# yangfei1223/CRFConv

Measured on AMD Instinct MI355X. Metric: M points/sec fwd+bwd, S3DIS 40960-pt cloud, K=16, 3 CRF iters; mIoU parity, higher is better.
Workload: dtype f32; 1 GPU; BASELINE configs[1]: S3DIS-like synthetic clouds (one point per 4 cm voxel of an 8x8x3 m box), 4 clouds x 40960 pts per GPU, K=16, ratios [4,4,4,4,2], PointConvBig(in=6, classes=13, use_crf, steps=3), train mode: fwd + weighted CE + bwd + flat-bucket grad all-reduce + SGD(momentum) step; tables resident in HBM; point order from the device collate: morton; global_batch=4, points_per_cloud=40960, parallelism=dp1 (batch-sharded)

## Files before the change

crfconv_amd/_lib.py:

```python
import ctypes
import os

_HERE = os.path.dirname(os.path.abspath(__file__))
LIB_PATH = os.environ.get('CRFCONV_LIB') or os.path.join(_HERE, 'libcrfconv_amd.so')

_vp, _i, _i64, _sz, _f = ctypes.c_void_p, ctypes.c_int, ctypes.c_int64, ctypes.c_size_t, ctypes.c_float
_d = ctypes.c_double
_u64 = ctypes.c_uint64

SIGNATURES = {
    'crfconv_abi_version': (_i, []),
    'crfconv_last_error': (ctypes.c_char_p, []),
    'crfconv_knn': (_i, [_vp, _sz, _sz, _vp, _sz, _sz, _vp]),
    'crfconv_knn_omp': (_i, [_vp, _sz, _sz, _vp, _sz, _sz, _vp]),
    'crfconv_knn_batch': (_i, [_vp, _sz, _sz, _sz, _vp, _sz, _sz, _vp]),
    'crfconv_knn_batch_omp': (_i, [_vp, _sz, _sz, _sz, _vp, _sz, _sz, _vp]),
    'crfconv_knn_batch_dev_workspace': (_sz, [_sz, _sz, _sz, _sz]),
    'crfconv_knn_batch_dev': (_i, [_vp, _sz, _sz, _sz, _vp, _sz, _sz, _vp, _vp, _vp, _sz, _vp]),
    'crfconv_fps': (_i, [_vp, _i, _vp, _vp, _vp, _vp, _vp, _vp, _vp, _vp]),
    'crfconv_grid_subsample': (_i64, [_vp, _i64, _vp, _i, _vp, _i, _f, _vp, _vp, _vp, _i64]),
    'crfconv_grid_subsample_dev_workspace': (_sz, [_i64, _i, _i]),
    'crfconv_grid_subsample_dev': (_i64, [_vp, _i64, _vp, _i, _vp, _i, _f, _vp, _vp, _vp, _i64, _vp, _sz, _vp]),
    'crfconv_index_narrow': (_i, [_vp, _i64, _i64, _i, _i64, _vp, _vp, _vp, _vp]),
    'crfconv_index_narrow_sorted': (_i, [_vp, _i64, _i64, _i, _i64, _i, _vp, _vp, _vp, _vp]),
    'crfconv_reverse_csr_workspace': (_sz, [_i64, _i64]),
    'crfconv_reverse_csr': (_i, [_vp, _i64, _i64, _vp, _vp, _vp, _sz, _vp]),
    'crfconv_reverse_csr_batched_workspace': (_sz, [_vp, _i]),
    'crfconv_reverse_csr_batched': (_i, [_vp, _i, _vp, _sz, _vp]),
    'crfconv_meanfield_forward': (_i, [_vp, _vp, _vp, _i, _i, _i64, _i, _vp, _vp, _i, _vp, _vp, _vp]),
    'crfconv_meanfield_forward_u16': (_i, [_vp, _vp, _vp, _vp, _i, _i, _i, _i, _i64, _i, _vp, _vp, _i, _vp, _vp, _vp]),
    'crfconv_meanfield_forward_block_rows': (_i, [_i64, _i, _i, _i, _i]),
    'crfconv_meanfield_forward_block': (_i, [_vp, _vp, _vp, _vp, _i, _i, _i, _i, _i64, _i, _vp, _vp, _i, _vp, _vp, _vp, _vp]),
    'crfconv_meanfield_forward_block_stamps': (_i, [_vp, _vp, _vp, _vp, _i, _i, _i64, _vp, _vp, _i, _vp, _vp, _vp, _i, _vp, _vp]),
    'crfconv_block_locality': (_i, [_vp, _i64, _i, _i, _i, _vp, _vp]),
    'crfconv_meanfield_bwd_edge': (_i, [_vp, _vp, _vp, _vp, _i, _i, _i64, _i, _vp, _vp, _vp, _vp, _i, _vp]),
    'crfconv_meanfield_bwd_scatter': (_i, [_vp, _vp, _vp, _vp, _i, _i, _i64, _i, _vp, _vp, _vp]),
    'crfconv_meanfield_backward_supported': (_i, [_i, _i, _i]),
    'crfconv_meanfield_backward_param_grads_inside': (_i, [_i]),
    'crfconv_meanfield_backward_workspace': (_sz, [_i64, _i, _i]),
    'crfconv_meanfield_backward': (_i, [_vp] * 7 + [_i, _i, _vp, _vp, _i, _i, _i64, _i, _vp, _vp, _i] + [_vp] * 11 + [_sz, _vp, _vp]),
    'crfconv_wide_similarity': (_i, [_vp, _vp, _i, _i, _i64, _i, _vp, _vp]),
    'crfconv_wide_aggregate': (_i, [_vp, _vp, _vp, _i, _i, _i64, _i, _vp, _vp]),
    'crfconv_wide_bwd_edge': (_i, [_vp, _vp, _vp, _i, _i, _i64, _i, _vp, _i, _vp]),
    'crfconv_wide_scatter': (_i, [_vp, _vp, _vp, _vp, _i, _i64, _i, _vp, _i, _vp, _vp]),
    'crfconv_wide_similarity_bwd': (_i, [_vp, _vp, _vp, _vp, _i, _i, _i64, _i, _vp, _vp, _vp]),
    'crfconv_similarity_bwd': (_i, [_vp, _vp, _vp, _vp, _i, _i, _i64, _i, _vp, _vp, _vp]),
    'crfconv_similarity_bwd_scatter': (_i, [_vp, _vp, _vp, _vp, _vp, _i, _i, _i64, _i, _vp, _vp]),
    'crfconv_pointconv_workspace': (_sz, [_i64, _i, _i]),
    'crfconv_pointconv_moments_packed': (_i, [_vp, _vp, _vp, _i, _i64, ctypes.c_double, _vp, _vp, _vp, _vp, _vp, _sz, _vp]),
    'crfconv_pointconv_moments': (_i, [_vp, _vp, _vp, _i, _i64, _vp, _vp, _sz, _vp]),
    'crfconv_pointconv_stats': (_i, [_vp, _vp, _vp, _i, _i64, _i, _vp, _vp, _vp, _f, _vp, _vp, _vp, _vp, _sz, _vp]),
    'crfconv_pointconv_forward_uv': (_i, [_vp, _vp, _vp, _vp, _i, _i64, _i, _vp, _vp, _vp, _f, _vp, _vp, _vp, _vp, _vp, _vp, _sz, _vp, _vp]),
    'crfconv_pointconv_forward_uv_hosts': (_i, [_i, _i]),
    'crfconv_pointconv_forward_uv_hosting': (_i, [_vp, _vp, _vp, _vp, _i, _i64, _i, _vp, _vp, _vp, _f, _vp, _vp, _vp, _vp, _vp, _vp, _sz, _vp,
                                                  _vp, _vp, _i, _vp, _vp, _vp]),
    'crfconv_pointconv_combine': (_i, [_vp, _vp, _vp, _vp, _vp, _vp, _d, _vp, _vp, _f, _f, _i64, _i, _vp, _vp, _vp, _vp, _vp]),
    'crfconv_pointconv_bwd_reduce_uv': (_i, [_vp, _vp, _vp, _i64, _i, _vp, _vp, _vp, _d, _i, _vp, _vp, _vp, _vp, _vp, _vp, _sz, _vp, _vp]),
    'crfconv_pointconv_forward': (_i, [_vp, _vp, _vp, _vp, _i, _i64, _i, _vp, _vp, _vp, _f, _vp, _vp, _vp, _vp]),
    'crfconv_pointconv_bwd_reduce': (_i, [_vp, _vp, _vp, _vp, _vp, _i, _i64, _i, _vp, _vp, _vp, _f, _vp, _vp, _vp, _sz, _vp]),
    'crfconv_pointconv_bwd_params': (_i, [_vp, _vp, _vp, _vp, _vp, _i, _i64, _i, _vp, _vp, _vp, _f, _vp, _vp, _vp,
                                          _vp, _vp, _vp, _sz, _vp]),
    'crfconv_pointconv_bwd_dump': (_i, [_vp, _vp, _vp, _vp, _vp, _i, _i64, _i, _vp, _vp, _vp, _f, _vp, _vp, _vp, _vp, _vp, _vp, _vp]),
    'crfconv_pointconv_bwd_a1_workspace': (_sz, [_i64, _i]),
    'crfconv_pointconv_bwd_a1': (_i, [_vp, _vp, _vp, _i64, _i, _f, _vp, _vp, _sz, _vp]),
    'crfconv_pointconv_bwd_input': (_i, [_vp, _vp, _vp, _vp, _vp, _i, _i64, _i, _vp, _vp, _vp, _f, _vp, _vp, _vp, _vp]),
    'crfconv_pointconv_bwd_input_reduce': (_i, [_vp, _vp, _vp, _vp, _vp, _i, _i64, _i64, _i, _vp, _vp, _vp, _f, _vp, _vp, _vp, _vp, _vp, _vp, _vp, _vp, _d, _i,
                                                _vp, _vp, _vp, _vp, _vp, _vp, _sz, _vp, _vp]),
    'crfconv_pointconv_fold1': (_i, [_vp, _vp, _vp, _vp, ctypes.c_double, _vp, _vp, _f, _f, _i, _i, _vp, _vp, _vp, _vp]),
    'crfconv_pointconv_fold1_batched': (_i, [_vp, _i, _vp]),
    'crfconv_pointconv_fold1_bwd_batched': (_i, [_vp, _i, _vp]),
    'crfconv_pointconv_fold1_bwd': (_i, [_vp, _vp, _vp, _vp, _vp, _f, _i, _i, _vp, _vp, _vp, _vp, _vp, _vp]),
    'crfconv_pointconv_fold2': (_i, [_vp, _vp, _vp, _vp, ctypes.c_double, _vp, _vp, _f, _f, _i, _i, _vp, _vp, _vp, _vp]),
    'crfconv_pointconv_fold2_bwd': (_i, [_vp, _vp, _vp, _vp, ctypes.c_double, _i, _i, _vp, _vp, _vp, _vp, _vp, _vp]),
    'crfconv_linear_wgrad_workspace': (_sz, [_i64, _i, _i]),
    'crfconv_linear_wgrad': (_i, [_vp, _vp, _i64, _i, _i, _vp, _vp, _vp, _sz, _vp]),
    'crfconv_random_subsets': (_i, [_vp, _vp, _vp, _vp, _i, _u64, _vp, _vp]),
    'crfconv_upindex_workspace': (_sz, [_i64, _i64]),
    'crfconv_upindex_from_table': (_i, [_vp, _vp, _vp, _vp, _i64, _i64, _i, _i64, _vp, _vp, _sz, _vp]),
    'crfconv_gather_rows_batched': (_i, [_vp, _vp, _vp, _i, _vp, _i, _i64, _i64, _i64, _vp]),
    'crfconv_argsort_codes_workspace': (_sz, [_i64, _i64]),
    'crfconv_argsort_codes': (_i, [_vp, _i64, _i64, _vp, _vp, _sz, _vp]),
    'crfconv_gridsync_workspace': (_sz, []),
    'crfconv_gridsync_fail_word': (_i, []),
    'crfconv_mlp_small_supported': (_i, [_i64, _i, _i]),
    'crfconv_mlp_small_workspace': (_sz, [_i64, _i]),
    'crfconv_mlp_small_forward': (_i, [_vp, _vp, _i64, _i, _i, _vp, _vp, _vp, _vp, _f, _f, _f, _vp, _vp, _vp, _vp, _sz, _vp, _sz, _vp]),
    'crfconv_mlp_small_forward_join': (_i, [_vp, _vp, _i64, _i, _i, _vp, _vp, _vp, _vp, _f, _f, _f, _vp, _f, _vp, _vp, _vp, _vp, _sz, _vp, _sz, _vp]),
    'crfconv_ticket_bytes': (_sz, []),
    'crfconv_mlp_backward_supported': (_i, [_i64, _i, _i]),
    'crfconv_mlp_backward_workspace': (_sz, [_i64, _i, _i]),
    'crfconv_mlp_backward': (_i, [_vp, _vp, _vp, _vp, _vp, _f, _i64, _i, _i, _vp, _vp, _vp, _vp, _vp, _sz, _vp, _vp]),
    'crfconv_linear_forward_cat': (_i, [_vp, _vp, _i, _vp, _vp, _i64, _i, _i, _vp, _vp, _vp]),
    'crfconv_linear_forward_uv_supported': (_i, [_i, _i]),
    'crfconv_linear_forward_uv': (_i, [_vp, _vp, _i64, _i, _i, _vp, _vp, _vp]),
    'crfconv_mlp_small_forward_uv_supported': (_i, [_i]),
    'crfconv_mlp_small_forward_join_uv': (_i, [_vp, _vp, _i64, _i, _i, _vp, _vp, _vp, _vp, _f, _f, _f, _vp, _f, _vp, _vp, _vp, _vp, _sz, _vp, _sz, _vp]),
    'crfconv_gemm_stats_uv_supported': (_i, [_i64, _i, _i]),
    'crfconv_gemm_stats_uv': (_i, [_vp, _vp, _i64, _i, _i, _vp, _vp, _vp]),
    'crfconv_mlp_dw_jobs': (_i, [_vp, _i, _vp]),
    'crfconv_mlp_dw_jobs_hosting': (_i, [_vp, _i, _vp, _vp, _vp, _vp, _vp, _i, _vp, _vp]),
    'crfconv_mlp_backward_add': (_i, [_vp, _vp, _vp, _vp, _vp, _f, _i64, _i, _i, _vp, _vp, _vp, _vp, _vp, _vp, _sz, _vp, _vp]),
    'crfconv_mlp_backward_add_mask': (_i, [_vp, _vp, _vp, _vp, _vp, _f, _i64, _i, _i, _vp, _f, _vp, _vp, _vp, _vp, _vp, _sz, _vp, _vp]),
    'crfconv_mlp_backward_cat': (_i, [_vp, _vp, _vp, _vp, _i, _vp, _vp, _f, _i64, _i, _i, _vp, _vp, _vp, _vp, _vp, _vp, _sz, _vp, _vp]),
    'crfconv_bn_workspace': (_sz, [_i64, _i]),
    'crfconv_bn_forward': (_i, [_vp, _i64, _i, _vp, _vp, _vp, _vp, _f, _f, _i, _f, _vp, _vp, _vp, _sz, _vp]),
    'crfconv_bn_backward': (_i, [_vp, _vp, _vp, _i64, _i, _i, _f, _vp, _vp, _vp, _vp, _sz, _vp]),
    'crfconv_bn_apply': (_i, [_vp, _i64, _i, _vp, _f, _vp, _vp]),
    'crfconv_pointconv_bwd_params_slabs': (_i, [_vp, _i64, _i, _vp, _vp, _vp]),
    'crfconv_pointconv_bwd_a1_nblk': (_i64, [_i64, _i]),
    'crfconv_reduce_jobs_f64': (_i, [_vp, _i, _vp]),
    'crfconv_pointconv_bwd_dump_jobs': (_i, [_vp, _i, _vp]),
    'crfconv_pointconv_bwd_a1_jobs': (_i, [_vp, _i, _vp]),
    'crfconv_pointconv_wide_params_supported': (_i, [_i64, _i, _i]),
    'crfconv_pointconv_wide_params_nblk': (_i64, [_i64, _i]),
    'crfconv_pointconv_wide_params_jobs': (_i, [_vp, _i, _vp]),
    'crfconv_gemm_jobs': (_i, [_vp, _i, _vp]),
    'crfconv_linear_wgrad_nblk': (_i, [_i64, _i, _i]),
    'crfconv_linear_wgrad_partial_jobs': (_i, [_vp, _i, _vp]),
    'crfconv_linear_wgrad_partial': (_i, [_vp, _vp, _i64, _i, _i, _i, _vp, _sz, _vp, _vp]),
    'crfconv_morton_codes': (_i, [_vp, _i64, _i64, _vp, _vp, _vp]),
    'crfconv_copy_jobs': (_i, [_vp, _i, _vp]),
    'crfconv_index_narrow_batched': (_i, [_vp, _i, _vp]),
    'crfconv_pointconv_moments_batched_workspace': (_sz, [_vp, _i]),
    'crfconv_pointconv_moments_batched': (_i, [_vp, _i, _vp, _sz, _vp]),
    'crfconv_reduce_jobs_both': (_i, [_vp, _i, _vp, _i, _vp]),
    'crfconv_reduce_jobs': (_i, [_vp, _i, _vp]),
    'crfconv_linear_forward_supported': (_i, [_i, _i]),
    'crfconv_linear_forward_stat_records': (_sz, [_i64]),
    'crfconv_linear_forward': (_i, [_vp, _vp, _vp, _i64, _i, _i, _i, _vp, _vp, _vp]),
    'crfconv_cat2': (_i, [_vp, _vp, _i64, _i, _i, _vp, _vp]),
    'crfconv_split2': (_i, [_vp, _i64, _i, _i, _vp, _vp, _vp]),
    'crfconv_add_i64': (_i, [_vp, _i64, _i64, _vp]),
    'crfconv_gate_mark': (_i, [_vp, _vp]),
    'crfconv_gate_wait': (_i, [_vp, _i, _vp]),
    'crfconv_mlp_small_backward_supported': (_i, [_i64, _i, _i]),
    'crfconv_gemm_stats_jobs': (_i, [_vp, _i, _vp]),
    'crfconv_bn_apply_from_records_jobs': (_i, [_vp, _i, _vp]),
    'crfconv_mlp_small_backward_jobs': (_i, [_vp, _i, _vp, _vp]),
    'crfconv_mlp_small_backward_jobs_one_launch': (_i, [_vp, _i, _vp, _vp, _vp]),
    'crfconv_mlp_small_backward_workspace': (_sz, [_i64, _i]),
    'crfconv_mlp_small_backward': (_i, [_vp, _vp, _vp, _vp, _vp, _i64, _i, _i, _i, _f, _vp, _vp, _vp, _vp, _vp, _sz, _vp, _vp]),
    'crfconv_gemm_stat_records': (_sz, [_i64]),
    'crfconv_gemm_stats': (_i, [_vp, _vp, _i64, _i, _i, _vp, _vp, _vp]),
    'crfconv_gemm_supported': (_i, [_i64, _i, _i]),
    'crfconv_gemm': (_i, [_vp, _vp, _vp, _vp, _i64, _i, _i, _i, _vp, _vp]),
    'crfconv_bn_apply_from_records': (_i, [_vp, _i64, _vp, _i64, _i, _vp, _vp, _vp, _vp, _f, _f, _vp, _f, _vp, _vp, _vp]),
    'crfconv_bn_coef_from_nrecords': (_i, [_vp, _i64, _i64, _i, _vp, _vp, _vp, _vp, _f, _f, _vp, _vp]),
    'crfconv_bn_coef_from_records': (_i, [_vp, _i64, _i, _vp, _vp, _vp, _vp, _f, _f, _vp, _vp]),
    'crfconv_softmax_ce_workspace': (_sz, [_i64]),
    'crfconv_softmax_ce_forward': (_i, [_vp, _vp, _vp, _i64, _i, _i64, _i64, _vp, _vp, _vp, _vp, _sz, _vp, _vp]),
    'crfconv_softmax_ce_backward': (_i, [_vp, _vp, _vp, _vp, _vp, _vp, _i64, _i, _i64, _i64, _vp, _vp]),
    'crfconv_crf_matrices': (_i, [_vp, _i, _vp, _vp, _vp]),
    'crfconv_crf_matrices_backward': (_i, [_vp, _vp, _vp, _vp, _i, _vp, _vp]),
    'crfconv_crf_matrices_batched': (_i, [_vp, _vp, _i, _vp, _vp, _vp]),
    'crfconv_crf_matrices_backward_batched': (_i, [_vp, _vp, _vp, _vp, _vp, _i, _vp, _vp]),
    'crfconv_add_lrelu': (_i, [_vp, _vp, _i64, _f, _vp, _vp]),
    'crfconv_bn_apply_add': (_i, [_vp, _i64, _i, _vp, _vp, _f, _vp, _vp]),
    'crfconv_bn_apply_dropout': (_i, [_vp, _i64, _i, _vp, _f, _f, _u64, _vp, _vp, _vp, _vp]),
    'crfconv_head_stats': (_i, [_vp, _vp, _i64, _i, _i, _vp, _vp]),
    'crfconv_head_stat_records': (_sz, [_i64]),
    'crfconv_head_supported': (_i, [_i64, _i, _i, _i]),
    'crfconv_head_mask_words': (_sz, [_i64]),
    'crfconv_head_backward_workspace': (_sz, [_i64, _i, _i, _i]),
    'crfconv_head_forward': (_i, [_vp, _vp, _vp, _f, _f, _u64, _vp, _vp, _vp, _i64, _i, _i, _i, _vp, _vp, _vp, _vp]),
    'crfconv_head_backward': (_i, [_vp, _vp, _vp, _vp, _f, _f, _vp, _vp, _i64, _i, _i, _i] + [_vp] * 7 + [_sz, _vp]),
    'crfconv_linear_forward_dropout': (_i, [_vp, _vp, _i64, _i, _i, _i, _f, _u64, _vp, _vp, _vp]),
    'crfconv_dropout_backward': (_i, [_vp, _i64, _f, _u64, _vp, _vp, _vp]),
    'crfconv_add_lrelu_backward': (_i, [_vp, _vp, _i64, _f, _vp, _vp]),
    'crfconv_add_mask': (_i, [_vp, _vp, _vp, _i64, _f, _vp, _vp]),
    'crfconv_sgd_step': (_i, [_vp, _vp, _vp, _i64, _f, _f, _f, _f, _i, _i, _vp]),
    'crfconv_sgd_step_hyper': (_i, [_vp, _vp, _vp, _i64, _vp, _i, _i, _vp]),
    'crfconv_sgd_step_guarded': (_i, [_vp, _vp, _vp, _i64, _vp, _i, _i, _vp, _vp]),
    'crfconv_sgd_step_guarded_all': (_i, [_vp, _vp, _vp, _i64, _vp, _i, _i, _vp, _i, _vp, _vp]),
    'crfconv_sgd_guard_publish': (_i, [_vp, _i, _vp, _vp]),
    'crfconv_adam_workspace': (_sz, [_i64]),
    'crfconv_adam_coef_floats': (_sz, []),
    'crfconv_adam_step': (_i, [_vp, _vp, _vp, _vp, _vp, _i64, _vp, _vp, _vp, _vp, _i, _i, _vp, _sz, _vp, _i, _vp, _vp]),
    'crfconv_spd_inverse': (_i, [_vp, _i, _vp, _vp]),
    'crfconv_spd_inverse_wide': (_i, [_vp, _i, _vp, _vp]),
    'crfconv_neighbor_maxpool_forward': (_i, [_vp, _vp, _i, _i64, _i, _vp, _vp, _vp]),
    'crfconv_neighbor_maxpool_affine_forward': (_i, [_vp, _vp, _vp, _i, _i64, _i, _vp, _vp, _vp]),
    'crfconv_neighbor_maxpool_backward': (_i, [_vp, _vp, _vp, _vp, _i, _i64, _i, _vp, _vp]),
    'crfconv_gather_rows': (_i, [_vp, _vp, _i64, _i, _vp, _vp]),
    'crfconv_gather_rows_backward': (_i, [_vp, _vp, _vp, _i64, _i, _vp, _vp]),
    'crfconv_meanfield_step': (_i, [_vp, _vp, _vp, _vp, _i, _i, _i64, _i, _vp, _vp, _vp, _vp]),
    'crfconv_kernel_weights_forward': (_i, [_vp, _vp, _i, _vp, _i, _i, _i64, _vp, _vp]),
    'crfconv_kernel_weights_partials': (_sz, [_i64]),
    'crfconv_kernel_weights_backward': (_i, [_vp, _vp, _vp, _vp, _vp, _i, _vp, _i, _i, _i64, _vp, _vp, _vp, _vp]),
    'crfconv_confusion_accumulate': (_i, [_vp, _vp, _vp, _i64, _i, _i64, _i64, _vp, _vp, _vp]),
    'crfconv_vote_accumulate': (_i, [_vp, _vp, _vp, _i64, _i, _d, _vp, _i64, _vp, _vp]),
    'crfconv_vote_accumulate_counted': (_i, [_vp, _vp, _vp, _i64, _i, _d, _vp, _i64, _vp, _vp, _vp]),
    'crfconv_vote_fold': (_i, [_vp, _vp, _vp, _vp, _i64, _i, _d, _vp]),
    'crfconv_vote_project': (_i, [_vp, _vp, _i64, _i, _i64, _i, _vp, _vp, _vp]),
    'crfconv_argmin_workspace': (_sz, []),
    'crfconv_argmin_f64': (_i, [_vp, _i64, _vp, _vp, _vp, _sz, _vp]),
    'crfconv_possibility_crop_workspace': (_sz, [_i64, _i64]),
    'crfconv_possibility_crop': (_i, [_vp, _i64, _i64, _vp, _vp, _vp, _vp, _vp, _vp, _vp, _vp, _vp, _sz, _vp]),
    'crfconv_augment_workspace': (_sz, [_i64, _i64]),
    'crfconv_augment': (_i, [_vp, _vp, _i64, _i64, _i, _vp, _u64, _vp, _vp, _vp, _vp, _vp, _sz, _vp]),
    'crfconv_possibility_crop_batch_workspace': (_sz, [_i64, _i64, _i64]),
    'crfconv_possibility_crop_batch': (_i, [_vp, _i, _i64, _vp, _vp, _i64, _i64, _u64, _vp, _d, _vp, _vp, _i, _vp, _vp, _i, _vp, _vp,
                                            _vp, _vp, _vp, _vp, _vp, _sz, _vp]),
    'crfconv_possibility_crop_batch_s3dis_workspace': (_sz, [_i64, _i64, _i64]),
    'crfconv_possibility_crop_batch_s3dis': (_i, [_vp, _i, _i64, _i64, _vp, _vp, _i64, _i64, _u64, _vp, _d, _vp, _vp, _i, _vp, _vp, _vp, _i,
                                                  _vp, _vp, _vp, _vp, _vp, _vp, _vp, _vp, _sz, _vp]),
    'crfconv_vote_update_repeated': (_i, [_vp, _vp, _vp, _i64, _i, _d, _vp, _i64, _vp, _vp, _vp, _vp]),
    'crfconv_vote_update_batch': (_i, [_vp, _i, _vp, _vp, _vp, _vp, _i64, _i64, _i64, _i, _d, _vp, _i, _vp]),
    'crfconv_vote_confusion': (_i, [_vp, _i64, _i, _vp, _vp, _i64, _i64, _vp, _vp, _vp]),
    'crfconv_linear_bn_act': (_i, [_vp, _vp, _i, _vp, _vp, _vp, _vp, _f, _i64, _i, _i, _vp, _vp]),
    'crfconv_gemm_bn_act': (_i, [_vp, _vp, _vp, _vp, _vp, _f, _i64, _i, _i, _i, _vp, _vp]),
    'crfconv_bn_eval_coef_jobs': (_i, [_vp, _i, _vp]),
}



class AugmentSpec(ctypes.Structure):
    _fields_ = [('rotate_axis', ctypes.c_int32), ('deg_lo', ctypes.c_float), ('deg_hi', ctypes.c_float), ('scale', ctypes.c_int32),
                ('scale_lo', ctypes.c_float), ('scale_span', ctypes.c_float), ('flip_axes', ctypes.c_int32), ('noise', ctypes.c_int32),
                ('sigma', ctypes.c_float), ('clip', ctypes.c_float), ('drop', ctypes.c_int32), ('drop_p', ctypes.c_float)]


class ReduceJob(ctypes.Structure):
    _fields_ = [('partial', ctypes.c_void_p), ('out', ctypes.c_void_p), ('nblk', ctypes.c_int32), ('nslots', ctypes.c_int32)]


class CopyJob(ctypes.Structure):
    _fields_ = [('src', ctypes.c_void_p), ('dst', ctypes.c_void_p), ('nbytes', ctypes.c_int64)]


class MlpDwJob(ctypes.Structure):
    _fields_ = [('workspace', ctypes.c_void_p), ('coef', ctypes.c_void_p), ('dW', ctypes.c_void_p), ('M', ctypes.c_int64),
                ('Ci', ctypes.c_int32), ('Co', ctypes.c_int32)]


class PcDumpJob(ctypes.Structure):
    _fields_ = [('x', ctypes.c_void_p), ('gout', ctypes.c_void_p), ('pos_src', ctypes.c_void_p), ('pos_tgt', ctypes.c_void_p),
                ('idx32', ctypes.c_void_p), ('K', ctypes.c_int32), ('m_tgt', ctypes.c_int64), ('d', ctypes.c_int32), ('A1', ctypes.c_void_p),
                ('b1', ctypes.c_void_p), ('W2', ctypes.c_void_p), ('slope', ctypes.c_float), ('ca', ctypes.c_void_p), ('cb', ctypes.c_void_p),
                ('cc', ctypes.c_void_p), ('h1', ctypes.c_void_p), ('gh2', ctypes.c_void_p), ('rel', ctypes.c_void_p)]


class PcWideJob(ctypes.Structure):
    _fields_ = [('x', ctypes.c_void_p), ('gout', ctypes.c_void_p), ('pos_src', ctypes.c_void_p), ('pos_tgt', ctypes.c_void_p),
                ('idx32', ctypes.c_void_p), ('K', ctypes.c_int32), ('m_tgt', ctypes.c_int64), ('d', ctypes.c_int32), ('A1', ctypes.c_void_p),
                ('b1', ctypes.c_void_p), ('W2', ctypes.c_void_p), ('slope', ctypes.c_float), ('ca', ctypes.c_void_p), ('cb', ctypes.c_void_p),
                ('cc', ctypes.c_void_p), ('dw2_partial', ctypes.c_void_p), ('a1_partial', ctypes.c_void_p)]

# ... 131 lines not shown
```

crfconv_amd/csrc/linear.hip:

```cpp
#include "common.hpp"
#include "gridsync.hpp"
#include "wgrad_body.hpp"
#include "crf_matrices_body.hpp"
#include "reduce64_body.hpp"
#include "uv_fold.hpp"

#include <cstdlib>

namespace crf {

template <int TCO, int TCI>
__global__ __launch_bounds__(WG_BLOCK) void wgrad_kernel(const float* __restrict__ G,
                                                         const float* __restrict__ X, int64_t M, int Co,
                                                         int Ci, int rows_per_block,
                                                         float* __restrict__ partial ,
                                                         float* __restrict__ partial_b ) {
    __shared__ float s_red[WG_RED_BUFS * TCO * TCI * 256];
    __shared__ float s_b[WG_WAVES * TCO * 16];
    wgrad_body<TCO, TCI>(G, X, M, Co, Ci, rows_per_block, partial, partial_b, blockIdx.x, blockIdx.y, blockIdx.z, s_red, s_b);
}

__global__ __launch_bounds__(WG_BLOCK) void wgrad_jobs_any_kernel(const WgJobTable t) {
    __shared__ float s_red[WG_RED_BUFS * 4 * 4 * 256];
    __shared__ float s_b[WG_WAVES * 4 * 16];
    wgrad_any_run(t, (int)blockIdx.x, s_red, s_b);
}


__device__ __forceinline__ void mlp_channel_part(int c, double s1, double s2, const float* __restrict__ coef, int64_t M, int Co,
                                                 float* __restrict__ dgamma, float* __restrict__ dbeta, float* __restrict__ bcoef) {
    dbeta[c] = (float)s1;
    dgamma[c] = (float)s2;
    const double a = coef[c], mu = coef[2 * Co + c], rs = coef[3 * Co + c];
    const double c2 = s1 / (double)M, c3 = s2 / (double)M;
    bcoef[c] = coef[c];
    bcoef[Co + c] = coef[Co + c];
    bcoef[2 * Co + c] = (float)a;
    bcoef[3 * Co + c] = (float)(-a * c3 * rs);
    bcoef[4 * Co + c] = (float)(-a * c2 + a * c3 * rs * mu);
}

template <int TCO, int TCI>
__global__ __launch_bounds__(WG_BLOCK) void mlp_bwd_p1_kernel(const float* __restrict__ GA, const float* __restrict__ Y,
                                                              const float* __restrict__ X,
                                                              const float* __restrict__ X2, int split ,
                                                              const float* __restrict__ coef ,
                                                              float slope, int64_t M, int Co, int Ci, int rows_per_block,
                                                              float* __restrict__ PA ,
                                                              float* __restrict__ PB ,
                                                              float* __restrict__ PG ,
                                                              float* __restrict__ PX ,
                                                              unsigned* __restrict__ ticket ,
                                                              float* __restrict__ dgamma, float* __restrict__ dbeta,
                                                              float* __restrict__ bcoef) {
    const int lane = threadIdx.x & 63, wave = threadIdx.x >> 6;
    const int co_base = blockIdx.y * 16 * TCO, ci_base = blockIdx.z * 16 * TCI;
    const int kk = lane >> 4, cc = lane & 15;
    f32x4 accA[TCO][TCI], accB[TCO][TCI];
#pragma unroll
    for (int a = 0; a < TCO; ++a)
#pragma unroll
        for (int b = 0; b < TCI; ++b) { accA[a][b] = f32x4{0.f, 0.f, 0.f, 0.f}; accB[a][b] = f32x4{0.f, 0.f, 0.f, 0.f}; }
    float ca[TCO], cb[TCO], cm[TCO], cr[TCO], sg[TCO], sgy[TCO], sx[TCI];
#pragma unroll
    for (int a = 0; a < TCO; ++a) {
        const int co = co_base + 16 * a + cc;
        const bool ok = co < Co;
        ca[a] = ok ? coef[co] : 0.f;
        cb[a] = ok ? coef[Co + co] : 0.f;
        cm[a] = ok ? coef[2 * Co + co] : 0.f;
        cr[a] = ok ? coef[3 * Co + co] : 0.f;
        sg[a] = 0.f;
        sgy[a] = 0.f;
    }
#pragma unroll
    for (int b = 0; b < TCI; ++b) sx[b] = 0.f;

    const int64_t row_begin = (int64_t)blockIdx.x * rows_per_block;
    const int64_t row_end = row_begin + rows_per_block < M ? row_begin + rows_per_block : M;
#ifndef P1_PREFETCH_
#define P1_PREFETCH_ 0
#endif
    struct Frag { float gv[4][TCO], yv[4][TCO], bv[4][TCI]; };
    auto load = [&](int64_t r0, Frag& f) {
#pragma unroll
        for (int u = 0; u < 4; ++u) {
            const int64_t r = r0 + 4 * u + kk;
            const bool rv = r < row_end;
#pragma unroll
            for (int a = 0; a < TCO; ++a) {
                const int co = co_base + 16 * a + cc;
                const bool ok = rv && co < Co;
                f.gv[u][a] = ok ? GA[r * Co + co] : 0.f;
                f.yv[u][a] = ok ? Y[r * Co + co] : cm[a];
            }
#pragma unroll
            for (int b = 0; b < TCI; ++b) {
                const int ci = ci_base + 16 * b + cc;
                float xv = 0.f;
                if (rv && ci < Ci) xv = (X2 == nullptr || ci < split) ? X[r * (X2 ? split : Ci) + ci] : X2[r * (Ci - split) + (ci - split)];
                f.bv[u][b] = xv;
            }
        }
    };
    auto compute = [&](const Frag& f) {
#pragma unroll
        for (int u = 0; u < 4; ++u) {
#pragma unroll
            for (int b = 0; b < TCI; ++b) sx[b] += f.bv[u][b];
#pragma unroll
            for (int a = 0; a < TCO; ++a) {
                const float g1 = f.gv[u][a] * (fmaf(ca[a], f.yv[u][a], cb[a]) > 0.f ? 1.f : slope);
                const float yh = (f.yv[u][a] - cm[a]) * cr[a];
                sg[a] += g1;
                sgy[a] = fmaf(g1, yh, sgy[a]);
#pragma unroll
                for (int b = 0; b < TCI; ++b) {
                    accA[a][b] = __builtin_amdgcn_mfma_f32_16x16x4f32(g1, f.bv[u][b], accA[a][b], 0, 0, 0);
                    accB[a][b] = __builtin_amdgcn_mfma_f32_16x16x4f32(yh, f.bv[u][b], accB[a][b], 0, 0, 0);
                }
            }
        }
    };
    if constexpr (P1_PREFETCH_ != 0) {
        Frag cur, nxt;
        load(row_begin + 16 * wave, cur);
        for (int64_t r0 = row_begin + 16 * wave; r0 < row_end; r0 += 16 * WG_WAVES) {
            load(r0 + 16 * WG_WAVES, nxt);
            compute(cur);
            cur = nxt;
        }
    } else {
        for (int64_t r0 = row_begin + 16 * wave; r0 < row_end; r0 += 16 * WG_WAVES) {
            Frag f;
            load(r0, f);
            compute(f);
        }
    }
    __shared__ __attribute__((aligned(16))) float s_red[WG_WAVES][TCO * TCI * 256];
    __shared__ float s_v[WG_WAVES][(2 * TCO + TCI) * 16];
    const int64_t pb = (int64_t)blockIdx.x;
    for (int pass = 0; pass < 2; ++pass) {
        if (pass) __syncthreads();
#pragma unroll
        for (int a = 0; a < TCO; ++a)
#pragma unroll
            for (int b = 0; b < TCI; ++b)
#pragma unroll
                for (int g = 0; g < 4; ++g)
                    s_red[wave][(a * TCI + b) * 256 + (4 * kk + g) * 16 + cc] = pass ? accB[a][b][g] : accA[a][b][g];
        if (pass == 0) {
#pragma unroll
            for (int a = 0; a < TCO; ++a) {
                float t1 = sg[a], t2 = sgy[a];
                t1 += __shfl_xor(t1, 16, WAVE); t1 += __shfl_xor(t1, 32, WAVE);
                t2 += __shfl_xor(t2, 16, WAVE); t2 += __shfl_xor(t2, 32, WAVE);
                if (kk == 0) { s_v[wave][a * 16 + cc] = t1; s_v[wave][(TCO + a) * 16 + cc] = t2; }
            }
// ... 465 lines not shown
    const bool live = (int)threadIdx.x < CMB_BLOCK && row < H && j < H;
    if (live) s_t[0][r][j] = (double)cmat[row * H + j];
    __syncthreads();
    double acc = 0.0;
    if (live)
        for (int k = 0; k < H; ++k) acc += s_t[0][r][k] * (double)s_q[k * 65 + j];
    if (live) s_t[1][r][j] = acc;
    __syncthreads();
    acc = 0.0;
    if (live)
        for (int k = 0; k < H; ++k) acc += s_t[1][r][k] * ((double)s_d[k * 65 + j] + (double)s_d[j * 65 + k]);
    if (live) s_t[0][r][j] = acc;
    __syncthreads();
    acc = 0.0;
    if (live) {
        for (int k = 0; k < H; ++k) acc += s_t[0][r][k] * (double)s_q[k * 65 + j];
        dc[row * H + j] = (float)(-acc);
    }
}
__global__ __launch_bounds__(CMB_BLOCK) void crf_matrices_bwd_kernel(const float* __restrict__ cmat, const float* __restrict__ Q,
                                                               const float* __restrict__ dQ, const float* __restrict__ dP,
                                                               int H, float* __restrict__ dc) {
    crf_matrices_bwd_slab(cmat, Q, dQ, dP, H, (int)blockIdx.x * CMB_ROWS, dc);
}
__global__ __launch_bounds__(CMB_BLOCK) void crf_matrices_bwd_batched_kernel(const CrfMatJobs j) {
    int b = 0;
    while (b + 1 < CM_MAX && (int)blockIdx.x >= j.slab_base[b + 1]) ++b;
    crf_matrices_bwd_slab(j.c[b], j.Q_in[b], j.gQ[b], j.gP[b], j.H[b], ((int)blockIdx.x - j.slab_base[b]) * CMB_ROWS, j.dc[b]);
}
static_assert(MF_BLOCK >= CMB_BLOCK, "a rider fits the host's workgroup");
__global__ __launch_bounds__(MF_BLOCK) void mlp_dw_jobs_hosting_kernel(const MlpDwTable t, const CrfMatJobs j, const int n_side) {
    if ((int)blockIdx.x < n_side) {
        int b = 0;
        while (b + 1 < CM_MAX && (int)blockIdx.x >= j.slab_base[b + 1]) ++b;
        crf_matrices_bwd_slab(j.c[b], j.Q_in[b], j.gQ[b], j.gP[b], j.H[b], ((int)blockIdx.x - j.slab_base[b]) * CMB_ROWS, j.dc[b]);
        return;
    }
    const int g = (int)blockIdx.x - n_side;
    int lo = 0, hi = t.njobs;
    while (hi - lo > 1) {
        const int mid = (lo + hi) >> 1;
        if (t.group_begin[mid] <= g) lo = mid; else hi = mid;
    }
    mlp_dw_slots(t.PA[lo], t.PB[lo], t.PG[lo], t.PX[lo], t.nblk[lo], t.coef[lo], (int64_t)t.M[lo], t.Co[lo], t.Ci[lo],
                 g - t.group_begin[lo], t.dW[lo]);
}
}

extern "C" int crfconv_crf_matrices_batched(const float* const* c, const int* H, int n, float* const* Q, float* const* P,
                                            crf_stream_t stream) {
    CRF_REQUIRE(c && H && Q && P && n >= 1 && n <= crf::CM_MAX, CRF_ERR_ARG, "null pointer or n=%d outside [1, %d]", n, crf::CM_MAX);
    crf::CrfMatJobs j = {};
    for (int i = 0; i < n; ++i) {
        CRF_REQUIRE(c[i] && Q[i] && P[i] && H[i] >= 1 && H[i] <= 64, CRF_ERR_ARG, "job %d: null pointer or H=%d outside [1, 64]", i, H[i]);
        j.c[i] = c[i]; j.Q[i] = Q[i]; j.P[i] = P[i]; j.H[i] = H[i];
    }
    hipLaunchKernelGGL(crf::crf_matrices_batched_kernel, dim3((unsigned)n), dim3(crf::CMF_BLOCK), 0, crf::as_stream(stream), j);
    CRF_LAUNCH_CHECK();
    return CRF_OK;
}

static int crf_matrices_bwd_jobs(const float* const* c, const float* const* Q, const float* const* gQ, const float* const* gP, const int* H, int n,
                                 float* const* dc, crf::CrfMatJobs& j, int& nslab) {
    CRF_REQUIRE(c && Q && gQ && gP && H && dc && n >= 1 && n <= crf::CM_MAX, CRF_ERR_ARG, "null pointer or n=%d outside [1, %d]", n, crf::CM_MAX);
    j = crf::CrfMatJobs();
    for (int i = 0; i < n; ++i) {
        CRF_REQUIRE(c[i] && Q[i] && dc[i] && H[i] >= 1 && H[i] <= 64, CRF_ERR_ARG, "job %d: null pointer or H=%d outside [1, 64]", i, H[i]);
        j.c[i] = c[i]; j.Q_in[i] = Q[i]; j.gQ[i] = gQ[i]; j.gP[i] = gP[i]; j.dc[i] = dc[i]; j.H[i] = H[i];
        j.slab_base[i + 1] = j.slab_base[i] + (H[i] + crf::CMB_ROWS - 1) / crf::CMB_ROWS;
    }
    nslab = j.slab_base[n];
    for (int i = n; i < crf::CM_MAX; ++i) j.slab_base[i + 1] = 0x7fffffff;
    return CRF_OK;
}
extern "C" int crfconv_crf_matrices_backward_batched(const float* const* c, const float* const* Q, const float* const* gQ,
                                                     const float* const* gP, const int* H, int n, float* const* dc,
                                                     crf_stream_t stream) {
    crf::CrfMatJobs j;
    int nslab = 0;
    if (int rc = crf_matrices_bwd_jobs(c, Q, gQ, gP, H, n, dc, j, nslab)) return rc;
    hipLaunchKernelGGL(crf::crf_matrices_bwd_batched_kernel, dim3((unsigned)nslab), dim3(crf::CMB_BLOCK), 0, crf::as_stream(stream), j);
    CRF_LAUNCH_CHECK();
    return CRF_OK;
}

namespace crf {
constexpr int SW_BLOCK = 1024, SW_MAXH = 512;
__global__ __launch_bounds__(SW_BLOCK) void spd_inverse_wide_kernel(const float* __restrict__ M, int H, float* __restrict__ Q) {
    __shared__ float s_row[SW_MAXH], s_col[SW_MAXH];
    const int n = H * H;
    for (int e = threadIdx.x; e < n; e += SW_BLOCK) Q[e] = M[e];
    __syncthreads();
    for (int k = 0; k < H; ++k) {
        for (int t = threadIdx.x; t < H; t += SW_BLOCK) {
            s_row[t] = Q[k * H + t];
            s_col[t] = Q[t * H + k];
        }
        __syncthreads();
        const float inv = 1.0f / s_row[k];
        for (int e = threadIdx.x; e < n; e += SW_BLOCK) {
            const int i = e / H, j = e - i * H;
            float v;
            if (i == k) v = j == k ? inv : s_row[j] * inv;
            else if (j == k) v = -s_col[i] * inv;
            else v = fmaf(-s_col[i] * inv, s_row[j], Q[e]);
            Q[e] = v;
        }
        __syncthreads();
    }
}
}

extern "C" int crfconv_spd_inverse_wide(const float* M, int H, float* Q, crf_stream_t stream) {
    CRF_REQUIRE(M && Q && M != Q, CRF_ERR_ARG, "null pointer / aliased operands");
    CRF_REQUIRE(H >= 1 && H <= crf::SW_MAXH, CRF_ERR_UNSUPPORTED, "H=%d outside [1, %d]", H, crf::SW_MAXH);
    hipLaunchKernelGGL(crf::spd_inverse_wide_kernel, dim3(1), dim3(crf::SW_BLOCK), 0, crf::as_stream(stream), M, H, Q);
    CRF_LAUNCH_CHECK();
    return CRF_OK;
}

extern "C" int crfconv_spd_inverse(const float* M, int H, float* Q, crf_stream_t stream) {
    CRF_REQUIRE(M && Q, CRF_ERR_ARG, "null pointer");
    CRF_REQUIRE(H >= 1 && H <= 64, CRF_ERR_UNSUPPORTED, "H=%d outside [1, 64]", H);
    hipLaunchKernelGGL(crf::spd_inverse_kernel, dim3(1), dim3(256), 0, crf::as_stream(stream), M, H, Q);
    CRF_LAUNCH_CHECK();
    return CRF_OK;
}

extern "C" int crfconv_crf_matrices(const float* c, int H, float* Q, float* P, crf_stream_t stream) {
    CRF_REQUIRE(c && Q && P, CRF_ERR_ARG, "null pointer");
    CRF_REQUIRE(H >= 1 && H <= 64, CRF_ERR_UNSUPPORTED, "H=%d outside [1, 64]", H);
    hipLaunchKernelGGL(crf::crf_matrices_kernel, dim3(1), dim3(crf::CMF_BLOCK), 0, crf::as_stream(stream), c, H, Q, P);
    CRF_LAUNCH_CHECK();
    return CRF_OK;
}

extern "C" int crfconv_crf_matrices_backward(const float* c, const float* Q, const float* dQ, const float* dP, int H,
                                             float* dc, crf_stream_t stream) {
    CRF_REQUIRE(c && Q && dc, CRF_ERR_ARG, "null pointer");
    CRF_REQUIRE(H >= 1 && H <= 64, CRF_ERR_UNSUPPORTED, "H=%d outside [1, 64]", H);
    hipLaunchKernelGGL(crf::crf_matrices_bwd_kernel, dim3((unsigned)((H + crf::CMB_ROWS - 1) / crf::CMB_ROWS)), dim3(crf::CMB_BLOCK), 0,
                       crf::as_stream(stream), c, Q, dQ, dP, H, dc);
    CRF_LAUNCH_CHECK();
    return CRF_OK;
}

namespace crf {

#ifndef LF_BLOCK_
#define LF_BLOCK_ 256
#endif
constexpr int LF_BLOCK = LF_BLOCK_, LF_WAVES = LF_BLOCK / WAVE;

constexpr int EPI_NONE = 0, EPI_ADD = 1, EPI_DROPOUT = 2, EPI_ADD_MASK = 3, EPI_UV = 4, EPI_BN_ACT = 5;
#ifndef LF_PF_MAX_
#define LF_PF_MAX_ 4
#endif
template <int TCO, bool PRO = false, bool VEC4 = true, int EPI = EPI_NONE, int NCH = 0>
__global__ __launch_bounds__(LF_BLOCK) void linear_fwd_kernel(const float* __restrict__ X, const float* __restrict__ W,
                                                              const float* __restrict__ bias, int64_t M, int Ci, int Co,
                                                              int transpose_w, float* __restrict__ Y,
                                                              float* __restrict__ stat_partial ,
                                                              const float* __restrict__ Y2 = nullptr,
                                                              const float* __restrict__ pro = nullptr, float slope = 1.f,
                                                              const float* __restrict__ Xb = nullptr, int xsplit = 0,
                                                              float* __restrict__ Yb = nullptr, int ysplit = 0,
                                                              const float* __restrict__ addend = nullptr,
                                                              const long long* __restrict__ drop_counter = nullptr,
                                                              unsigned long long drop_seed = 0ull, unsigned drop_threshold = 0u,
                                                              float drop_scale = 1.f,
                                                              const float* __restrict__ mask_ref = nullptr, float mask_slope = 1.f,
                                                              const UvFold uv = UvFold()) {
    static_assert(EPI != EPI_ADD_MASK || (PRO && VEC4), "the masked epilogue is the aligned dX product's");
    static_assert(EPI != EPI_UV || (!PRO && VEC4 && NCH == 1), "the combine prologue is the narrow aligned forward's");
    static_assert(EPI != EPI_BN_ACT || !PRO, "the BatchNorm epilogue is the forward product's");
    constexpr bool UV = EPI == EPI_UV, TWO = PRO || UV;
    constexpr bool BNA = EPI == EPI_BN_ACT;
    extern __shared__ float sW[];
    const int Cip = ((Ci + 15) / 16) * 16 + 4;
    const int Cik = ((Ci + 15) / 16) * 16;
    float* sPro = sW + 16 * TCO * Cip;
    [[maybe_unused]] float* sTile = sPro + (PRO ? 5 * Cik : 0);
    if constexpr (PRO) {
        for (int t = threadIdx.x; t < 5 * Cik; t += LF_BLOCK) {
            const int which = t / Cik, k = t - which * Cik;
            sPro[t] = k < Ci ? pro[which * Ci + k] : 0.f;
        }
    }
    const int co_base = blockIdx.y * 16 * TCO;
    if (!transpose_w && (Ci % 4) == 0) {
        const int Cip4 = Cip / 4, Ci4 = Ci / 4;
        for (int t = threadIdx.x; t < 16 * TCO * Cip4; t += LF_BLOCK) {
            const int r = t / Cip4, k4 = t - r * Cip4;
            const int co = co_base + r;
            float4 v = make_float4(0.f, 0.f, 0.f, 0.f);
            if (co < Co && k4 < Ci4) v = *reinterpret_cast<const float4*>(W + (int64_t)co * Ci + 4 * k4);
            *reinterpret_cast<float4*>(sW + r * Cip + 4 * k4) = v;
        }
    } else {
        for (int t = threadIdx.x; t < 16 * TCO * Cip; t += LF_BLOCK) {
            const int r = t / Cip, k = t - r * Cip;
            const int co = co_base + r;
            float v = 0.f;
            if (co < Co && k < Ci) v = transpose_w ? W[(int64_t)k * Co + co] : W[(int64_t)co * Ci + k];
            sW[t] = v;
        }
    }
    __syncthreads();
    const int lane = threadIdx.x & 63, wave = threadIdx.x >> 6;
    const int rr = lane & 15, g = lane >> 4;
    const bool vec = (Ci % 4) == 0;
    float bsel[TCO][4];
#pragma unroll
    for (int t = 0; t < TCO; ++t)
#pragma unroll
        for (int e = 0; e < 4; ++e) {
            const int co = co_base + 16 * t + 4 * g + e;
            bsel[t][e] = (bias != nullptr && co < Co) ? bias[co] : 0.f;
        }
    [[maybe_unused]] float4 bna[BNA ? TCO : 1], bnb[BNA ? TCO : 1];
    if constexpr (BNA) {
#pragma unroll
        for (int t = 0; t < TCO; ++t) {
            const int co = TCO >= 2 ? co_base + 4 * ((lane + WAVE * t) % (4 * TCO)) : co_base + 16 * t + 4 * g;
            bna[t] = bnb[t] = make_float4(0.f, 0.f, 0.f, 0.f);
            if (co < Co) {
                bna[t] = *reinterpret_cast<const float4*>(pro + co);
                bnb[t] = *reinterpret_cast<const float4*>(pro + Co + co);
            }
        }
    }
    [[maybe_unused]] auto bn_act4 = [&](float4 y, const float4 a, const float4 b, const float* skp) -> float4 {
        float4 o = make_float4(fmaf(a.x, y.x, b.x), fmaf(a.y, y.y, b.y), fmaf(a.z, y.z, b.z), fmaf(a.w, y.w, b.w));
        if (skp != nullptr) {
            const float4 k = *reinterpret_cast<const float4*>(skp);
            o = make_float4(add_rn(o.x, k.x), add_rn(o.y, k.y), add_rn(o.z, k.z), add_rn(o.w, k.w));
        }
        if (slope != 1.f) {
            o.x = o.x > 0.f ? o.x : slope * o.x;
            o.y = o.y > 0.f ? o.y : slope * o.y;
            o.z = o.z > 0.f ? o.z : slope * o.z;
            o.w = o.w > 0.f ? o.w : slope * o.w;
        }
        return o;
    };
    float s1[TCO][4], s2[TCO][4], sh[TCO][4];
#pragma unroll
    for (int t = 0; t < TCO; ++t)
#pragma unroll
        for (int e = 0; e < 4; ++e) { s1[t][e] = 0.f; s2[t][e] = 0.f; sh[t][e] = 0.f; }
    bool have_shift = false;
    const int nchunk = (Ci + 15) / 16;

    const float4 zero4 = make_float4(0.f, 0.f, 0.f, 0.f);
    auto load_raw = [&](int64_t r, bool rv, int c, float4& xa, float4& xb2) {
        const int k0 = 16 * c + 4 * g;
        xa = zero4;
        xb2 = zero4;
        if (!rv || k0 >= Ci) return;
        if constexpr (PRO) {
            xa = *reinterpret_cast<const float4*>(X + r * Ci + k0);
            xb2 = *reinterpret_cast<const float4*>(Y2 + r * Ci + k0);
        } else if constexpr (UV) {
            xa = *reinterpret_cast<const float4*>(X + r * Ci + k0);
            xb2 = *reinterpret_cast<const float4*>(uv.V + r * Ci + k0);
        } else if (Xb != nullptr) {
            if (k0 < xsplit) xa = *reinterpret_cast<const float4*>(X + r * xsplit + k0);
            else xa = *reinterpret_cast<const float4*>(Xb + r * (Ci - xsplit) + (k0 - xsplit));
        } else if (VEC4 || vec) {
            xa = *reinterpret_cast<const float4*>(X + r * Ci + k0);
        } else if constexpr (!VEC4) {
            const float* xp = X + r * Ci;
            xa.x = xp[k0];
            xa.y = k0 + 1 < Ci ? xp[k0 + 1] : 0.f;
            xa.z = k0 + 2 < Ci ? xp[k0 + 2] : 0.f;
            xa.w = k0 + 3 < Ci ? xp[k0 + 3] : 0.f;
        }
    };
    auto operand = [&](bool rv, int c, float4 gv, float4 yv) -> float4 {
        if constexpr (PRO) {
            const int k0 = 16 * c + 4 * g;
            float4 xv = zero4;
            if (rv && k0 < Ci) {
                const float4 pa = *reinterpret_cast<const float4*>(sPro + k0), pb = *reinterpret_cast<const float4*>(sPro + Cik + k0);
                const float4 al = *reinterpret_cast<const float4*>(sPro + 2 * Cik + k0), be = *reinterpret_cast<const float4*>(sPro + 3 * Cik + k0);
                const float4 de = *reinterpret_cast<const float4*>(sPro + 4 * Cik + k0);
                xv.x = fmaf(al.x * (fmaf(pa.x, yv.x, pb.x) > 0.f ? 1.f : slope), gv.x, fmaf(be.x, yv.x, de.x));
                xv.y = fmaf(al.y * (fmaf(pa.y, yv.y, pb.y) > 0.f ? 1.f : slope), gv.y, fmaf(be.y, yv.y, de.y));
                xv.z = fmaf(al.z * (fmaf(pa.z, yv.z, pb.z) > 0.f ? 1.f : slope), gv.z, fmaf(be.z, yv.z, de.z));
                xv.w = fmaf(al.w * (fmaf(pa.w, yv.w, pb.w) > 0.f ? 1.f : slope), gv.w, fmaf(be.w, yv.w, de.w));
            }
            return xv;
        } else {
            return gv;
        }
    };
    [[maybe_unused]] float4 uva = zero4, uvt = zero4;
    if constexpr (UV) {
        if (blockIdx.x == 0 && blockIdx.y == 0 && (int)threadIdx.x < Ci) {
            const UvCoef k = uv_coef(threadIdx.x, Ci, uv.stats, uv.shift, uv.gamma, uv.beta, uv.n_edges, uv.eps);
            uv_publish(threadIdx.x, Ci, k, uv.n_edges, uv.run_mean, uv.run_var, uv.momentum, uv.a2, uv.b2, uv.aux2);
        }
        if (4 * g < Ci) {
            float a[4], tv[4];
#pragma unroll
            for (int e = 0; e < 4; ++e) {
                const UvCoef k = uv_coef(4 * g + e, Ci, uv.stats, uv.shift, uv.gamma, uv.beta, uv.n_edges, uv.eps);
                a[e] = k.a;
                tv[e] = uv_vcoef(k);
            }
            uva = make_float4(a[0], a[1], a[2], a[3]);
            uvt = make_float4(tv[0], tv[1], tv[2], tv[3]);
        }
    }
    [[maybe_unused]] auto uv_operand = [&](int64_t r, bool rv, float4 u, float4 v) -> float4 {
        if (!rv || 4 * g >= Ci) return zero4;
        const float4 o = uv_out4(uva, uvt, u, v);
        if (blockIdx.y == 0) *reinterpret_cast<float4*>(uv.out + r * Ci + 4 * g) = o;
        return o;
    };
    constexpr int NCA = NCH > 0 ? NCH : 1;
    constexpr bool PF = NCH > 0 && NCH <= LF_PF_MAX_;
    const int64_t row_stride = (int64_t)gridDim.x * (LF_BLOCK / WAVE) * 16;
    [[maybe_unused]] float4 fa[NCA], fb[TWO ? NCA : 1], na[PF ? NCA : 1], nb[(PF && TWO) ? NCA : 1];
    [[maybe_unused]] auto load_group = [&](int64_t rw0, float4 (&xa)[NCA], float4 (&xb)[TWO ? NCA : 1]) {
        const int64_t rq = rw0 + rr;
        const bool ok = rw0 < M && rq < M;
#pragma unroll
        for (int c = 0; c < NCA; ++c) {
            float4 t0, t1;
            load_raw(rq, ok, c, t0, t1);
            xa[c] = t0;
            if constexpr (TWO) xb[c] = t1;
        }
    };
    if constexpr (PF) load_group(((int64_t)blockIdx.x * (LF_BLOCK / WAVE) + wave) * 16, fa, fb);
    for (int64_t row0 = ((int64_t)blockIdx.x * (LF_BLOCK / WAVE) + wave) * 16; row0 < M; row0 += row_stride) {
        const int64_t r = row0 + rr;
        const bool rv = r < M;
        f32x4 acc[TCO];
#pragma unroll
        for (int t = 0; t < TCO; ++t) acc[t] = f32x4{bsel[t][0], bsel[t][1], bsel[t][2], bsel[t][3]};
        if constexpr (NCH > 0) {
            if constexpr (PF) {
                if constexpr (TWO) load_group(row0 + row_stride, na, nb);
                else load_group(row0 + row_stride, na, fb);
            } else {
                load_group(row0, fa, fb);
            }
#pragma unroll
            for (int c = 0; c < NCH; ++c) {
                const int k0 = 16 * c + 4 * g;
                float4 xv;
                if constexpr (UV) xv = uv_operand(r, rv, fa[c], fb[c]);
                else xv = operand(rv, c, fa[c], fb[PRO ? c : 0]);
#pragma unroll
                for (int t = 0; t < TCO; ++t) {
                    const float4 wv = *reinterpret_cast<const float4*>(sW + (16 * t + rr) * Cip + k0);
                    acc[t] = __builtin_amdgcn_mfma_f32_16x16x4f32(wv.x, xv.x, acc[t], 0, 0, 0);
                    acc[t] = __builtin_amdgcn_mfma_f32_16x16x4f32(wv.y, xv.y, acc[t], 0, 0, 0);
                    acc[t] = __builtin_amdgcn_mfma_f32_16x16x4f32(wv.z, xv.z, acc[t], 0, 0, 0);
                    acc[t] = __builtin_amdgcn_mfma_f32_16x16x4f32(wv.w, xv.w, acc[t], 0, 0, 0);
                }
            }
            if constexpr (PF) {
#pragma unroll
                for (int c = 0; c < NCH; ++c) {
                    fa[c] = na[c];
                    if constexpr (TWO) fb[c] = nb[c];
                }
            }
        } else {
        for (int c = 0; c < nchunk; ++c) {
            const int k0 = 16 * c + 4 * g;
            float4 ra, rb;
            load_raw(r, rv, c, ra, rb);
            const float4 xv = operand(rv, c, ra, rb);
#pragma unroll
            for (int t = 0; t < TCO; ++t) {
                const float4 wv = *reinterpret_cast<const float4*>(sW + (16 * t + rr) * Cip + k0);
                acc[t] = __builtin_amdgcn_mfma_f32_16x16x4f32(wv.x, xv.x, acc[t], 0, 0, 0);
                acc[t] = __builtin_amdgcn_mfma_f32_16x16x4f32(wv.y, xv.y, acc[t], 0, 0, 0);
                acc[t] = __builtin_amdgcn_mfma_f32_16x16x4f32(wv.z, xv.z, acc[t], 0, 0, 0);
                acc[t] = __builtin_amdgcn_mfma_f32_16x16x4f32(wv.w, xv.w, acc[t], 0, 0, 0);
            }
        }
        }
        if constexpr (TCO >= 2) {
            constexpr int TW = 16 * TCO, TLD = TW + 4, F4R = TW / 4;
            float* tile = sTile + wave * 16 * TLD;
#pragma unroll
            for (int t = 0; t < TCO; ++t)
                *reinterpret_cast<float4*>(tile + rr * TLD + 16 * t + 4 * g) = make_float4(acc[t][0], acc[t][1], acc[t][2], acc[t][3]);
            __builtin_amdgcn_wave_barrier();
#pragma unroll
            for (int i = 0; i < (16 * F4R) / WAVE; ++i) {
                const int qd = lane + WAVE * i, trow = qd / F4R, tc4 = qd - trow * F4R;
                const int64_t orow = row0 + trow;
                const int co = co_base + 4 * tc4;
                if (orow < M && co < Co) {
                    float4 o4 = *reinterpret_cast<const float4*>(tile + trow * TLD + 4 * tc4);
                    if constexpr (EPI == EPI_ADD) {
                        {
                            if (VEC4 || (Co % 4) == 0) {
                                const float4 a4 = *reinterpret_cast<const float4*>(addend + orow * Co + co);
                                o4.x += a4.x; o4.y += a4.y; o4.z += a4.z; o4.w += a4.w;
                            } else {
                                o4.x += addend[orow * Co + co];
                                if (co + 1 < Co) o4.y += addend[orow * Co + co + 1];
                                if (co + 2 < Co) o4.z += addend[orow * Co + co + 2];
                                if (co + 3 < Co) o4.w += addend[orow * Co + co + 3];
                            }
                        }
                    }
                    if constexpr (EPI == EPI_ADD_MASK) {
                        const float4 a4 = *reinterpret_cast<const float4*>(addend + orow * Co + co);
                        const float4 r4 = *reinterpret_cast<const float4*>(mask_ref + orow * Co + co);
                        o4.x += a4.x; o4.y += a4.y; o4.z += a4.z; o4.w += a4.w;
                        o4.x = r4.x > 0.f ? o4.x : mask_slope * o4.x;
                        o4.y = r4.y > 0.f ? o4.y : mask_slope * o4.y;
                        o4.z = r4.z > 0.f ? o4.z : mask_slope * o4.z;
                        o4.w = r4.w > 0.f ? o4.w : mask_slope * o4.w;
                    }
                    if constexpr (BNA) o4 = bn_act4(o4, bna[i], bnb[i], addend != nullptr ? addend + orow * Co + co : nullptr);
                    if constexpr (EPI == EPI_DROPOUT) {
                        {
                            const unsigned long long ctr = (unsigned long long)drop_counter[0];
                            const unsigned long long e = (unsigned long long)(orow * Co + co);
                            o4.x = dropout_keep(drop_seed, ctr, e, drop_threshold) ? o4.x * drop_scale : 0.f;
                            o4.y = dropout_keep(drop_seed, ctr, e + 1, drop_threshold) ? o4.y * drop_scale : 0.f;
                            o4.z = dropout_keep(drop_seed, ctr, e + 2, drop_threshold) ? o4.z * drop_scale : 0.f;
                            o4.w = dropout_keep(drop_seed, ctr, e + 3, drop_threshold) ? o4.w * drop_scale : 0.f;
                        }
                    }
                    if (Yb != nullptr) {
                        if (co < ysplit) *reinterpret_cast<float4*>(Y + orow * ysplit + co) = o4;
                        else *reinterpret_cast<float4*>(Yb + orow * (Co - ysplit) + (co - ysplit)) = o4;
                    } else if (VEC4 || (Co % 4) == 0) {
                        *reinterpret_cast<float4*>(Y + orow * Co + co) = o4;
                    } else if constexpr (!VEC4) {
                        const float ov[4] = {o4.x, o4.y, o4.z, o4.w};
#pragma unroll
                        for (int e = 0; e < 4; ++e)
                            if (co + e < Co) Y[orow * Co + co + e] = ov[e];
                    }
                }
            }
            __builtin_amdgcn_wave_barrier();
        } else {
#pragma unroll
        for (int t = 0; t < TCO; ++t) {
            const int co = co_base + 16 * t + 4 * g;
            if constexpr (EPI == EPI_ADD) {
                if (rv) {
#pragma unroll
                    for (int e = 0; e < 4; ++e)
                        if (co + e < Co) acc[t][e] += addend[r * Co + co + e];
                }
            }
            if constexpr (EPI == EPI_ADD_MASK) {
                if (rv && co < Co) {
                    const float4 a4 = *reinterpret_cast<const float4*>(addend + r * Co + co);
                    const float4 r4 = *reinterpret_cast<const float4*>(mask_ref + r * Co + co);
                    const float av[4] = {a4.x, a4.y, a4.z, a4.w}, rf[4] = {r4.x, r4.y, r4.z, r4.w};
#pragma unroll
                    for (int e = 0; e < 4; ++e) {
                        const float v = acc[t][e] + av[e];
                        acc[t][e] = rf[e] > 0.f ? v : mask_slope * v;
                    }
                }
            }
            if constexpr (BNA) {
                if (rv && co < Co) {
                    const float4 o4 = bn_act4(make_float4(acc[t][0], acc[t][1], acc[t][2], acc[t][3]), bna[t], bnb[t],
                                              addend != nullptr ? addend + r * Co + co : nullptr);
                    acc[t] = f32x4{o4.x, o4.y, o4.z, o4.w};
                }
            }
            if constexpr (EPI == EPI_DROPOUT) {
                if (rv) {
                    const unsigned long long ctr = (unsigned long long)drop_counter[0];
#pragma unroll
                    for (int e = 0; e < 4; ++e)
                        if (co + e < Co)
                            acc[t][e] = dropout_keep(drop_seed, ctr, (unsigned long long)(r * Co + co + e), drop_threshold)
                                            ? acc[t][e] * drop_scale : 0.f;
                }
            }
            if (rv) {
                if (Yb != nullptr) {
                    const float4 o4 = make_float4(acc[t][0], acc[t][1], acc[t][2], acc[t][3]);
                    if (co < ysplit) *reinterpret_cast<float4*>(Y + r * ysplit + co) = o4;
                    else if (co < Co) *reinterpret_cast<float4*>(Yb + r * (Co - ysplit) + (co - ysplit)) = o4;
                } else if (VEC4) {
                    if (co < Co) *reinterpret_cast<float4*>(Y + r * Co + co) = make_float4(acc[t][0], acc[t][1], acc[t][2], acc[t][3]);
                } else if (co + 3 < Co && (Co % 4) == 0) {
                    *reinterpret_cast<float4*>(Y + r * Co + co) = make_float4(acc[t][0], acc[t][1], acc[t][2], acc[t][3]);
                } else if constexpr (!VEC4) {
#pragma unroll
                    for (int e = 0; e < 4; ++e)
                        if (co + e < Co) Y[r * Co + co + e] = acc[t][e];
                }
            }
        }
        }
        if (!BNA && stat_partial != nullptr) {
            if (!have_shift) {
// ... 22 lines not shown
        for (int64_t row0 = ((int64_t)blockIdx.x * (LF_BLOCK / WAVE) + wave) * 16; row0 < M;
             row0 += (int64_t)gridDim.x * (LF_BLOCK / WAVE) * 16)
            nrows += (M - row0) < 16 ? (M - row0) : 16;
#pragma unroll
        for (int t = 0; t < TCO; ++t)
#pragma unroll
            for (int e = 0; e < 4; ++e) {
                float a = s1[t][e], b = s2[t][e];
#pragma unroll
                for (int o = 8; o > 0; o >>= 1) {
                    a += __shfl_xor(a, o, WAVE);
                    b += __shfl_xor(b, o, WAVE);
                }
                if (rr == 0) {
                    const int cl = 16 * t + 4 * g + e;
                    sw[cl] = sh[t][e];
                    sw[16 * TCO + cl] = (float)nrows;
                    sw[2 * 16 * TCO + cl] = a;
                    sw[3 * 16 * TCO + cl] = b;
                }
            }
        __syncthreads();
        for (int cl = threadIdx.x; cl < 16 * TCO; cl += LF_BLOCK) {
            const int co = co_base + cl;
            if (co >= Co) continue;
            const float s0 = sW[cl];
            double n = 0.0, S1 = 0.0, S2 = 0.0;
            for (int w = 0; w < LF_BLOCK / WAVE; ++w) {
                const float* q = sW + w * 4 * 16 * TCO;
                const double nb = q[16 * TCO + cl];
                if (nb <= 0.0) continue;
                const double d = (double)q[cl] - (double)s0, a = q[2 * 16 * TCO + cl], b = q[3 * 16 * TCO + cl];
                n += nb;
                S1 += a + nb * d;
                S2 += b + 2.0 * d * a + nb * d * d;
            }
            *reinterpret_cast<float4*>(stat_partial + ((int64_t)blockIdx.x * Co + co) * 4) =
                make_float4(s0, (float)n, (float)S1, (float)S2);
        }
    }
}

constexpr int FR_BLOCK = 1024, FR_CH = 16, FR_RL = FR_BLOCK / FR_CH;
template <int FR_UN = 8>
__device__ __forceinline__ bool bn_finalize_records_body(const float* __restrict__ rec, int nrec, int64_t M, int C,
                                                         const float* __restrict__ gamma, const float* __restrict__ beta, float eps,
                                                         float* __restrict__ run_mean, float* __restrict__ run_var, float momentum,
                                                         float* __restrict__ coef, int slab, bool write, float (&ab)[2]) {
    __shared__ double s_red[FR_BLOCK / WAVE][2][FR_CH];
    const int cl = threadIdx.x & (FR_CH - 1), rl = threadIdx.x >> 4;
    const int c = slab * FR_CH + cl;
    const bool cv = c < C;
    const int cc = cv ? c : C - 1;
    const double s0 = rec[(int64_t)cc * 4];
    double S1 = 0.0, S2 = 0.0;
    for (int r0 = rl; r0 < nrec; r0 += FR_UN * FR_RL) {
        float4 v[FR_UN];
#pragma unroll
        for (int u = 0; u < FR_UN; ++u) {
            const int r = r0 + u * FR_RL;
            v[u] = r < nrec ? *reinterpret_cast<const float4*>(rec + ((int64_t)r * C + cc) * 4)
                            : make_float4(0.f, 0.f, 0.f, 0.f);
        }
#pragma unroll
        for (int u = 0; u < FR_UN; ++u) {
            const double nb = v[u].y;
            if (nb > 0.0) {
                const double d = (double)v[u].x - s0, a = v[u].z, b = v[u].w;
                S1 += a + nb * d;
                S2 += b + 2.0 * d * a + nb * d * d;
            }
        }
    }
    S1 += __shfl_xor(S1, 16, WAVE); S2 += __shfl_xor(S2, 16, WAVE);
    S1 += __shfl_xor(S1, 32, WAVE); S2 += __shfl_xor(S2, 32, WAVE);
    const int wave = threadIdx.x >> 6;
    if ((threadIdx.x & 63) < FR_CH) { s_red[wave][0][cl] = S1; s_red[wave][1][cl] = S2; }
    __syncthreads();
    if (threadIdx.x >= FR_CH || !cv) return false;
    S1 = 0.0; S2 = 0.0;
    for (int w = 0; w < FR_BLOCK / WAVE; ++w) { S1 += s_red[w][0][cl]; S2 += s_red[w][1][cl]; }
    const double m1 = S1 / (double)M;
    const double mean = s0 + m1;
    const double m2 = S2 - S1 * m1;
    double var = m2 / (double)M;
    if (var < 0.0) var = 0.0;
    const double rstd = 1.0 / sqrt(var + (double)eps);
    const double a = (double)gamma[c] * rstd;
    ab[0] = (float)a;
    ab[1] = (float)((double)beta[c] - a * mean);
    if (!write) return true;
    coef[c] = ab[0];
    coef[C + c] = ab[1];
    coef[2 * C + c] = (float)mean;
    coef[3 * C + c] = (float)rstd;
    if (run_mean != nullptr) {
        const double unb = M > 1 ? var * ((double)M / (double)(M - 1)) : var;
        run_mean[c] = (float)((1.0 - (double)momentum) * (double)run_mean[c] + (double)momentum * mean);
        run_var[c] = (float)((1.0 - (double)momentum) * (double)run_var[c] + (double)momentum * unb);
    }
    return true;
}
__global__ __launch_bounds__(FR_BLOCK) void bn_finalize_records_kernel(const float* __restrict__ rec, int nrec, int64_t M,
                                                                       int C, const float* __restrict__ gamma,
                                                                       const float* __restrict__ beta, float eps,
                                                                       float* __restrict__ run_mean, float* __restrict__ run_var,
                                                                       float momentum, float* __restrict__ coef) {
    float ab[2];
    bn_finalize_records_body(rec, nrec, M, C, gamma, beta, eps, run_mean, run_var, momentum, coef, blockIdx.x, true, ab);
}

template <bool ADD, int UN = 8>
__device__ __forceinline__ void bn_apply_records_body(const float* __restrict__ rec, int nrec, int64_t M, int C,
                                                      const float* __restrict__ gamma, const float* __restrict__ beta,
                                                      float eps, float* __restrict__ run_mean, float* __restrict__ run_var,
                                                      float momentum, float* __restrict__ coef, const float* __restrict__ x,
                                                      const float* __restrict__ skip, float slope, int rows_per_tile,
                                                      float* __restrict__ y, const int slab, const int tile) {
    __shared__ float s_ab[2][FR_CH];
    float ab[2];
    const int q = threadIdx.x & 3, rl = threadIdx.x >> 2;
    const int c = slab * FR_CH + 4 * q;
    const bool cok = c < C;
    const int64_t r0 = (int64_t)tile * rows_per_tile;
    const int64_t r1 = r0 + rows_per_tile < M ? r0 + rows_per_tile : M;
    float4 v[4];
    [[maybe_unused]] float4 k[ADD ? 4 : 1];
    auto request = [&](int64_t rb) {
#pragma unroll
        for (int u = 0; u < 4; ++u) {
            const int64_t r = rb + (int64_t)u * (FR_BLOCK / 4);
            const bool in = cok && r < r1;
            v[u] = in ? *reinterpret_cast<const float4*>(x + r * C + c) : make_float4(0.f, 0.f, 0.f, 0.f);
            if constexpr (ADD) k[u] = in ? *reinterpret_cast<const float4*>(skip + r * C + c) : make_float4(0.f, 0.f, 0.f, 0.f);
        }
    };
#ifndef BN_APPLY_PREFETCH_
#define BN_APPLY_PREFETCH_ 1
#endif
    if (BN_APPLY_PREFETCH_) request(r0 + rl);
    if (bn_finalize_records_body<UN>(rec, nrec, M, C, gamma, beta, eps, run_mean, run_var, momentum, coef, slab, tile == 0, ab)) {
        s_ab[0][threadIdx.x] = ab[0];
        s_ab[1][threadIdx.x] = ab[1];
    }
    __syncthreads();
    if (!cok) return;
    const float4 a = *reinterpret_cast<const float4*>(&s_ab[0][4 * q]), b = *reinterpret_cast<const float4*>(&s_ab[1][4 * q]);
    for (int64_t rb = r0 + rl; rb < r1; rb += 4 * (FR_BLOCK / 4)) {
        if (!BN_APPLY_PREFETCH_ || rb != r0 + rl) request(rb);
#pragma unroll
        for (int u = 0; u < 4; ++u) {
            const int64_t r = rb + (int64_t)u * (FR_BLOCK / 4);
            if (r >= r1) continue;
            float4 o = make_float4(fmaf(a.x, v[u].x, b.x), fmaf(a.y, v[u].y, b.y), fmaf(a.z, v[u].z, b.z), fmaf(a.w, v[u].w, b.w));
            if constexpr (ADD) {
                o.x = add_rn(o.x, k[u].x); o.y = add_rn(o.y, k[u].y); o.z = add_rn(o.z, k[u].z); o.w = add_rn(o.w, k[u].w);
            }
            o.x = o.x > 0.f ? o.x : slope * o.x;
            o.y = o.y > 0.f ? o.y : slope * o.y;
            o.z = o.z > 0.f ? o.z : slope * o.z;
            o.w = o.w > 0.f ? o.w : slope * o.w;
            *reinterpret_cast<float4*>(y + r * C + c) = o;
        }
    }
}

template <bool ADD>
__global__ __launch_bounds__(FR_BLOCK) void bn_apply_records_kernel(const float* __restrict__ rec, int nrec, int64_t M, int C,
                                                                    const float* __restrict__ gamma, const float* __restrict__ beta,
                                                                    float eps, float* __restrict__ run_mean, float* __restrict__ run_var,
                                                                    float momentum, float* __restrict__ coef, const float* __restrict__ x,
                                                                    const float* __restrict__ skip, float slope, int rows_per_tile,
                                                                    float* __restrict__ y) {
    bn_apply_records_body<ADD>(rec, nrec, M, C, gamma, beta, eps, run_mean, run_var, momentum, coef, x, skip, slope, rows_per_tile, y,
                               blockIdx.y, blockIdx.x);
}
constexpr int BA_MAX = 4;
struct BnApplyJobs {
    const float* rec[BA_MAX]; const float* gamma[BA_MAX]; const float* beta[BA_MAX]; float* run_mean[BA_MAX]; float* run_var[BA_MAX];
    float* coef[BA_MAX]; const float* x[BA_MAX]; const float* skip[BA_MAX]; float* y[BA_MAX];
    long long M[BA_MAX];
    int nrec[BA_MAX], C[BA_MAX], rows_per_tile[BA_MAX], tiles[BA_MAX];
    float eps[BA_MAX], momentum[BA_MAX], slope[BA_MAX];
    int blk_base[BA_MAX + 1];
    int njobs;
};
__global__ __launch_bounds__(FR_BLOCK) void bn_apply_records_jobs_kernel(const BnApplyJobs t) {
    int j = 0;
    while (j + 1 < t.njobs && t.blk_base[j + 1] <= (int)blockIdx.x) ++j;
    const int local = (int)blockIdx.x - t.blk_base[j];
    const int tiles = uni(t.tiles[j]);
    const int tile = uni(local % tiles), slab = uni(local / tiles);
    const float* rec = uni(t.rec[j]); const float* gamma = uni(t.gamma[j]); const float* beta = uni(t.beta[j]);
    float* run_mean = uni(t.run_mean[j]); float* run_var = uni(t.run_var[j]); float* coef = uni(t.coef[j]);
    const float* x = uni(t.x[j]); const float* skip = uni(t.skip[j]); float* y = uni(t.y[j]);
    const long long M = uni(t.M[j]);
    const int nrec = uni(t.nrec[j]), C = uni(t.C[j]), rows = uni(t.rows_per_tile[j]);
    const float eps = uni(t.eps[j]), momentum = uni(t.momentum[j]), slope = uni(t.slope[j]);
    if (skip != nullptr) bn_apply_records_body<true, 4>(rec, nrec, M, C, gamma, beta, eps, run_mean, run_var, momentum, coef, x, skip, slope, rows, y, slab, tile);
    else bn_apply_records_body<false, 4>(rec, nrec, M, C, gamma, beta, eps, run_mean, run_var, momentum, coef, x, nullptr, slope, rows, y, slab, tile);
}

static int lf_blocks(int64_t M) {
    constexpr int cap = 512;
    int64_t nb = (M + 16 * LF_WAVES - 1) / (16 * LF_WAVES);
    if (nb > cap) nb = cap;
    return (int)(nb < 1 ? 1 : nb);
}

}

static size_t lf_lds_bytes_at(int Ci, int tco, bool pro) {
    const size_t cip = (size_t)((Ci + 15) / 16) * 16 + 4, cik = cip - 4;
    size_t floats = 16 * (size_t)tco * cip;
    const size_t stats = (size_t)crf::LF_WAVES * 4 * 16 * (size_t)tco;
    if (floats < stats) floats = stats;
    if (pro) floats += 5 * cik;
    if (tco >= 2) floats += (size_t)crf::LF_WAVES * 16 * (16 * (size_t)tco + 4);
    return sizeof(float) * floats;
}
static int lf_tco(int Ci, int Co, bool pro) {
    constexpr int max_tco = 4;
    const int tiles = (Co + 15) / 16;
    int tco = tiles >= 8 ? 8 : (tiles >= 4 ? 4 : (tiles >= 2 ? 2 : 1));
    if (tco > max_tco) tco = max_tco;
    while (tco > 1 && lf_lds_bytes_at(Ci, tco, pro) > 64 * 1024) tco >>= 1;
    return tco;
}
static size_t lf_lds_bytes(int Ci, int Co, bool pro) { return lf_lds_bytes_at(Ci, lf_tco(Ci, Co, pro), pro); }
static int lf_hoist_chunks(int Ci, bool vec4) {
    if (!vec4 || Ci > 128) return 0;
    const int n = (Ci + 15) / 16;
    return n <= 1 ? 1 : (n <= 2 ? 2 : (n <= 4 ? 4 : 8));
}

extern "C" int crfconv_linear_forward_supported(int Ci, int Co) {
    if (Ci < 1 || Co < 1) return 0;
    return lf_lds_bytes(Ci, Co, false) <= 64 * 1024 ? 1 : 0;
}

extern "C" size_t crfconv_linear_forward_stat_records(int64_t M) { return (size_t)crf::lf_blocks(M); }

struct LinearDropout {
    const long long* counter = nullptr;
    unsigned long long seed = 0ull;
    unsigned threshold = 0u;
    float scale = 1.f;
};

struct LinearBnAct {
    const float* coef = nullptr;
    const float* skip = nullptr;
    float slope = 1.f;
};

static int linear_forward_impl(const float* X, const float* Xb, int xsplit, const float* W, const float* bias, int64_t M,
                               int Ci, int Co, int transpose_w, float* Y, float* stat_rec, crf_stream_t stream,
                               LinearDropout drop = LinearDropout(), LinearBnAct bn = LinearBnAct()) {
    CRF_REQUIRE(X && W && Y, CRF_ERR_ARG, "null pointer");
    CRF_REQUIRE(M > 0, CRF_ERR_ARG, "M must be positive");
    CRF_REQUIRE(crfconv_linear_forward_supported(Ci, Co), CRF_ERR_UNSUPPORTED, "weight slab %dx%d does not fit LDS", Co, Ci);
    CRF_REQUIRE(Xb == nullptr || (xsplit > 0 && xsplit < Ci && xsplit % 4 == 0 && Ci % 4 == 0), CRF_ERR_ARG,
                "two-operand form needs 0 < split < Ci, both multiples of 4 (split=%d Ci=%d)", xsplit, Ci);
    const int tiles = (Co + 15) / 16;
    const int tco = lf_tco(Ci, Co, false);
    const int gy = (tiles + tco - 1) / tco;
    const dim3 grid((unsigned)crf::lf_blocks(M), (unsigned)gy), blk(crf::LF_BLOCK);
    const size_t lds = lf_lds_bytes(Ci, Co, false);
    hipStream_t st = crf::as_stream(stream);
    const bool vec4 = (Ci % 4) == 0 && (Co % 4) == 0;
    const int nch = lf_hoist_chunks(Ci, vec4);
#define LF4(T, V, E, N) hipLaunchKernelGGL((crf::linear_fwd_kernel<T, false, V, E, N>), grid, blk, lds, st, X, W, bias, M, Ci, Co, transpose_w, Y, stat_rec, (const float*)nullptr, bn.coef, bn.slope, Xb, xsplit, (float*)nullptr, 0, bn.skip, drop.counter, drop.seed, drop.threshold, drop.scale)
#define LF3(T, V, E) do { if (V && nch == 1) LF4(T, V, E, 1); else if (V && nch == 2) LF4(T, V, E, 2); else if (V && nch == 4) LF4(T, V, E, 4); else if (V && nch == 8) LF4(T, V, E, 8); else LF4(T, V, E, 0); } while (0)
#define LF2(T, V) do { if (bn.coef != nullptr) LF3(T, V, crf::EPI_BN_ACT); else if (drop.counter != nullptr) LF4(T, V, crf::EPI_DROPOUT, 0); else LF3(T, V, crf::EPI_NONE); } while (0)
#define LF(T) do { if (vec4) LF2(T, true); else if (bn.coef != nullptr) LF4(T, false, crf::EPI_BN_ACT, 0); else if (drop.counter != nullptr) LF4(T, false, crf::EPI_DROPOUT, 0); else LF4(T, false, crf::EPI_NONE, 0); } while (0)
    switch (tco) {
        case 1: LF(1); break;
        case 2: LF(2); break;
        case 4: LF(4); break;
        default: LF(8); break;
    }
#undef LF
#undef LF2
#undef LF3
#undef LF4
    CRF_LAUNCH_CHECK();
    return CRF_OK;
}

extern "C" int crfconv_linear_forward(const float* X, const float* W, const float* bias, int64_t M, int Ci, int Co,
                                      int transpose_w, float* Y, float* stat_rec, crf_stream_t stream) {
    return linear_forward_impl(X, nullptr, 0, W, bias, M, Ci, Co, transpose_w, Y, stat_rec, stream);
}

extern "C" int crfconv_linear_forward_dropout(const float* X, const float* W, int64_t M, int Ci, int Co, int transpose_w,
                                              float p, uint64_t seed, const int64_t* counter, float* Y, crf_stream_t stream) {
    CRF_REQUIRE(counter, CRF_ERR_ARG, "null pointer");
    CRF_REQUIRE(p >= 0.f && p < 1.f, CRF_ERR_ARG, "dropout probability %g outside [0, 1)", (double)p);
    LinearDropout d;
    d.counter = reinterpret_cast<const long long*>(counter);
    d.seed = (unsigned long long)seed;
    d.threshold = crf::dropout_threshold(p);
    d.scale = 1.f / (1.f - p);
    return linear_forward_impl(X, nullptr, 0, W, nullptr, M, Ci, Co, transpose_w, Y, nullptr, stream, d);
}

extern "C" int crfconv_linear_forward_cat(const float* Xa, const float* Xb, int split, const float* W, const float* bias,
                                          int64_t M, int Ci, int Co, float* Y, float* stat_rec, crf_stream_t stream) {
    CRF_REQUIRE(Xb, CRF_ERR_ARG, "null pointer");
    return linear_forward_impl(Xa, Xb, split, W, bias, M, Ci, Co, 0, Y, stat_rec, stream);
}

extern "C" int crfconv_linear_bn_act(const float* X, const float* Xb, int split, const float* W, const float* bias, const float* coef,
                                     const float* skip, float slope, int64_t M, int Ci, int Co, float* Y, crf_stream_t stream) {
    CRF_REQUIRE(coef, CRF_ERR_ARG, "null pointer");
    CRF_REQUIRE(Co % 4 == 0, CRF_ERR_UNSUPPORTED, "Co=%d must be a multiple of 4", Co);
    LinearBnAct bn;
    bn.coef = coef;
    bn.skip = skip;
    bn.slope = slope;
    return linear_forward_impl(X, Xb, Xb ? split : 0, W, bias, M, Ci, Co, 0, Y, nullptr, stream, LinearDropout(), bn);
}

extern "C" int crfconv_linear_forward_uv_supported(int Ci, int Co) { return ((Ci == 8 && Co == 32) || (Ci == 16 && Co == 64)) ? 1 : 0; }

extern "C" int crfconv_linear_forward_uv(const crf_uv_fold* f, const float* W, int64_t M, int Ci, int Co, float* Y, float* stat_rec,
                                         crf_stream_t stream) {
    CRF_REQUIRE(W && Y, CRF_ERR_ARG, "null pointer");
    CRF_REQUIRE(crf::uv_fold_complete(f), CRF_ERR_ARG, "combine record: null pointer, or running statistics not as a pair");
    CRF_REQUIRE(M > 0, CRF_ERR_ARG, "M must be positive");
    CRF_REQUIRE(crfconv_linear_forward_uv_supported(Ci, Co), CRF_ERR_UNSUPPORTED, "combine prologue: %d -> %d is not a fine-level lin_out", Ci, Co);
    const int tco = lf_tco(Ci, Co, false);
    CRF_REQUIRE(16 * tco == Co && lf_hoist_chunks(Ci, true) == 1, CRF_ERR_UNSUPPORTED, "combine prologue: one column group, one chunk");
    const dim3 grid((unsigned)crf::lf_blocks(M), 1u), blk(crf::LF_BLOCK);
    const size_t lds = lf_lds_bytes(Ci, Co, false);
    hipStream_t st = crf::as_stream(stream);
    const crf::UvFold uv = crf::uv_fold_args(f);
#define LFU(T) hipLaunchKernelGGL((crf::linear_fwd_kernel<T, false, true, crf::EPI_UV, 1>), grid, blk, lds, st, f->U, W, (const float*)nullptr, M, Ci, Co, 0, Y, stat_rec, (const float*)nullptr, (const float*)nullptr, 1.f, (const float*)nullptr, 0, (float*)nullptr, 0, (const float*)nullptr, (const long long*)nullptr, 0ull, 0u, 1.f, (const float*)nullptr, 1.f, uv)
    if (tco == 2) LFU(2);
    else LFU(4);
#undef LFU
    CRF_LAUNCH_CHECK();
    return CRF_OK;
}

extern "C" int crfconv_bn_coef_from_records(const float* stat_rec, int64_t M, int C, const float* gamma,
                                            const float* beta, float* run_mean, float* run_var, float momentum,
                                            float eps, float* coef, crf_stream_t stream) {
    CRF_REQUIRE(stat_rec && gamma && beta && coef, CRF_ERR_ARG, "null pointer");
    CRF_REQUIRE(M > 0 && C > 0, CRF_ERR_ARG, "bad shape");
    return crfconv_bn_coef_from_nrecords(stat_rec, (int64_t)crfconv_linear_forward_stat_records(M), M, C, gamma, beta, run_mean, run_var,
                                         momentum, eps, coef, stream);
}

extern "C" int crfconv_bn_coef_from_nrecords(const float* stat_rec, int64_t nrec, int64_t M, int C, const float* gamma,
                                             const float* beta, float* run_mean, float* run_var, float momentum,
                                             float eps, float* coef, crf_stream_t stream) {
    CRF_REQUIRE(stat_rec && gamma && beta && coef, CRF_ERR_ARG, "null pointer");
    CRF_REQUIRE(M > 0 && C > 0 && nrec > 0 && nrec < ((int64_t)1 << 31), CRF_ERR_ARG, "bad shape");
    hipLaunchKernelGGL(crf::bn_finalize_records_kernel, dim3((C + crf::FR_CH - 1) / crf::FR_CH), dim3(crf::FR_BLOCK), 0, crf::as_stream(stream), stat_rec,
                       (int)nrec, M, C, gamma, beta, eps, run_mean, run_var, momentum, coef);
    CRF_LAUNCH_CHECK();
    return CRF_OK;
}

#ifndef BN_APPLY_WGS_
#define BN_APPLY_WGS_ 256
#endif
static void bn_apply_plan(int64_t M, int C, int wgs, int64_t& tiles, int64_t& rows) {
    const int slabs = (C + crf::FR_CH - 1) / crf::FR_CH;
    tiles = wgs / slabs;
    if (tiles < 1) tiles = 1;
    rows = (M + tiles - 1) / tiles;
    rows = (rows + 1023) / 1024 * 1024;
    tiles = (M + rows - 1) / rows;
    if (tiles > 8) tiles = (tiles + 7) / 8 * 8;
}

extern "C" int crfconv_bn_apply_from_records(const float* stat_rec, int64_t nrec, const float* x, int64_t M, int C, const float* gamma,
                                             const float* beta, float* run_mean, float* run_var, float momentum, float eps,
                                             const float* skip, float slope, float* coef, float* y, crf_stream_t stream) {
    CRF_REQUIRE(stat_rec && x && gamma && beta && coef && y, CRF_ERR_ARG, "null pointer");
    CRF_REQUIRE(M > 0 && C >= 4 && C % 4 == 0 && nrec > 0 && nrec < ((int64_t)1 << 31), CRF_ERR_ARG, "bad shape");
    const int slabs = (C + crf::FR_CH - 1) / crf::FR_CH;
    int64_t tiles, rows;
    bn_apply_plan(M, C, BN_APPLY_WGS_, tiles, rows);
    const dim3 grid((unsigned)tiles, (unsigned)slabs), blk(crf::FR_BLOCK);
    if (skip != nullptr)
        hipLaunchKernelGGL(crf::bn_apply_records_kernel<true>, grid, blk, 0, crf::as_stream(stream), stat_rec, (int)nrec, M, C, gamma, beta, eps,
                           run_mean, run_var, momentum, coef, x, skip, slope, (int)rows, y);
    else
        hipLaunchKernelGGL(crf::bn_apply_records_kernel<false>, grid, blk, 0, crf::as_stream(stream), stat_rec, (int)nrec, M, C, gamma, beta, eps,
                           run_mean, run_var, momentum, coef, x, skip, slope, (int)rows, y);
    CRF_LAUNCH_CHECK();
    return CRF_OK;
}

extern "C" int crfconv_bn_apply_from_records_jobs(const crf_bn_apply_job* jobs, int njobs, crf_stream_t stream) {
    CRF_REQUIRE(jobs && njobs >= 1 && njobs <= crf::BA_MAX, CRF_ERR_ARG, "1 .. %d jobs (got %d)", crf::BA_MAX, njobs);
    crf::BnApplyJobs t;
    int64_t blocks = 0;
    for (int j = 0; j <= crf::BA_MAX; ++j) {
        t.blk_base[j] = (int)blocks;
        if (j >= crf::BA_MAX) break;
        if (j >= njobs) {
            t.rec[j] = nullptr; t.gamma[j] = nullptr; t.beta[j] = nullptr; t.run_mean[j] = nullptr; t.run_var[j] = nullptr; t.coef[j] = nullptr;
            t.x[j] = nullptr; t.skip[j] = nullptr; t.y[j] = nullptr; t.M[j] = 0; t.nrec[j] = 0; t.C[j] = 4; t.rows_per_tile[j] = 1024; t.tiles[j] = 1;
            t.eps[j] = 0.f; t.momentum[j] = 0.f; t.slope[j] = 1.f;
            continue;
        }
        const crf_bn_apply_job& b = jobs[j];
        CRF_REQUIRE(b.stat_rec && b.x && b.gamma && b.beta && b.coef && b.y, CRF_ERR_ARG, "job %d: null pointer", j);
        CRF_REQUIRE(b.M > 0 && b.C >= 4 && b.C % 4 == 0 && b.nrec > 0 && b.nrec < ((int64_t)1 << 31), CRF_ERR_ARG, "job %d: bad shape", j);
        int64_t tiles, rows;
        bn_apply_plan(b.M, b.C, BN_APPLY_WGS_ / njobs, tiles, rows);
        t.rec[j] = b.stat_rec; t.gamma[j] = b.gamma; t.beta[j] = b.beta; t.run_mean[j] = b.run_mean; t.run_var[j] = b.run_var; t.coef[j] = b.coef;
        t.x[j] = b.x; t.skip[j] = b.skip; t.y[j] = b.y; t.M[j] = (long long)b.M; t.nrec[j] = (int)b.nrec; t.C[j] = b.C; t.rows_per_tile[j] = (int)rows;
        t.tiles[j] = (int)tiles; t.eps[j] = b.eps; t.momentum[j] = b.momentum; t.slope[j] = b.slope;
        blocks += tiles * ((b.C + crf::FR_CH - 1) / crf::FR_CH);
        CRF_REQUIRE(blocks < ((int64_t)1 << 31), CRF_ERR_UNSUPPORTED, "too many workgroups in one batch");
    }
    t.njobs = njobs;
    hipLaunchKernelGGL(crf::bn_apply_records_jobs_kernel, dim3((unsigned)blocks), dim3(crf::FR_BLOCK), 0, crf::as_stream(stream), t);
    CRF_LAUNCH_CHECK();
    return CRF_OK;
}

namespace crf {
struct MlpPlan {
    int tco, tci, gy, gz, nblk, rows_per_block;
};
static MlpPlan mlp_plan(int64_t M, int Co, int Ci) {
    MlpPlan p;
    const int t_co = (Co + 15) / 16, t_ci = (Ci + 15) / 16;
    p.tco = t_co >= 4 ? 4 : (t_co >= 2 ? 2 : 1);
    p.tci = t_ci >= 4 ? 4 : (t_ci >= 2 ? 2 : 1);
    if (p.tco * p.tci == 16) p.tci = 2;
    p.gy = (t_co + p.tco - 1) / p.tco;
    p.gz = (t_ci + p.tci - 1) / p.tci;
#ifndef MLP_P1_TARGET_
#define MLP_P1_TARGET_ 512
#endif
    constexpr int target = MLP_P1_TARGET_;
    int64_t slices = target / ((int64_t)p.gy * p.gz);
    if (slices < 32) slices = 32;
    int64_t rows = (M + slices - 1) / slices;
    if (rows < 64) rows = 64;
    rows = (rows + 63) / 64 * 64;
    p.rows_per_block = (int)rows;
    p.nblk = (int)((M + rows - 1) / rows);
    return p;
}
static size_t mlp_ws_layout(int64_t M, int Co, int Ci, size_t off[5]) {
    const MlpPlan p = mlp_plan(M, Co, Ci);
    auto up = [](size_t v) { return (v + 255) & ~(size_t)255; };
    size_t o = 0;
    off[0] = o; o = up(o + sizeof(float) * (size_t)p.nblk * Co * Ci);
    off[1] = o; o = up(o + sizeof(float) * (size_t)p.nblk * Co * Ci);
    off[2] = o; o = up(o + sizeof(float) * (size_t)p.nblk * 2 * Co);
    off[3] = o; o = up(o + sizeof(float) * (size_t)p.nblk * Ci);
    off[4] = o; o = up(o + sizeof(float) * 5 * (size_t)Co);
    return o;
}
}

extern "C" size_t crfconv_ticket_bytes(void) { return sizeof(unsigned) * crf::LW_TICKET_WORDS; }

extern "C" int crfconv_mlp_backward_supported(int64_t M, int Ci, int Co) {
    if (!(M > 0 && Co % 4 == 0 && Ci >= 1 && Co >= 4 && Co <= 1024 && Ci <= 1024)) return 0;
    return lf_lds_bytes(Co, Ci, true) <= 64 * 1024 ? 1 : 0;
}

extern "C" size_t crfconv_mlp_backward_workspace(int64_t M, int Ci, int Co) {
    if (M <= 0 || Co <= 0 || Ci <= 0) return 0;
    size_t off[5];
    return crf::mlp_ws_layout(M, Co, Ci, off) + 256;
}

static int mlp_backward_impl(const float* gA, const float* Y, const float* X, const float* Xb, int xsplit, const float* W,
                             const float* coef, float slope, int64_t M, int Ci, int Co, float* dX, float* dXb, float* dW,
                             float* dgamma, float* dbeta, void* workspace, size_t workspace_bytes, unsigned* ticket,
                             crf_stream_t stream, const float* dX_add = nullptr, const float* mask_ref = nullptr,
                             float mask_slope = 1.f);

extern "C" int crfconv_mlp_backward(const float* gA, const float* Y, const float* X, const float* W, const float* coef,
                                    float slope, int64_t M, int Ci, int Co, float* dX, float* dW, float* dgamma,
                                    float* dbeta, void* workspace, size_t workspace_bytes, unsigned* ticket,
                                    crf_stream_t stream) {
    return mlp_backward_impl(gA, Y, X, nullptr, 0, W, coef, slope, M, Ci, Co, dX, nullptr, dW, dgamma, dbeta, workspace,
                             workspace_bytes, ticket, stream);
}

extern "C" int crfconv_mlp_backward_add(const float* gA, const float* Y, const float* X, const float* W, const float* coef,
                                        float slope, int64_t M, int Ci, int Co, const float* dX_add, float* dX, float* dW,
// ... 161 lines not shown
```

crfconv_amd/models/common.py:

```python
import torch
import torch.nn as nn

from .. import ops
from ..graph import require_gpu


class FastBatchNorm1d(nn.Module):
    def __init__(self, num_features, momentum=0.1, **kwargs):
        super().__init__()
        self.batch_norm = nn.BatchNorm1d(num_features, momentum=momentum, **kwargs)

    def forward(self, x):
        if x.dim() not in (2, 3):
            raise ValueError('Non supported number of dimensions {}'.format(x.dim()))
        bn = self.batch_norm
        if not bn.affine or x.dtype != torch.float32:
            raise ops._lib.CrfConvError('FastBatchNorm1d: affine float32 BatchNorm only (the kernels of csrc/bn.hip); got affine=%s, %s'
                                        % (bn.affine, x.dtype))
        return ops.bn_act(x, bn, self.training)


class MLP(nn.Module):

    def __init__(self, in_channels, out_channels, bn=True, activation=None):
        super(MLP, self).__init__()
        self.lin = nn.Linear(in_channels, out_channels, bias=not bn)
        self.bn = FastBatchNorm1d(out_channels) if bn else None
        self.activation = activation

    def forward(self, x, *args, **kwargs):
        require_gpu(x)
        co = self.lin.out_features
        fusable = (self.bn is not None and x.dtype == torch.float32 and co % 4 == 0 and co <= 1024
                   and self.bn.batch_norm.affine
                   and (self.activation is None or isinstance(self.activation, nn.LeakyReLU)))
        if fusable:
            slope = 1.0 if self.activation is None else self.activation.negative_slope
            if ops.mlp_block_ok(x, self.lin.weight, self.lin.bias, self.bn.batch_norm, self.training):
                return ops.mlp_block(x, self.lin.weight, self.bn.batch_norm, slope)
            records = None
            if self.training:
                x, records = ops.linear(x, self.lin.weight, self.lin.bias, want_stats=True)
            else:
                x = ops.linear(x, self.lin.weight, self.lin.bias)
            slope = 1.0 if self.activation is None else self.activation.negative_slope
            return ops.bn_act(x, self.bn.batch_norm, self.training, slope, records=records)
        x = ops.linear(x, self.lin.weight, self.lin.bias)
        if self.bn is not None:
            x = self.bn(x)
        if self.activation is not None:
            x = self.activation(x)
        return x


def mlp_fork(mlp, x, input_mask=None):
    if (mlp.training and mlp.bn is not None and x.dtype == torch.float32 and mlp.bn.batch_norm.affine and x.requires_grad
            and mlp.lin.out_features % 4 == 0 and mlp.lin.out_features <= 1024
            and (mlp.activation is None or isinstance(mlp.activation, nn.LeakyReLU))
            and ops.mlp_block_ok(x, mlp.lin.weight, mlp.lin.bias, mlp.bn.batch_norm, True)):
        require_gpu(x)
        slope = 1.0 if mlp.activation is None else mlp.activation.negative_slope
        return ops.mlp_block(x, mlp.lin.weight, mlp.bn.batch_norm, slope, fork=True, input_mask=input_mask)
    return mlp(x), x


def _group_spec(mlp, x):
    if not (isinstance(mlp, MLP) and mlp.training and mlp.bn is not None and mlp.lin.bias is None and x.dtype == torch.float32
            and mlp.bn.batch_norm.affine and (mlp.activation is None or isinstance(mlp.activation, nn.LeakyReLU))):
        return None
    return mlp.lin.weight, mlp.bn.batch_norm, (1.0 if mlp.activation is None else mlp.activation.negative_slope)


def mlp_group(pairs, shared=False, input_mask=None):
    blocks = []
    for mlp, x, fork in pairs:
        spec = _group_spec(mlp, x)
        if spec is None:
            return None
        require_gpu(x)
        blocks.append((x, spec[0], spec[1], spec[2], fork))
    return ops.mlp_group(blocks, shared=shared, input_mask=input_mask)


def mlp_join(mlp, x, skip, slope=0.01, mask=None, combine=None):
    if (mlp.training and mlp.bn is not None and mlp.activation is None and mlp.lin.bias is None and x.dtype == torch.float32
            and mlp.bn.batch_norm.affine and mlp.lin.out_features % 4 == 0):
        out = ops.mlp_block_join(x, mlp.lin.weight, mlp.bn.batch_norm, skip, slope, mask=mask, combine=combine)
        if out is not None:
            return out
    if combine is not None:
        combine.flush()
    return ops.add_lrelu(mlp(x), skip, slope)


class Base(nn.Module):

    def save(self, filename):
        torch.save(self.state_dict(), filename)

    def __getstate__(self):
        state = dict(super().__getstate__())
        state.pop('_autograph', None)
        return state

    def _apply(self, fn, *args, **kwargs):
        self.__dict__.pop('_autograph', None)
        return super()._apply(fn, *args, **kwargs)

    def load(self, filename):
        self.load_state_dict(torch.load(filename))
```

crfconv_amd/models/point_conv_big.py:

```python
import torch
import torch.nn as nn
import torch.nn.functional as F

from .. import ops
from ..graph import table_of
from .common import MLP, Base, mlp_fork, mlp_group, mlp_join
from .continuous_crf_conv_big import ContinuousGaussianCRFConv as CRFConv

WIDTHS = (32, 64, 128, 256, 512)


def _lrelu():
    return nn.LeakyReLU(negative_slope=0.1)


def _flat(t):
    return t.reshape(-1, t.shape[-1])


class PointConv(nn.Module):

    def __init__(self, d_model):
        super().__init__()
        self.weight_nn = nn.Sequential(MLP(3, d_model, activation=_lrelu()), MLP(d_model, d_model, activation=None))

    def _moments(self, table, p_src, p_tgt):
        key = ('moments', p_src.data_ptr(), p_tgt.data_ptr(), tuple(p_src.shape), tuple(p_tgt.shape))
        entry = table.cache.get(key)
        if entry is None:
            ps, pt = p_src.float().contiguous(), p_tgt.float().contiguous()
            keep_s = p_src if ps.data_ptr() == p_src.data_ptr() else ps
            keep_t = p_tgt if pt.data_ptr() == p_tgt.data_ptr() else pt
            entry = table.cache[key] = ops.MomentsEntry(ops.relpos_moments(ps, pt, table), keep_s, keep_t)
        elif entry.stale():
            entry.refresh_(table)
        return entry

    def _geometry(self, pos, neighbor_idx):
        strided = not torch.is_tensor(pos)
        src = pos[0] if strided else pos
        p_src = _flat(src)
        p_tgt = _flat(pos[1]) if strided else p_src
        return table_of(neighbor_idx, src.shape[1]), p_src, p_tgt

    def prefold_entry(self, pos, neighbor_idx):
        table, p_src, p_tgt = self._geometry(pos, neighbor_idx)
        first = self.weight_nn[0]
        return first.lin.weight, first.bn.batch_norm, self._moments(table, p_src, p_tgt), table

    def forward(self, x, pos, neighbor_idx, prefold=None, defer_combine=False):
        table, p_src, p_tgt = self._geometry(pos, neighbor_idx)
        first, second = self.weight_nn[0], self.weight_nn[1]
        y = ops.point_conv(_flat(x), p_src, p_tgt, table, first.lin.weight, first.bn.batch_norm, second.lin.weight,
                           second.bn.batch_norm, self.training, moments=self._moments(table, p_src, p_tgt), prefold=prefold,
                           defer_combine=defer_combine)
        if defer_combine:
            return y[0].reshape(x.shape[0], -1, x.shape[-1]), y[1]
        return y.reshape(x.shape[0], -1, x.shape[-1])


class ResNetBBlock(nn.Module):

    def __init__(self, in_channels, out_channels):
        super().__init__()
        mid = out_channels // 4
        self.lin_in = MLP(in_channels, mid, activation=_lrelu())
        self.lin_out = MLP(mid, out_channels, activation=None)
        self.shortcut = MLP(in_channels, out_channels, activation=None) if in_channels != out_channels else nn.Identity()
        self.point_conv = PointConv(mid)

    @staticmethod
    def max_pooling(x, idx):
        pooled = ops.neighbor_maxpool(_flat(x), table_of(idx, x.shape[1]))
        return pooled.reshape(x.shape[0], -1, x.shape[-1])

    def forward(self, x, pos, neighbor_idx, return_input_alias=False, prefold=None, join_mask=None, input_mask=None):
        strided = not torch.is_tensor(pos)
        skip = None
        sc = self.shortcut
        grouped = None
        if isinstance(sc, MLP):
            grouped = mlp_group([(self.lin_in, x, True), (sc, x, False)], shared=True, input_mask=input_mask)
        if grouped is not None:
            (h_in, x), skip = grouped
            if strided:
                skip = self.max_pooling(skip, neighbor_idx)
            y, comb = self.point_conv(h_in, pos, neighbor_idx, prefold=prefold, defer_combine=True)
            out = mlp_join(self.lin_out, y, skip, 0.01, mask=join_mask, combine=comb)
            return (out, x) if return_input_alias else out
        h_in, x = mlp_fork(self.lin_in, x, input_mask)
        if (strided and self.training and isinstance(sc, MLP) and sc.bn is not None and sc.activation is None
                and sc.lin.bias is None and x.dtype == torch.float32 and sc.bn.batch_norm.affine):
            pooled = ops.mlp_block_pool(_flat(x), sc.lin.weight, sc.bn.batch_norm, table_of(neighbor_idx, x.shape[1]),
                                        fork=return_input_alias)
            if pooled is not None:
                if return_input_alias:
                    pooled, alias = pooled
                    x = alias.reshape(x.shape)
                skip = pooled.reshape(x.shape[0], -1, pooled.shape[-1])
        if skip is None:
            if return_input_alias and isinstance(sc, MLP):
                skip, x = mlp_fork(sc, x)
            else:
                skip = sc(x)
            if strided:
                skip = self.max_pooling(skip, neighbor_idx)
        y, comb = self.point_conv(h_in, pos, neighbor_idx, prefold=prefold, defer_combine=True)
        out = mlp_join(self.lin_out, y, skip, 0.01, mask=join_mask, combine=comb)
        return (out, x) if return_input_alias else out


class Upsampling(nn.Module):

    def __init__(self, down_channels, up_channels, out_channels):
        super().__init__()
        self.lin = MLP(down_channels, up_channels, activation=_lrelu())
        self.fusion = MLP(up_channels * 2, out_channels, activation=_lrelu())

    @staticmethod
    def upsampling(x, idx):
        up = ops.gather_rows(_flat(x), table_of(idx, x.shape[1]))
        return up.reshape(x.shape[0], -1, x.shape[-1])

    def forward(self, x_down, x_up, up_idx, neighbor_idx=None):
        return self.fusion(ops.cat2(x_up, self.lin(self.upsampling(x_down, up_idx))))


class PointConvResNet(Base):

    def __init__(self, in_channels, n_classes, use_crf=True, steps=1):
        super().__init__()
        self.C = n_classes
        cin = in_channels
        for lvl, width in enumerate(WIDTHS, start=1):
            setattr(self, 'conv%d_1' % lvl, ResNetBBlock(cin, width))
            setattr(self, 'conv%d_2' % lvl, ResNetBBlock(width, width))
            cin = width
        for lvl in range(len(WIDTHS) - 1, 0, -1):
            coarse, fine = WIDTHS[lvl], WIDTHS[lvl - 1]
            stage = CRFConv(coarse, fine, fine, steps=steps) if use_crf else Upsampling(coarse, fine, fine)
            setattr(self, 'deconv%d' % lvl, stage)
        self.classifier = nn.Sequential(MLP(WIDTHS[0], WIDTHS[0] * 4, activation=_lrelu()), nn.Dropout(p=0.5),
                                        nn.Linear(WIDTHS[0] * 4, n_classes))

    phase_hook = None

    def forward(self, data):
        if self.training:
            from .. import train
            if train.autograph_wanted(data):
                out = train.autograph_forward(self, data)
                if out is not None:
                    return out
            with ops.advance_counters(self):
                return self._forward(data)
        return self._forward(data)

    def _forward(self, data):
        ms = data.multiscale
        plan = [(self.conv1_1, ms[0].pos, ms[0].neighbor_idx), (self.conv1_2, ms[0].pos, ms[0].neighbor_idx)]
        for lvl in range(1, len(WIDTHS)):
            fine, coarse = ms[lvl - 1], ms[lvl]
            plan.append((getattr(self, 'conv%d_1' % (lvl + 1)), (fine.pos, coarse.pos), fine.sub_idx))
            plan.append((getattr(self, 'conv%d_2' % (lvl + 1)), coarse.pos, coarse.neighbor_idx))
        decoders = [getattr(self, 'deconv%d' % (lvl + 1)) for lvl in range(len(WIDTHS) - 2, -1, -1)]
        mats = [None] * len(decoders)
        if all(isinstance(d, CRFConv) for d in decoders):
            mats = ops.crf_matrices_batched([d.c for d in decoders], ride=self.training and data.x.is_cuda)
        pre = [None] * len(plan)
        if self.training and data.x.is_cuda and not ops.state.no_prefold:
            pre = ops.point_conv_prefold([blk.point_conv.prefold_entry(p, i) for blk, p, i in plan], True)
        masks = [ops.JoinMask() for _ in plan]
        h = plan[0][0](data.x, plan[0][1], plan[0][2], prefold=pre[0], join_mask=masks[0])
        h = plan[1][0](h, plan[1][1], plan[1][2], prefold=pre[1], join_mask=masks[1], input_mask=masks[0])
        skips = [h]
        for lvl in range(1, len(WIDTHS)):
            if lvl == 2 and self.phase_hook is not None:
                self.phase_hook('coarse')
            (b1, p1, i1), (b2, p2, i2) = plan[2 * lvl], plan[2 * lvl + 1]
            h, skips[-1] = b1(h, p1, i1, return_input_alias=True, prefold=pre[2 * lvl], join_mask=masks[2 * lvl], input_mask=masks[2 * lvl - 1])
            h = b2(h, p2, i2, prefold=pre[2 * lvl + 1], join_mask=masks[2 * lvl + 1] if lvl + 1 < len(WIDTHS) else None,
                   input_mask=masks[2 * lvl])
            skips.append(h)
        ops.flush_riders()
        for d, mat, lvl in zip(decoders, mats, range(len(WIDTHS) - 2, -1, -1)):
            if mat is not None:
                h = d(h, skips[lvl], ms[lvl].up_idx, ms[lvl].neighbor_idx, matrices=mat)
            else:
                h = d(h, skips[lvl], ms[lvl].up_idx, ms[lvl].neighbor_idx)
            if lvl == 2 and self.phase_hook is not None and h.requires_grad:
                h.register_hook(lambda g, f=self.phase_hook: (f('coarse_backward'), None)[1])
        head, drop, last = self.classifier[0], self.classifier[1], self.classifier[2]
        fused = logits = None
        if (self.training and type(drop) is nn.Dropout and not drop.inplace and isinstance(head, MLP) and head.bn is not None
                and head.lin.bias is None and isinstance(head.activation, nn.LeakyReLU) and head.bn.batch_norm.affine
                and h.dtype == torch.float32):
            slope = head.activation.negative_slope
            if type(last) is nn.Linear:
                logits = ops.mlp_dropout_linear(h, head.lin.weight, head.bn.batch_norm, slope, drop.p, last.weight, last.bias)
            if logits is None:
                fused = ops.mlp_block_dropout(h, head.lin.weight, head.bn.batch_norm, slope, drop.p)
        if logits is None:
            h = fused if fused is not None else drop(head(h))
            logits = ops.linear(h, last.weight, last.bias)
        h = logits
        return h.reshape(-1, self.C)
```

crfconv_amd/ops/_base.py:

```python
import ctypes

import torch

from .. import _lib
from ..graph import NeighborTable, ptr, require_gpu, stream_ptr

BN_EPS = 1e-5


def _f32c(t):
    if t.dtype is torch.float32 and t.is_contiguous():
        return t.detach()
    return t.detach().to(torch.float32).contiguous()


def _pad_channels(t, C):
    if t.shape[-1] == C:
        return t
    return torch.nn.functional.pad(t, (0, C - t.shape[-1]))


def _next_supported(c, choices):
    for v in choices:
        if c <= v:
            return v
    raise _lib.CrfConvError('channel count %d exceeds the largest supported (%d)' % (c, choices[-1]))


def _ptr_array(tensors):
    return (ctypes.c_void_p * len(tensors))(*[None if t is None else t.data_ptr() for t in tensors])



_TICKETS = {}
_raw_stream = getattr(torch._C, '_cuda_getCurrentRawStream', None)


def _stream_key(device):
    idx = device.index if isinstance(device, torch.device) else None
    if idx is None:
        dev = torch.device(device)
        idx = dev.index if dev.index is not None else torch.cuda.current_device()
    if torch.cuda.is_current_stream_capturing():
        return idx, 'capture'
    if _raw_stream is not None:
        return idx, int(_raw_stream(idx))
    return idx, int(torch.cuda.current_stream(idx).cuda_stream)


def _stream_buf(table, device, make):
    key = _stream_key(device)
    buf = table.get(key)
    if buf is None:
        buf = table[key] = make()
        if key[1] != 'capture' and (key[0], 'capture') not in table:
            table[(key[0], 'capture')] = make()
    return buf


def _ticket(device):
    return _stream_buf(_TICKETS, device, lambda: torch.zeros(_lib.load().crfconv_ticket_bytes() // 4, dtype=torch.int32, device=device))




def _pc_ticket(device):
    return ptr(_ticket(device))




def _mlp_ticket(device):
    return ptr(_ticket(device))


_sync_ws = {}


def gridsync_ws(dev):
    return _stream_buf(_sync_ws, dev, lambda: torch.zeros(_lib.load().crfconv_gridsync_workspace() // 4, dtype=torch.int32, device=dev))




def fail_word_ptrs(dev):
    want = torch.device(dev).index
    if want is None:
        want = torch.cuda.current_device()
    word = _lib.load().crfconv_gridsync_fail_word()
    keys = [k for k in _sync_ws if k[0] == want]
    first = [k for k in ((want, 'capture'), (want, int(torch.cuda.current_stream(want).cuda_stream))) if k in _sync_ws]
    rest = [k for k in reversed(keys) if k not in first]
    if len(first) + len(rest) > 8:
        import warnings
        warnings.warn('fail_word_ptrs: %d barrier workspaces on device %d, the update guard watches 8 (capture buffer, current stream, '
                      'newest streams); ops.check_gridsync() reads all of them' % (len(first) + len(rest), want))
    return [_sync_ws[k].data_ptr() + 4 * word for k in (first + rest)[:8]]


def check_gridsync(dev=None, reduced_flag=None):
    word = _lib.load().crfconv_gridsync_fail_word()
    bad = []
    want = None if dev is None else torch.device(dev).index
    for table in (_sync_ws,):
        for key, ws in list(table.items()):
            if want is not None and key[0] is not None and key[0] != want:
                continue
            code = int(ws[word].item())
            if code != 0:
                ws.zero_()
                bad.append((key, code))
    remote = False
    if reduced_flag is not None and reduced_flag.numel():
        v = float(reduced_flag.reshape(-1)[0].item())
        remote = not (v == 0.0)
        if remote:
            reduced_flag.zero_()
    if bad or remote:
        state.small_mlp_disabled = True
        where = ('device(s) %s (code 0x%x)' % (sorted({k[0] for k, _ in bad}), bad[0][1])) if bad else 'another rank of the process group'
        raise _lib.CrfConvError('grid barrier timed out on %s: a one-launch kernel could not get all its '
                                'workgroups resident; its outputs were poisoned with NaN.  The one-launch MLP path is now '
                                'disabled for this process (CRFCONV_NO_ONE_LAUNCH_MLP=1 does the same up front).' % where)




def _env_families(name):
    v = __import__('os').environ.get(name)
    if v is None:
        return False
    v = v.strip().lower()
    return True if v in ('', '1', 'all') else frozenset(q.strip() for q in v.split(',') if q.strip())


class _State:
    no_join = False
    no_fork = False
    no_prefold = False
    no_mask_fold = __import__('os').environ.get('CRFCONV_NO_MASK_FOLD') is not None
    no_combine_fold = _env_families('CRFCONV_NO_COMBINE_FOLD')
    small_mlp_disabled = __import__('os').environ.get('CRFCONV_NO_ONE_LAUNCH_MLP') is not None
    small_bwd_one_launch = __import__('os').environ.get('CRFCONV_SMALL_BWD_TWO_LAUNCHES') is None
    dw_hosts_mats = __import__('os').environ.get('CRFCONV_NO_TAIL_RIDERS') is None
    mfma_min_rows = 12288
    mf_block = __import__('os').environ.get('CRFCONV_MF_BLOCK', 'auto')
    mf_block_min_rows = 65536
    mf_block_min_locality = 0.6


state = _State()
```

crfconv_amd/ops/mlp.py:

```python
import ctypes

import torch

from .. import _lib
from ..graph import ptr, require_gpu, stream_ptr
from ._base import _f32c, _mlp_ticket, _ticket, gridsync_ws, state



class JoinMask:
    __slots__ = ('slope', 'folded')

    def __init__(self):
        self.slope = None
        self.folded = False


def _take_mask(mask, ok):
    if mask is None or mask.slope is None or mask.folded or state.no_mask_fold or not ok:
        return None
    mask.folded = True
    return float(mask.slope)


def _bn_args(bn):
    return bn.weight, bn.bias, bn.running_mean, bn.running_var, 0.1 if bn.momentum is None else bn.momentum, bn.eps


def _use_fork(fork, x):
    return bool(fork and x.requires_grad and torch.is_grad_enabled() and not state.no_fork)


def _stream_fwd(x, Wc, gamma, beta, run_mean, run_var, momentum, eps, slope=None, skip=None, fold=None):
    st = stream_ptr()
    if fold is not None:
        m, ci = x.shape
        co = Wc.shape[0]
        y = torch.empty((m, co), dtype=torch.float32, device=x.device)
        nrec = _lib.load().crfconv_linear_forward_stat_records(m)
        rec = torch.empty((nrec, 4, co), dtype=torch.float32, device=x.device)
        _lib.call('crfconv_linear_forward_uv', ctypes.byref(fold[0]), ptr(Wc), m, ci, co, ptr(y), ptr(rec), st)
    elif isinstance(x, tuple):
        xa, xb = x
        m, split = xa.shape
        ci, co = split + xb.shape[1], Wc.shape[0]
        y = torch.empty((m, co), dtype=torch.float32, device=xa.device)
        nrec = _lib.load().crfconv_linear_forward_stat_records(m)
        rec = torch.empty((nrec, 4, co), dtype=torch.float32, device=xa.device)
        _lib.call('crfconv_linear_forward_cat', ptr(xa), ptr(xb), split, ptr(Wc), None, m, ci, co, ptr(y), ptr(rec), st)
    else:
        y, rec = _mfma_matmul(x, Wc, None, False, True)
    m, co = y.shape
    coef = torch.empty(4 * co, dtype=torch.float32, device=y.device)
    g, b = _f32c(gamma), _f32c(beta)
    if slope is None:
        _lib.call('crfconv_bn_coef_from_records', ptr(rec), m, co, ptr(g), ptr(b), ptr(run_mean), ptr(run_var), float(momentum),
                  float(eps), ptr(coef), st)
        return y, coef, None
    out = torch.empty_like(y)
    _lib.call('crfconv_bn_apply_from_records', ptr(rec), rec.shape[0], ptr(y), m, co, ptr(g), ptr(b), ptr(run_mean), ptr(run_var),
              float(momentum), float(eps), ptr(skip), float(slope), ptr(coef), ptr(out), st)
    return y, coef, out


def _dropout_fwd(x, Wc, gamma, beta, run_mean, run_var, momentum, eps, slope, p, seed, counter):
    y, coef, _ = _stream_fwd(x, Wc, gamma, beta, run_mean, run_var, momentum, eps)
    m, co = y.shape
    out = torch.empty_like(y)
    used = torch.empty(1, dtype=torch.int64, device=y.device)
    _lib.call('crfconv_bn_apply_dropout', ptr(y), m, co, ptr(coef), float(slope), float(p), int(seed), ptr(counter), ptr(out),
              ptr(used), stream_ptr())
    return y, coef, out, used


def _stream_bwd(prm, x, W, y, coef, gA, slope, want_dx, adds=False, g_alias=None, mask_slope=None):
    m = y.shape[0]
    co, ci = W.shape
    dev = y.device
    outs, dfr = _mlp_param_outs(prm, W, dev)
    dW, dgamma, dbeta = outs[0][0], outs[1][0], outs[2][0]
    nbytes = _lib.load().crfconv_mlp_backward_workspace(m, ci, co)
    ws = torch.empty(nbytes, dtype=torch.uint8, device=dev)
    tail = (ptr(None if dfr else dW), ptr(dgamma), ptr(dbeta), ptr(ws), nbytes, _mlp_ticket(dev), stream_ptr())
    if isinstance(x, tuple):
        xa, xb = x
        dxs = (torch.empty_like(xa), torch.empty_like(xb)) if want_dx else (None, None)
        _lib.call('crfconv_mlp_backward_cat', ptr(gA), ptr(y), ptr(xa), ptr(xb), xa.shape[1], ptr(W), ptr(coef), slope, m, ci, co,
                  ptr(dxs[0]), ptr(dxs[1]), *tail)
        return (*dxs, *_mlp_param_rets(prm, outs, dfr, ws, m, ci, co, coef))
    dX = torch.empty_like(x) if want_dx else None
    head = (ptr(gA), ptr(y), ptr(x), ptr(W), ptr(coef), slope, m, ci, co)
    if adds or mask_slope is not None:
        add = _f32c(g_alias) if (g_alias is not None and want_dx) else None
        if mask_slope is None:
            _lib.call('crfconv_mlp_backward_add', *head, ptr(add), ptr(dX), *tail)
        elif not want_dx:
            raise _lib.CrfConvError('_MLPBlock: a folded join mask without an input gradient')
        else:
            _lib.call('crfconv_mlp_backward_add_mask', *head, ptr(add), mask_slope, ptr(dX), *tail)
    else:
        _lib.call('crfconv_mlp_backward', *head, ptr(dX), *tail)
    return (dX, *_mlp_param_rets(prm, outs, dfr, ws, m, ci, co, coef))


def _join_g1(ctx, g, out):
    if ctx.mask is not None and ctx.mask.folded:
        return g
    g1 = torch.empty_like(g)
    _lib.call('crfconv_add_lrelu_backward', ptr(g), ptr(out), out.numel(), ctx.slope, ptr(g1), stream_ptr())
    return g1


class _MLPBlock(torch.autograd.Function):

    @staticmethod
    def forward(ctx, x_in, W, gamma, beta, run_mean, run_var, momentum, eps, slope, fork=False, mask=None):
        x = x_in.contiguous()
        Wc = W.contiguous()
        ci, co = x.shape[1], Wc.shape[0]
        ctx.mask_slope = _take_mask(mask, fork and ci % 4 == 0 and co % 4 == 0)
        y, coef, out = _stream_fwd(x, Wc, gamma, beta, run_mean, run_var, momentum, eps, slope)
        ctx.prm = (W, gamma, beta)
        ctx.save_for_backward(x, Wc, y, coef)
        ctx.slope = float(slope)
        if fork:
            ctx.set_materialize_grads(False)
            return out, x_in
        return out

    @staticmethod
    def backward(ctx, gA, g_alias=None):
        x, W, y, coef = ctx.saved_tensors
        gA = torch.zeros_like(y) if gA is None else gA.contiguous()
        return (*_stream_bwd(ctx.prm, x, W, y, coef, gA, ctx.slope, ctx.needs_input_grad[0], True, g_alias, ctx.mask_slope),
                None, None, None, None, None, None, None)


class _MLPBlockJoin(torch.autograd.Function):

    @staticmethod
    def forward(ctx, x, W, gamma, beta, run_mean, run_var, momentum, eps, skip, slope, mask=None, fold=None):
        x, Wc, skip = x.contiguous(), W.contiguous(), skip.contiguous()
        ctx.mask = mask
        y, coef, out = _stream_fwd(x, Wc, gamma, beta, run_mean, run_var, momentum, eps, slope, skip, fold)
        ctx.prm = (W, gamma, beta)
        ctx.save_for_backward(x, Wc, y, coef, out)
        ctx.slope = float(slope)
        return out

    @staticmethod
    def backward(ctx, g):
        x, W, y, coef, out = ctx.saved_tensors
        g1 = _join_g1(ctx, g.contiguous(), out)
        gskip = g1 if ctx.needs_input_grad[8] else None
        return (*_stream_bwd(ctx.prm, x, W, y, coef, g1, 1.0, ctx.needs_input_grad[0]), None, None, None, None, gskip, None, None, None)


class _MLPBlockDropout(torch.autograd.Function):

    @staticmethod
    def forward(ctx, x, W, gamma, beta, run_mean, run_var, momentum, eps, slope, p, seed, counter):
        x, Wc = x.contiguous(), W.contiguous()
        y, coef, out, used = _dropout_fwd(x, Wc, gamma, beta, run_mean, run_var, momentum, eps, slope, p, seed, counter)
        ctx.prm = (W, gamma, beta)
        ctx.save_for_backward(x, Wc, y, coef, used)
        ctx.slope, ctx.p, ctx.seed = float(slope), float(p), int(seed)
        return out

    @staticmethod
    def backward(ctx, g):
        x, W, y, coef, counter = ctx.saved_tensors
        g = g.contiguous()
        gA = torch.empty_like(g)
        _lib.call('crfconv_dropout_backward', ptr(g), g.numel(), ctx.p, ctx.seed, ptr(counter), ptr(gA), stream_ptr())
        return (*_stream_bwd(ctx.prm, x, W, y, coef, gA, ctx.slope, ctx.needs_input_grad[0]), None, None, None, None, None, None, None, None)


class _MLPDropoutLinear(torch.autograd.Function):

    @staticmethod
    def forward(ctx, x, W, gamma, beta, run_mean, run_var, momentum, eps, slope, p, seed, counter, W2, b2):
        x, Wc, W2c = x.contiguous(), W.contiguous(), W2.contiguous()
        y, coef, h, used = _dropout_fwd(x, Wc, gamma, beta, run_mean, run_var, momentum, eps, slope, p, seed, counter)
        logits = _mfma_matmul(h, W2c, None if b2 is None else b2.contiguous(), False)[0]
        ctx.prm = (W, gamma, beta)
        ctx.save_for_backward(x, Wc, y, coef, used, h, W2c)
        ctx.slope, ctx.p, ctx.seed = float(slope), float(p), int(seed)
        ctx.params2 = (W2, b2)
        return logits

    @staticmethod
    def backward(ctx, g):
        x, W, y, coef, counter, h, W2 = ctx.saved_tensors
        m = x.shape[0]
        co, c2 = W.shape[0], W2.shape[0]
        g = g.contiguous()
        gA = torch.empty((m, co), dtype=torch.float32, device=x.device)
        _lib.call('crfconv_linear_forward_dropout', ptr(g), ptr(W2), m, c2, co, 1, ctx.p, ctx.seed, ptr(counter), ptr(gA), stream_ptr())
        dW2, db2 = _weight_grad(g, h, ctx.params2, ctx.params2[1] is not None)
        return (*_stream_bwd(ctx.prm, x, W, y, coef, gA, ctx.slope, ctx.needs_input_grad[0]), None, None, None, None, None, None, None, None,
                dW2, db2)


class _HeadRecompute(torch.autograd.Function):

    @staticmethod
    def forward(ctx, x, W, gamma, beta, run_mean, run_var, momentum, eps, slope, p, seed, counter, W2, b2):
        x, Wc, W2c = x.contiguous(), W.contiguous(), W2.contiguous()
        m, ci = x.shape
        co, c2 = Wc.shape[0], W2c.shape[0]
        dev = x.device
        lib = _lib.load()
        st = stream_ptr()
        nrec = lib.crfconv_head_stat_records(m)
        rec = torch.empty((nrec, co, 4), dtype=torch.float32, device=dev)
        _lib.call('crfconv_head_stats', ptr(x), ptr(Wc), m, ci, co, ptr(rec), st)
        coef = torch.empty(4 * co, dtype=torch.float32, device=dev)
        _lib.call('crfconv_bn_coef_from_nrecords', ptr(rec), nrec, m, co, ptr(_f32c(gamma)), ptr(_f32c(beta)), ptr(run_mean),
                  ptr(run_var), float(momentum), float(eps), ptr(coef), st)
        logits = torch.empty((m, c2), dtype=torch.float32, device=dev)
        mask = torch.empty(lib.crfconv_head_mask_words(m), dtype=torch.int32, device=dev)
        b2c = None if b2 is None else b2.contiguous()
        _lib.call('crfconv_head_forward', ptr(x), ptr(Wc), ptr(coef), float(slope), float(p), int(seed), ptr(counter), ptr(W2c),
                  ptr(b2c), m, ci, co, c2, ptr(logits), ptr(mask), None, st)
        ctx.prm = (W, gamma, beta, W2, b2)
        ctx.save_for_backward(x, Wc, coef, mask, W2c)
        ctx.slope, ctx.p = float(slope), float(p)
        return logits

    @staticmethod
    def backward(ctx, g):
        x, W, coef, mask, W2 = ctx.saved_tensors
        m, ci = x.shape
        co, c2 = W.shape[0], W2.shape[0]
        dev = x.device
        g = g.contiguous()
        Wp, gp, bp, W2p, b2p = ctx.prm
        outs = [_param_out(Wp, (co, ci), dev), _param_out(gp, (co,), dev), _param_out(bp, (co,), dev), _param_out(W2p, (c2, co), dev)]
        ob2 = _param_out(b2p, (c2,), dev) if b2p is not None else (None, False)
        dX = torch.empty_like(x) if ctx.needs_input_grad[0] else None
        nbytes = _lib.load().crfconv_head_backward_workspace(m, ci, co, c2)
        ws = torch.empty(nbytes, dtype=torch.uint8, device=dev)
        _lib.call('crfconv_head_backward', ptr(g), ptr(x), ptr(W), ptr(coef), ctx.slope, ctx.p, ptr(W2), ptr(mask), m, ci, co, c2,
                  ptr(dX), ptr(outs[0][0]), ptr(outs[1][0]), ptr(outs[2][0]), ptr(outs[3][0]), ptr(ob2[0]), ptr(ws), nbytes, stream_ptr())
        rets = [_param_ret(prm, o[0], o[1]) for prm, o in zip((Wp, gp, bp, W2p), outs)]
        rb2 = _param_ret(b2p, ob2[0], ob2[1]) if b2p is not None else None
        return dX, rets[0], rets[1], rets[2], None, None, None, None, None, None, None, None, rets[3], rb2


def dropout_seed(ci, co):
    return (torch.initial_seed() * 0x9E3779B97F4A7C15 + co * 7919 + ci) & 0xFFFFFFFFFFFFFFFF


def dropout_keep_mask(seed, counter, n, p):
    import numpy as np
    t = float(p) * 4294967296.0
    thr = np.uint32(0xffffffff if t >= 4294967295.0 else (0 if t <= 0.0 else int(t)))
    mask64 = 0xFFFFFFFFFFFFFFFF
    z = (int(seed) + 0x9E3779B97F4A7C15 * (int(counter) + 1)) & mask64
    z = ((z ^ (z >> 30)) * 0xBF58476D1CE4E5B9) & mask64
    z = ((z ^ (z >> 27)) * 0x94D049BB133111EB) & mask64
    z ^= z >> 31
    k0, k1 = np.uint32(z & 0xFFFFFFFF), np.uint32(z >> 32)
    with np.errstate(over='ignore'):
        e = np.arange(int(n), dtype=np.uint64)
        hi = (e >> np.uint64(32)).astype(np.uint32)
        x = e.astype(np.uint32) + k0 + ((hi << np.uint32(13)) | (hi >> np.uint32(19)))
        x ^= x >> np.uint32(16)
        x *= np.uint32(0x7feb352d)
        x ^= x >> np.uint32(15)
        x += k1
        x *= np.uint32(0x846ca68b)
        x ^= x >> np.uint32(16)
    return x >= thr


def mlp_dropout_linear(x, W, bn, slope, p, W2, b2, recompute=None):
    if not (0.0 <= p < 1.0) or bn.num_batches_tracked is None:
        return None
    m = x.numel() // x.shape[-1]
    ci, co, c2 = x.shape[-1], W.shape[0], W2.shape[0]
    if not (mlp_block_ok(x, W, None, bn, True) and not _mlp_small_ok(m, ci, co) and _mfma_ok(m, co, c2) and _mfma_ok(m, c2, co)
            and W2.dtype == torch.float32):
        return None
    require_gpu(x, W, W2)
    tick(bn)
    seed = dropout_seed(ci, co)
    node = _MLPDropoutLinear
    head_ok = bool(_lib.load().crfconv_head_supported(m, ci, co, c2))
    if recompute and not head_ok:
        return None
    if head_ok and (recompute or recompute is None):
        node = _HeadRecompute
    out = node.apply(x.reshape(-1, ci), W, *_bn_args(bn), slope, p, seed, bn.num_batches_tracked, W2, b2)
    return out.reshape(x.shape[:-1] + (c2,))


def mlp_block_dropout(x, W, bn, slope, p):
    if not (0.0 <= p < 1.0) or bn.num_batches_tracked is None:
        return None
    m = x.numel() // x.shape[-1]
    ci, co = x.shape[-1], W.shape[0]
    if not mlp_block_ok(x, W, None, bn, True):
        return None
    if _mlp_small_ok(m, ci, co):
        lib = _lib.load()
        if not (co % 4 == 0 and lib.crfconv_linear_forward_supported(ci, co) and lib.crfconv_mlp_backward_supported(m, ci, co) == 1):
            return None
# ... 15 lines not shown
        arg = torch.empty((table.m_tgt, co), dtype=torch.int32, device=x.device)
        _lib.call('crfconv_neighbor_maxpool_affine_forward', ptr(y), ptr(coef), ptr(table.idx32), table.K, table.m_tgt, co,
                  ptr(out), ptr(arg), stream_ptr())
        ctx.table = table
        ctx.prm = (W, gamma, beta)
        ctx.save_for_backward(x, Wc, y, coef, arg)
        if fork:
            ctx.set_materialize_grads(False)
            return out, x_in
        return out

    @staticmethod
    def backward(ctx, g, g_alias=None):
        x, W, y, coef, arg = ctx.saved_tensors
        table = ctx.table
        m, co = y.shape
        dev = x.device
        g = torch.zeros((table.m_tgt, co), dtype=torch.float32, device=dev) if g is None else _f32c(g)
        rev_ptr, rev_eid = table.reverse
        gA = torch.empty((m, co), dtype=torch.float32, device=dev)
        _lib.call('crfconv_neighbor_maxpool_backward', ptr(g), ptr(arg), ptr(rev_ptr), ptr(rev_eid), table.K, m, co, ptr(gA), stream_ptr())
        return (*_stream_bwd(ctx.prm, x, W, y, coef, gA, 1.0, ctx.needs_input_grad[0], True, g_alias), None, None, None, None, None, None)


def mlp_block_pool(x, W, bn, table, fork=False):
    if state.no_join or table.padded:
        return None
    m, ci = x.shape
    co = W.shape[0]
    if m != table.m_src or not (mlp_block_ok(x, W, None, bn, True) and not _mlp_small_ok(m, ci, co)):
        return None
    require_gpu(x, W)
    tick(bn)
    if _use_fork(fork, x):
        return _MLPBlockPool.apply(x, W, *_bn_args(bn), table, True)
    out = _MLPBlockPool.apply(x, W, *_bn_args(bn), table, False)
    return (out, x) if fork else out

def _small_bwd_jobs(jobs, n, dev, st):
    if state.small_bwd_one_launch and not state.small_mlp_disabled:
        _lib.call('crfconv_mlp_small_backward_jobs_one_launch', ctypes.cast(jobs, ctypes.c_void_p), n, ptr(_ticket(dev)), ptr(gridsync_ws(dev)), st)
    else:
        _lib.call('crfconv_mlp_small_backward_jobs', ctypes.cast(jobs, ctypes.c_void_p), n, ptr(_ticket(dev)), st)


def _mlp_bwd_jobs(blocks):
    jobs = (_lib.MlpBwdJob * len(blocks))()
    for i, (gA, y, coef, W, add, slope, gY, dX, dgamma, dbeta, ws, mask) in enumerate(blocks):
        m, co = y.shape
        mref, mslope = (None, 1.0) if mask is None else (mask[0].data_ptr(), float(mask[1]))
        jobs[i] = _lib.MlpBwdJob(gA.data_ptr(), y.data_ptr(), coef.data_ptr(), W.data_ptr(), None if add is None else add.data_ptr(), m,
                                 W.shape[1], co, 1, float(slope), gY.data_ptr(), dX.data_ptr(), dgamma.data_ptr(), dbeta.data_ptr(),
                                 ws.data_ptr(), ws.numel(), mref, mslope)
    return jobs


def _small_bwd(gA, y, coef, W, addend, slope, dgamma, dbeta, need_dx, mask=None):
    m, co = y.shape
    ci = W.shape[1]
    dev = y.device
    gY = torch.empty_like(y)
    lib = _lib.load()
    if need_dx and lib.crfconv_mlp_small_backward_supported(m, ci, co) == 1:
        dX = torch.empty((m, ci), dtype=torch.float32, device=dev)
        nbytes = lib.crfconv_mlp_small_backward_workspace(m, co)
        ws = torch.empty(nbytes, dtype=torch.uint8, device=dev)
        add = None if addend is None else addend.contiguous()
        jobs = _mlp_bwd_jobs([(gA, y, coef, W, add, slope, gY, dX, dgamma, dbeta, ws, mask)])
        _small_bwd_jobs(jobs, 1, dev, stream_ptr())
        return gY, dX
    if mask is not None:
        raise _lib.CrfConvError('_small_bwd: a folded join mask needs the fused dX product (%d x %d -> %d)' % (m, ci, co))
    nbytes = lib.crfconv_bn_workspace(m, co)
    ws = torch.empty(nbytes, dtype=torch.uint8, device=dev)
    _lib.call('crfconv_bn_backward', ptr(gA), ptr(y), ptr(coef), m, co, 1, float(slope), ptr(gY), ptr(dgamma), ptr(dbeta), ptr(ws),
              nbytes, stream_ptr())
    return gY, (_gemm(gY, W, addend=addend) if need_dx else None)


def _small_fwd(x, Wc, gamma, beta, run_mean, run_var, momentum, eps, slope, skip=None, join_slope=1.0, fold=None):
    m, ci = x.shape
    co = Wc.shape[0]
    dev = x.device
    lib = _lib.load()
    y = torch.empty((m, co), dtype=torch.float32, device=dev)
    out = torch.empty_like(y)
    coef = torch.empty(4 * co, dtype=torch.float32, device=dev)
    g, b = _f32c(gamma), _f32c(beta)
    if not state.small_mlp_disabled and lib.crfconv_mlp_small_supported(m, ci, co) == 1:
        nbytes = lib.crfconv_mlp_small_workspace(m, co)
        ws = torch.empty(nbytes, dtype=torch.uint8, device=dev)
        sync = gridsync_ws(dev)
        if fold is not None:
            _lib.call('crfconv_mlp_small_forward_join_uv', ctypes.byref(fold[0]), ptr(Wc), m, ci, co, ptr(g), ptr(b), ptr(run_mean),
                      ptr(run_var), float(momentum), float(eps), float(slope), ptr(skip), float(join_slope), ptr(y), ptr(out), ptr(coef),
                      ptr(ws), nbytes, ptr(sync), sync.numel() * 4, stream_ptr())
        elif skip is None:
            _lib.call('crfconv_mlp_small_forward', ptr(x), ptr(Wc), m, ci, co, ptr(g), ptr(b), ptr(run_mean), ptr(run_var),
                      float(momentum), float(eps), float(slope), ptr(y), ptr(out), ptr(coef), ptr(ws), nbytes, ptr(sync),
                      sync.numel() * 4, stream_ptr())
        else:
            _lib.call('crfconv_mlp_small_forward_join', ptr(x), ptr(Wc), m, ci, co, ptr(g), ptr(b), ptr(run_mean), ptr(run_var),
                      float(momentum), float(eps), float(slope), ptr(skip), float(join_slope), ptr(y), ptr(out), ptr(coef), ptr(ws),
                      nbytes, ptr(sync), sync.numel() * 4, stream_ptr())
        return y, out, coef
    nrec = lib.crfconv_gemm_stat_records(m)
    rec = torch.empty((nrec, co, 4), dtype=torch.float32, device=dev)
    if fold is not None:
        _lib.call('crfconv_gemm_stats_uv', ctypes.byref(fold[0]), ptr(Wc), m, co, ci, ptr(y), ptr(rec), stream_ptr())
    else:
        _lib.call('crfconv_gemm_stats', ptr(x), ptr(Wc), m, co, ci, ptr(y), ptr(rec), stream_ptr())
    _lib.call('crfconv_bn_apply_from_records', ptr(rec), nrec, ptr(y), m, co, ptr(g), ptr(b), ptr(run_mean), ptr(run_var),
              float(momentum), float(eps), ptr(skip), float(slope if skip is None else join_slope), ptr(coef), ptr(out), stream_ptr())
    return y, out, coef


def _small_tail(ctx, x, W, y, coef, gA, addend, slope, mask=None):
    outs = [_param_out(q, (W.shape[0],), x.device) for q in ctx.prm[1:]]
    gY, dX = _small_bwd(gA, y, coef, W, addend, slope, outs[0][0], outs[1][0], ctx.needs_input_grad[0], mask)
    dW = _weight_grad(gY, x, ctx.params, False)[0]
    return (dX, dW, *(_param_ret(q, o, k) for q, (o, k) in zip(ctx.prm[1:], outs)))


class _MLPSmallJoin(torch.autograd.Function):

    @staticmethod
    def forward(ctx, x, W, gamma, beta, run_mean, run_var, momentum, eps, skip, slope, mask=None, fold=None):
        x, Wc, skip = x.contiguous(), W.contiguous(), skip.contiguous()
        ctx.mask = mask
        y, out, coef = _small_fwd(x, Wc, gamma, beta, run_mean, run_var, momentum, eps, 1.0, skip, slope, fold)
        ctx.prm = (W, gamma, beta)
        ctx.save_for_backward(x, Wc, y, coef, out)
        ctx.slope = float(slope)
        ctx.params = (W, None)
        return out

    @staticmethod
    def backward(ctx, g):
        x, W, y, coef, out = ctx.saved_tensors
        g1 = _join_g1(ctx, g.contiguous(), out)
        gskip = g1 if ctx.needs_input_grad[8] else None
        return (*_small_tail(ctx, x, W, y, coef, g1, None, 1.0), None, None, None, None, gskip, None, None, None)


def _join_fold_family(small, m, ci, co):
    lib = _lib.load()
    if not small:
        return 'fine' if lib.crfconv_linear_forward_uv_supported(ci, co) == 1 else None
    if not state.small_mlp_disabled and lib.crfconv_mlp_small_supported(m, ci, co) == 1:
        return 'small' if lib.crfconv_mlp_small_forward_uv_supported(ci) == 1 else None
    return 'tiled' if lib.crfconv_gemm_stats_uv_supported(m, co, ci) == 1 else None


def mlp_block_join(x, W, bn, skip, slope, mask=None, combine=None):
    if state.no_join or skip.shape[:-1] != x.shape[:-1] or skip.shape[-1] != W.shape[0] or skip.dtype != torch.float32:
        return None
    m = x.numel() // x.shape[-1]
    ci, co = x.shape[-1], W.shape[0]
    if not mlp_block_ok(x, W, None, bn, True):
        return None
    require_gpu(x, W, skip)
    tick(bn)
    small = _mlp_small_ok(m, ci, co)
    fn = _MLPSmallJoin if small else _MLPBlockJoin
    fold = None
    if combine is not None and combine.pending:
        family = _join_fold_family(small, m, ci, co) if combine.feeds(x.reshape(-1, ci)) else None
        if family is not None and not combine.fold_off(family):
            fold = combine.take()
        else:
            combine.flush()
    if mask is not None and not state.no_mask_fold and torch.is_grad_enabled():
        mask.slope = float(slope)
    else:
        mask = None
    out = fn.apply(x.reshape(-1, ci), W, *_bn_args(bn), skip.reshape(-1, co), slope, mask, fold)
    return out.reshape(x.shape[:-1] + (co,))


def _mlp_small_ok(m, ci, co):
    if m >= state.mfma_min_rows:
        return False
    lib = _lib.load()
    if not state.small_mlp_disabled and lib.crfconv_mlp_small_supported(m, ci, co) == 1:
        return True
    return ci % 4 == 0 and co % 4 == 0 and lib.crfconv_mlp_small_backward_supported(m, ci, co) == 1


class _MLPSmall(torch.autograd.Function):

    @staticmethod
    def forward(ctx, x_in, W, gamma, beta, run_mean, run_var, momentum, eps, slope, fork=False, mask=None):
        x = x_in.contiguous()
        Wc = W.contiguous()
        ctx.mask_slope = _take_mask(mask, fork and _lib.load().crfconv_mlp_small_backward_supported(x.shape[0], x.shape[1], Wc.shape[0]) == 1)
        y, out, coef = _small_fwd(x, Wc, gamma, beta, run_mean, run_var, momentum, eps, slope)
        ctx.prm = (W, gamma, beta)
        ctx.save_for_backward(x, Wc, y, coef)
        ctx.slope = float(slope)
        ctx.params = (W, None)
        if fork:
            ctx.set_materialize_grads(False)
            return out, x_in
        return out

    @staticmethod
    def backward(ctx, gA, g_alias=None):
        x, W, y, coef = ctx.saved_tensors
        gA = torch.zeros_like(y) if gA is None else gA.contiguous()
        return (*_small_tail(ctx, x, W, y, coef, gA, None if g_alias is None else g_alias.reshape(x.shape), ctx.slope,
                             None if ctx.mask_slope is None else (x, ctx.mask_slope)), None, None, None, None, None, None, None)


class _MLPSmallGroup(torch.autograd.Function):

    NARG = 10

    @staticmethod
    def forward(ctx, shared, mask, *args):
        n = len(args) // _MLPSmallGroup.NARG
        jobs = [args[i * _MLPSmallGroup.NARG:(i + 1) * _MLPSmallGroup.NARG] for i in range(n)]
        lib = _lib.load()
        st = stream_ptr()
        keep, outs, prm, slopes, forks, tmp = [], [], [], [], [], []
        gs = (_lib.GemmStatsJob * n)()
        ba = (_lib.BnApplyJob * n)()
        for i, (x_in, W, gamma, beta, rm, rv, mom, eps, slope, fork) in enumerate(jobs):
            if x_in is None:
                x_in = jobs[0][0]
            x, Wc = x_in.contiguous(), W.contiguous()
            m, ci = x.shape
            co = Wc.shape[0]
            dev = x.device
            y = torch.empty((m, co), dtype=torch.float32, device=dev)
            out = torch.empty_like(y)
            coef = torch.empty(4 * co, dtype=torch.float32, device=dev)
            nrec = lib.crfconv_gemm_stat_records(m)
            rec = torch.empty((nrec, co, 4), dtype=torch.float32, device=dev)
            g, b = _f32c(gamma), _f32c(beta)
            gs[i] = _lib.GemmStatsJob(x.data_ptr(), Wc.data_ptr(), m, co, ci, y.data_ptr(), rec.data_ptr())
            ba[i] = _lib.BnApplyJob(rec.data_ptr(), nrec, y.data_ptr(), m, co, g.data_ptr(), b.data_ptr(),
                                    None if rm is None else rm.data_ptr(), None if rv is None else rv.data_ptr(), float(mom), float(eps),
                                    None, float(slope), coef.data_ptr(), out.data_ptr())
            keep += [x, Wc, y, coef]
            prm.append((W, gamma, beta))
            slopes.append(float(slope))
            forks.append(bool(fork))
            outs.append(out)
            if fork:
                outs.append(x_in)
            tmp.append((rec, g, b))
        _lib.call('crfconv_gemm_stats_jobs', ctypes.cast(gs, ctypes.c_void_p), n, st)
        _lib.call('crfconv_bn_apply_from_records_jobs', ctypes.cast(ba, ctypes.c_void_p), n, st)
        del tmp
        ctx.n, ctx.prm, ctx.slopes, ctx.forks, ctx.shared = n, prm, slopes, forks, bool(shared)
        ctx.mask_slope = _take_mask(mask, bool(shared) and n >= 2 and forks[0] and ctx.needs_input_grad[2])
        ctx.save_for_backward(*keep)
        ctx.set_materialize_grads(False)
        return tuple(outs)

    @staticmethod
    def backward(ctx, *grads):
        n = ctx.n
        saved = ctx.saved_tensors
        lib = _lib.load()
        st = stream_ptr()
        per, gi = [], 0
        for i in range(n):
            x, W, y, coef = saved[4 * i:4 * i + 4]
            m, ci = x.shape
            co = W.shape[0]
            dev = x.device
            gA = grads[gi]
            gi += 1
            g_alias = None
            if ctx.forks[i]:
                g_alias = grads[gi]
                gi += 1
            gA = torch.zeros_like(y) if gA is None else gA.contiguous()
            need_dx = ctx.needs_input_grad[2 + (0 if (ctx.shared and i == 1) else i) * _MLPSmallGroup.NARG]
            outs = [_param_out(q, (co,), dev) for q in ctx.prm[i][1:]]
            gY = torch.empty_like(y)
            dX = torch.empty((m, ci), dtype=torch.float32, device=dev)
            nbytes = lib.crfconv_mlp_small_backward_workspace(m, co)
            ws = torch.empty(nbytes, dtype=torch.uint8, device=dev)
            add = None if g_alias is None else _f32c(g_alias).reshape(m, ci)
            per.append((x, W, gY, dX, outs, need_dx, (gA, y, coef, W, add, ctx.slopes[i], gY, dX, outs[0][0], outs[1][0], ws, None)))
        _small_bwd_jobs(_mlp_bwd_jobs([p[6] for p in per]), n, per[0][0].device, st)
        rets = [None, None]
        dxs = [p[3] if p[5] else None for p in per]
        if ctx.shared and dxs[0] is not None and dxs[1] is not None:
            tot = torch.empty_like(dxs[0])
            if ctx.mask_slope is not None:
                _lib.call('crfconv_add_mask', ptr(dxs[0]), ptr(dxs[1]), ptr(saved[0]), tot.numel(), ctx.mask_slope, ptr(tot), st)
            else:
                _lib.call('crfconv_add_lrelu', ptr(dxs[0]), ptr(dxs[1]), tot.numel(), 1.0, ptr(tot), st)
            dxs[0], dxs[1] = tot, None
        elif ctx.mask_slope is not None:
            raise _lib.CrfConvError('_MLPSmallGroup: a folded join mask without both input gradients')
        for i, (x, W, gY, dX, outs, need_dx, _) in enumerate(per):
            Wp, gp, bp = ctx.prm[i]
            dW = _weight_grad(gY, x, (Wp, None), False)[0]
            rets += [dxs[i], dW, _param_ret(gp, outs[0][0], outs[0][1]), _param_ret(bp, outs[1][0], outs[1][1]), None, None, None, None, None, None]
        return tuple(rets)


def mlp_group(blocks, shared=False, input_mask=None):
    if not (2 <= len(blocks) <= 4):
        return None
    lib = _lib.load()
    args, shapes = [], []
    for x, W, bn, slope, fork in blocks:
        ci, co = x.shape[-1], W.shape[0]
        m = x.numel() // max(ci, 1)
        if not (x.is_cuda and x.dtype == torch.float32 and W.dtype == torch.float32 and bn.affine and bn.running_mean is not None
                and m >= 1 and _mlp_small_ok(m, ci, co) and ci % 4 == 0 and co % 4 == 0
                and lib.crfconv_mlp_small_backward_supported(m, ci, co) == 1):
            return None
    if shared and (state.no_fork or blocks[0][0] is not blocks[1][0]):
        return None
    for i, (x, W, bn, slope, fork) in enumerate(blocks):
        tick(bn)
        use_fork = _use_fork(fork, x)
        xa = None if (shared and i == 1) else x.reshape(-1, x.shape[-1])
        args += [xa, W, *_bn_args(bn), float(slope), use_fork]
        shapes.append((x.shape, W.shape[0], fork, use_fork))
    fold = input_mask if (shared and len(blocks) == 2 and args[9]) else None
    res = list(_MLPSmallGroup.apply(bool(shared), fold, *args))
    out = []
    for (xs, co, fork, use_fork), (x, _, _, _, _) in zip(shapes, blocks):
        o = res.pop(0).reshape(xs[:-1] + (co,))
        if fork:
            alias = res.pop(0).reshape(xs) if use_fork else x
            out.append((o, alias))
        else:
            out.append(o)
    return out


class _MLPBlockCat(torch.autograd.Function):

    @staticmethod
    def forward(ctx, xa, xb, W, gamma, beta, run_mean, run_var, momentum, eps, slope):
        xa, xb, Wc = xa.contiguous(), xb.contiguous(), W.contiguous()
        y, coef, out = _stream_fwd((xa, xb), Wc, gamma, beta, run_mean, run_var, momentum, eps, slope)
        ctx.prm = (W, gamma, beta)
        ctx.save_for_backward(xa, xb, Wc, y, coef)
        ctx.slope = float(slope)
        return out

    @staticmethod
    def backward(ctx, gA):
        xa, xb, W, y, coef = ctx.saved_tensors
        want_a, want_b = ctx.needs_input_grad[:2]
        dxa, dxb, *rets = _stream_bwd(ctx.prm, (xa, xb), W, y, coef, gA.contiguous(), ctx.slope, want_a or want_b)
        return (dxa if want_a else None, dxb if want_b else None, *rets, None, None, None, None, None)


class _Cat2(torch.autograd.Function):

    @staticmethod
    def forward(ctx, xa, xb):
        xa, xb = xa.contiguous(), xb.contiguous()
        m, ca = xa.shape
        cb = xb.shape[1]
        out = torch.empty((m, ca + cb), dtype=torch.float32, device=xa.device)
        _lib.call('crfconv_cat2', ptr(xa), ptr(xb), m, ca, cb, ptr(out), stream_ptr())
        ctx.widths = (ca, cb)
        return out

    @staticmethod
    def backward(ctx, g):
        ca, cb = ctx.widths
        g = g.contiguous()
        m = g.shape[0]
        ga = torch.empty((m, ca), dtype=torch.float32, device=g.device)
        gb = torch.empty((m, cb), dtype=torch.float32, device=g.device)
        _lib.call('crfconv_split2', ptr(g), m, ca, cb, ptr(ga), ptr(gb), stream_ptr())
        return ga, gb


def cat2(xa, xb):
    ca, cb = xa.shape[-1], xb.shape[-1]
    if not (xa.is_cuda and xb.is_cuda and xa.dtype == torch.float32 and xb.dtype == torch.float32
            and xa.shape[:-1] == xb.shape[:-1] and ca % 4 == 0 and cb % 4 == 0 and ca >= 4 and cb >= 4 and xa.numel() > 0):
        return torch.cat([xa, xb], dim=-1)
    out = _Cat2.apply(xa.reshape(-1, ca), xb.reshape(-1, cb))
    return out.reshape(xa.shape[:-1] + (ca + cb,))


def mlp_block_cat(xa, xb, W, bn, training, slope=1.0):
    if xa.dim() != xb.dim() or xa.shape[:-1] != xb.shape[:-1]:
        return None
    ca, cb = xa.shape[-1], xb.shape[-1]
    m = xa.numel() // ca
    probe = xa.new_empty((1, ca + cb))
    if not (ca % 4 == 0 and cb % 4 == 0 and xb.dtype == torch.float32 and m >= state.mfma_min_rows
            and mlp_block_ok(probe.expand(m, ca + cb), W, None, bn, training)):
        return None
    require_gpu(xa, xb, W)
    tick(bn)
    out = _MLPBlockCat.apply(xa.reshape(-1, ca), xb.reshape(-1, cb), W, *_bn_args(bn), slope)
    return out.reshape(xa.shape[:-1] + (W.shape[0],))


def mlp_block_ok(x, W, bias, bn, training):
    if not training or bias is not None or x.dtype != torch.float32 or not bn.affine:
        return False
    m = x.numel() // x.shape[-1]
    ci, co = x.shape[-1], W.shape[0]
    if bn.running_mean is None:
        return False
    if _mlp_small_ok(m, ci, co):
        return True
    return (_mfma_ok(m, ci, co) and co % 4 == 0
            and _lib.load().crfconv_mlp_backward_supported(m, ci, co) == 1)


def mlp_block(x, W, bn, slope=1.0, fork=False, input_mask=None):
    require_gpu(x, W)
    shape = x.shape
    tick(bn)
    x2 = x.reshape(-1, shape[-1])
    fn = _MLPSmall if _mlp_small_ok(x2.shape[0], shape[-1], W.shape[0]) else _MLPBlock
    if _use_fork(fork, x2):
        out, alias = fn.apply(x2, W, *_bn_args(bn), slope, True, input_mask)
        return out.reshape(shape[:-1] + (W.shape[0],)), alias.reshape(shape)
    out = fn.apply(x2, W, *_bn_args(bn), slope, False, None)
    out = out.reshape(shape[:-1] + (W.shape[0],))
    return (out, x) if fork else out


def run_lin_bn(seq, x):
    mods = list(seq)
    i = 0
    while i < len(mods):
        lin = mods[i]
        if not isinstance(lin, torch.nn.Linear):
            raise _lib.CrfConvError('run_lin_bn: expected a Linear at position %d, got %s' % (i, type(lin).__name__))
        bn = mods[i + 1] if i + 1 < len(mods) and isinstance(mods[i + 1], torch.nn.BatchNorm1d) else None
        j = i + 1 + (bn is not None)
        act = mods[j] if j < len(mods) and isinstance(mods[j], torch.nn.LeakyReLU) else None
        slope = act.negative_slope if act is not None else 1.0
        co = lin.out_features
        if bn is not None and co % 4 == 0 and co <= 1024 and bn.affine and x.dtype == torch.float32:
            if mlp_block_ok(x, lin.weight, lin.bias, bn, seq.training):
                x = mlp_block(x, lin.weight, bn, slope)
            else:
                records = None
                if seq.training:
                    x, records = linear(x, lin.weight, lin.bias, want_stats=True)
                else:
                    x = linear(x, lin.weight, lin.bias)
                x = bn_act(x, bn, seq.training, slope, records=records)
        else:
            x = linear(x, lin.weight, lin.bias)
            if bn is not None:
                if not bn.affine:
                    raise _lib.CrfConvError('run_lin_bn: affine BatchNorm only (csrc/bn.hip)')
                x = bn_act(x, bn, seq.training, slope)
            elif act is not None:
                x = _LRelu.apply(x, slope)
        i = j + (act is not None)
    return x


from .rows import _LRelu
from .defer import _mlp_param_outs, _mlp_param_rets, _param_out, _param_ret
from .dense import _gemm, _mfma_matmul, _mfma_ok, _weight_grad, bn_act, linear, tick
```

include/crfconv_amd.h:

```cpp
#ifndef CRFCONV_AMD_H
#define CRFCONV_AMD_H

#include <stddef.h>
#include <stdint.h>

#ifdef __cplusplus
extern "C" {
#endif

typedef void* crf_stream_t;

enum {
    CRF_OK = 0,
    CRF_ERR_ARG = -1,
    CRF_ERR_HIP = -2,
    CRF_ERR_UNSUPPORTED = -3,
    CRF_ERR_WORKSPACE = -4
};

#define CRFCONV_ABI_VERSION 1
int crfconv_abi_version(void);
const char* crfconv_last_error(void);


// ... 174 lines not shown
typedef struct { const float* gw; const float* h1; const float* rel; int64_t n_edges; int d; float slope; void* workspace;
                 size_t workspace_bytes; } crf_pc_a1_job;
int crfconv_pointconv_bwd_dump_jobs(const crf_pc_dump_job* jobs, int njobs, crf_stream_t stream);
typedef struct { const float* x; const float* gout; const float* pos_src; const float* pos_tgt; const int32_t* idx32; int K; int64_t m_tgt;
                 int d; const float* A1; const float* b1; const float* W2; float slope; const float* ca; const float* cb; const float* cc;
                 float* dw2_partial; double* a1_partial; } crf_pc_wide_job;
int crfconv_pointconv_wide_params_supported(int64_t m_tgt, int K, int d);
int64_t crfconv_pointconv_wide_params_nblk(int64_t m_tgt, int d);
int crfconv_pointconv_wide_params_jobs(const crf_pc_wide_job* jobs, int njobs, crf_stream_t stream);
int crfconv_pointconv_bwd_a1_jobs(const crf_pc_a1_job* jobs, int njobs, crf_stream_t stream);
typedef struct { const void* partial; int is_float; int64_t nblk; int nslots; double* out; } crf_reduce64_job;
int crfconv_pointconv_bwd_params_slabs(void* workspace, int64_t m_tgt, int d, const float** slab_w2, const double** slab_a1,
                                       int64_t* nblk_out);
int64_t crfconv_pointconv_bwd_a1_nblk(int64_t n_edges, int d);
int crfconv_reduce_jobs_f64(const crf_reduce64_job* jobs, int njobs, crf_stream_t stream);
int crfconv_pointconv_bwd_input(const float* gout, const float* pos_src, const float* pos_tgt,
                                const int32_t* rev_ptr, const int32_t* rev_eid, int K,
                                int64_t m_src, int d, const float* A1, const float* b1,
                                const float* W2, float slope, const float* a2, const float* b2, float* dx,
                                crf_stream_t stream);
int crfconv_pointconv_bwd_input_reduce(const float* gout, const float* pos_src, const float* pos_tgt, const int32_t* rev_ptr,
                                       const int32_t* rev_eid, int K, int64_t m_src, int64_t m_tgt, int d, const float* A1, const float* b1,
                                       const float* W2, float slope, const float* a2, const float* b2, float* dx, const float* U,
                                       const float* V, const float* shift, const double* aux2, const float* gamma2, double n_edges,
                                       int use_batch, float* ca, float* cb, float* cc, float* dgamma2, float* dbeta2, void* workspace,
                                       size_t workspace_bytes, unsigned* ticket, crf_stream_t stream);

int crfconv_pointconv_fold1(const float* W1, const float* gamma1, const float* beta1, const double* mom,
                            double n_edges, float* run_mean, float* run_var, float momentum, float eps,
                            int use_batch, int d, float* A1, float* b1, double* aux1, crf_stream_t stream);
int crfconv_pointconv_fold1_bwd(const float* W1, const float* gamma1, const double* mom, const double* aux1,
                                const double* dA1b1, float eps, int use_batch, int d, float* dW1,
                                float* dgamma1, float* dbeta1, const double* dW2_f64, float* dW2_f32, crf_stream_t stream);
typedef struct {
    const float* W1; const float* gamma1; const float* beta1; const double* mom; double n_edges;
    float* run_mean; float* run_var; float momentum; float eps; int32_t use_batch; int32_t d;
    float* A1; float* b1; double* aux1;
} crf_fold1_job;
int crfconv_pointconv_fold1_batched(const crf_fold1_job* jobs, int njobs, crf_stream_t stream);
typedef struct {
    const float* W1; const float* gamma1; const double* mom; const double* aux1; const double* dA1b1;
    float eps; int32_t use_batch; int32_t d; int32_t pad_;
    float* dW1; float* dgamma1; float* dbeta1; const double* dW2_f64; float* dW2_f32;
} crf_fold1_bwd_job;
int crfconv_pointconv_fold1_bwd_batched(const crf_fold1_bwd_job* jobs, int njobs, crf_stream_t stream);
int crfconv_pointconv_fold2(const double* stats, const float* shift, const float* gamma2, const float* beta2,
                            double n_edges, float* run_mean, float* run_var, float momentum, float eps,
                            int use_batch, int d, float* a2, float* b2, double* aux2, crf_stream_t stream);
int crfconv_pointconv_fold2_bwd(const double* red, const float* shift, const double* aux2, const float* gamma2,
                                double n_edges, int use_batch, int d, float* ca, float* cb, float* cc,
                                float* dgamma2, float* dbeta2, crf_stream_t stream);

size_t crfconv_linear_wgrad_workspace(int64_t M, int Co, int Ci);
int crfconv_linear_wgrad(const float* G, const float* X, int64_t M, int Co, int Ci, float* dW, float* db,
                         void* workspace, size_t workspace_bytes, crf_stream_t stream);
typedef struct { const float* partial; float* out; int32_t nblk; int32_t nslots; } crf_reduce_job;
int crfconv_linear_wgrad_partial(const float* G, const float* X, int64_t M, int Co, int Ci, int want_bias,
                                 void* workspace, size_t workspace_bytes, int* nblk_out, crf_stream_t stream);
typedef struct { const float* G; const float* X; int64_t M; int Co; int Ci; int want_bias; void* workspace; size_t workspace_bytes; } crf_wgrad_job;
int crfconv_linear_wgrad_nblk(int64_t M, int Co, int Ci);
int crfconv_linear_wgrad_partial_jobs(const crf_wgrad_job* jobs, int njobs, crf_stream_t stream);
int crfconv_reduce_jobs(const crf_reduce_job* jobs, int njobs, crf_stream_t stream);
int crfconv_reduce_jobs_both(const crf_reduce_job* jobs, int njobs, const crf_reduce64_job* jobs64, int njobs64, crf_stream_t stream);

size_t crfconv_gridsync_workspace(void);
int crfconv_gridsync_fail_word(void);
int crfconv_mlp_small_supported(int64_t M, int Ci, int Co);
size_t crfconv_mlp_small_workspace(int64_t M, int Co);
int crfconv_mlp_small_forward(const float* X, const float* W, int64_t M, int Ci, int Co, const float* gamma,
                              const float* beta, float* run_mean, float* run_var, float momentum, float eps, float slope,
                              float* Y, float* A, float* coef, void* workspace, size_t workspace_bytes, void* sync_ws,
                              size_t sync_bytes, crf_stream_t stream);

int crfconv_mlp_small_forward_join(const float* X, const float* W, int64_t M, int Ci, int Co, const float* gamma,
                                   const float* beta, float* run_mean, float* run_var, float momentum, float eps, float slope,
                                   const float* skip, float join_slope, float* Y, float* A, float* coef, void* workspace,
                                   size_t workspace_bytes, void* sync_ws, size_t sync_bytes, crf_stream_t stream);
int crfconv_mlp_small_forward_uv_supported(int Ci);
int crfconv_mlp_small_forward_join_uv(const crf_uv_fold* f, const float* W, int64_t M, int Ci, int Co, const float* gamma,
                                      const float* beta, float* run_mean, float* run_var, float momentum, float eps, float slope,
                                      const float* skip, float join_slope, float* Y, float* A, float* coef, void* ws, size_t ws_bytes,
                                      void* sync_ws, size_t sync_bytes, crf_stream_t stream);

size_t crfconv_ticket_bytes(void);
int crfconv_mlp_backward_supported(int64_t M, int Ci, int Co);
size_t crfconv_mlp_backward_workspace(int64_t M, int Ci, int Co);
int crfconv_mlp_backward(const float* gA, const float* Y, const float* X, const float* W, const float* coef, float slope,
                         int64_t M, int Ci, int Co, float* dX, float* dW, float* dgamma, float* dbeta, void* workspace,
                         size_t workspace_bytes, unsigned* ticket, crf_stream_t stream);
typedef struct { const void* workspace; const float* coef; float* dW; int64_t M; int32_t Ci; int32_t Co; } crf_mlp_dw_job;
int crfconv_mlp_dw_jobs(const crf_mlp_dw_job* jobs, int njobs, crf_stream_t stream);
int crfconv_mlp_dw_jobs_hosting(const crf_mlp_dw_job* jobs, int njobs, const float* const* c, const float* const* Q,
                                const float* const* gQ, const float* const* gP, const int* H, int n, float* const* dc,
                                crf_stream_t stream);
int crfconv_mlp_backward_add(const float* gA, const float* Y, const float* X, const float* W, const float* coef, float slope,
                             int64_t M, int Ci, int Co, const float* dX_add, float* dX, float* dW, float* dgamma, float* dbeta,
                             void* workspace, size_t workspace_bytes, unsigned* ticket, crf_stream_t stream);
int crfconv_mlp_backward_add_mask(const float* gA, const float* Y, const float* X, const float* W, const float* coef, float slope,
                                  int64_t M, int Ci, int Co, const float* dX_add, float mask_slope, float* dX, float* dW,
                                  float* dgamma, float* dbeta, void* workspace, size_t workspace_bytes, unsigned* ticket,
                                  crf_stream_t stream);
int crfconv_linear_forward_cat(const float* Xa, const float* Xb, int split, const float* W, const float* bias, int64_t M,
                               int Ci, int Co, float* Y, float* stat_rec, crf_stream_t stream);
int crfconv_linear_bn_act(const float* X, const float* Xb, int split, const float* W, const float* bias, const float* coef,
                          const float* skip, float slope, int64_t M, int Ci, int Co, float* Y, crf_stream_t stream);
int crfconv_gemm_bn_act(const float* A, const float* B, const float* bias, const float* coef, const float* skip, float slope,
                        int64_t M, int N, int K, int b_is_nk, float* C, crf_stream_t stream);
typedef struct { const float* gamma; const float* beta; const float* run_mean; const float* run_var; float eps; int C; float* coef;
} crf_bn_coef_job;
int crfconv_bn_eval_coef_jobs(const crf_bn_coef_job* jobs, int njobs, crf_stream_t stream);
int crfconv_linear_forward_uv_supported(int Ci, int Co);
int crfconv_linear_forward_uv(const crf_uv_fold* f, const float* W, int64_t M, int Ci, int Co, float* Y, float* stat_rec,
                              crf_stream_t stream);
int crfconv_mlp_backward_cat(const float* gA, const float* Y, const float* Xa, const float* Xb, int split, const float* W,
                             const float* coef, float slope, int64_t M, int Ci, int Co, float* dXa, float* dXb, float* dW,
                             float* dgamma, float* dbeta, void* workspace, size_t workspace_bytes, unsigned* ticket,
                             crf_stream_t stream);

size_t crfconv_bn_workspace(int64_t M, int C);
int crfconv_bn_forward(const float* x, int64_t M, int C, const float* gamma, const float* beta, float* run_mean,
                       float* run_var, float momentum, float eps, int use_batch_stats, float slope, float* coef,
                       float* y, void* workspace, size_t workspace_bytes, crf_stream_t stream);
int crfconv_bn_backward(const float* gy, const float* x, const float* coef, int64_t M, int C, int training,
                        float slope, float* gx, float* dgamma, float* dbeta, void* workspace,
                        size_t workspace_bytes, crf_stream_t stream);

int crfconv_bn_apply(const float* x, int64_t M, int C, const float* coef, float slope, float* y, crf_stream_t stream);

int crfconv_linear_forward_supported(int Ci, int Co);
size_t crfconv_linear_forward_stat_records(int64_t M);
int crfconv_linear_forward(const float* X, const float* W, const float* bias, int64_t M, int Ci, int Co,
                           int transpose_w, float* Y, float* stat_rec, crf_stream_t stream);
int crfconv_cat2(const float* xa, const float* xb, int64_t m, int ca, int cb, float* out, crf_stream_t stream);
int crfconv_split2(const float* g, int64_t m, int ca, int cb, float* ga, float* gb, crf_stream_t stream);
int crfconv_add_i64(int64_t* x, int64_t n, int64_t delta, crf_stream_t stream);
int crfconv_gate_mark(uint64_t* gate, crf_stream_t stream);
int crfconv_gate_wait(uint64_t* gate, int max_wait_us, crf_stream_t stream);

int crfconv_mlp_small_backward_supported(int64_t M, int Ci, int Co);
size_t crfconv_mlp_small_backward_workspace(int64_t M, int Co);
int crfconv_mlp_small_backward(const float* gA, const float* Y, const float* coef, const float* W, const float* addend, int64_t M,
                               int Ci, int Co, int training, float slope, float* gY, float* dX, float* dgamma, float* dbeta,
                               void* workspace, size_t workspace_bytes, unsigned* ticket, crf_stream_t stream);
size_t crfconv_gemm_stat_records(int64_t M);
int crfconv_gemm_stats(const float* A, const float* B, int64_t M, int N, int K, float* C, float* stat_rec, crf_stream_t stream);
int crfconv_gemm_stats_uv_supported(int64_t M, int N, int K);
int crfconv_gemm_stats_uv(const crf_uv_fold* f, const float* B, int64_t M, int N, int K, float* C, float* stat_rec, crf_stream_t stream);
typedef struct { const float* A; const float* B; int64_t M; int N; int K; float* C; float* stat_rec; } crf_gemm_stats_job;
int crfconv_gemm_stats_jobs(const crf_gemm_stats_job* jobs, int njobs, crf_stream_t stream);
typedef struct { const float* stat_rec; int64_t nrec; const float* x; int64_t M; int C; const float* gamma; const float* beta;
                 float* run_mean; float* run_var; float momentum; float eps; const float* skip; float slope; float* coef; float* y;
} crf_bn_apply_job;
int crfconv_bn_apply_from_records_jobs(const crf_bn_apply_job* jobs, int njobs, crf_stream_t stream);
typedef struct { const float* gA; const float* Y; const float* coef; const float* W; const float* addend; int64_t M; int Ci; int Co;
                 int training; float slope; float* gY; float* dX; float* dgamma; float* dbeta; void* workspace; size_t workspace_bytes;
                 const float* mask_ref; float mask_slope;
} crf_mlp_bwd_job;
int crfconv_mlp_small_backward_jobs(const crf_mlp_bwd_job* jobs, int njobs, unsigned* ticket, crf_stream_t stream);
int crfconv_mlp_small_backward_jobs_one_launch(const crf_mlp_bwd_job* jobs, int njobs, unsigned* ticket, unsigned* sync_ws,
                                               crf_stream_t stream);
typedef struct { const float* A; const float* B; float* C; int64_t M; int N; int K; } crf_gemm_job;
int crfconv_gemm_jobs(const crf_gemm_job* jobs, int njobs, crf_stream_t stream);
int crfconv_gemm_supported(int64_t M, int N, int K);
int crfconv_gemm(const float* A, const float* B, const float* bias, const float* addend, int64_t M, int N, int K,
                 int b_is_nk, float* C, crf_stream_t stream);
int crfconv_bn_coef_from_records(const float* stat_rec, int64_t M, int C, const float* gamma, const float* beta,
                                 float* run_mean, float* run_var, float momentum, float eps, float* coef,
                                 crf_stream_t stream);
int crfconv_bn_apply_from_records(const float* stat_rec, int64_t nrec, const float* x, int64_t M, int C, const float* gamma,
                                  const float* beta, float* run_mean, float* run_var, float momentum, float eps, const float* skip,
                                  float slope, float* coef, float* y, crf_stream_t stream);
int crfconv_bn_coef_from_nrecords(const float* stat_rec, int64_t nrec, int64_t M, int C, const float* gamma, const float* beta,
                                  float* run_mean, float* run_var, float momentum, float eps, float* coef, crf_stream_t stream);

int crfconv_spd_inverse(const float* M, int H, float* Q, crf_stream_t stream);
int crfconv_spd_inverse_wide(const float* M, int H, float* Q, crf_stream_t stream);
int crfconv_crf_matrices(const float* c, int H, float* Q, float* P, crf_stream_t stream);
int crfconv_crf_matrices_backward(const float* c, const float* Q, const float* dQ, const float* dP, int H,
                                  float* dc, crf_stream_t stream);
int crfconv_crf_matrices_batched(const float* const* c, const int* H, int n, float* const* Q, float* const* P,
                                 crf_stream_t stream);
int crfconv_crf_matrices_backward_batched(const float* const* c, const float* const* Q, const float* const* gQ,
                                          const float* const* gP, const int* H, int n, float* const* dc,
                                          crf_stream_t stream);

int crfconv_neighbor_maxpool_forward(const float* x, const int32_t* idx32, int K, int64_t m_tgt,
                                     int C, float* out, int32_t* arg, crf_stream_t stream);
int crfconv_neighbor_maxpool_affine_forward(const float* x, const float* coef, const int32_t* idx32, int K, int64_t m_tgt,
                                            int C, float* out, int32_t* arg, crf_stream_t stream);
int crfconv_neighbor_maxpool_backward(const float* gout, const int32_t* arg,
                                      const int32_t* rev_ptr, const int32_t* rev_eid, int K,
                                      int64_t m_src, int C, float* dx, crf_stream_t stream);
int crfconv_gather_rows(const float* x, const int32_t* idx32, int64_t m_tgt, int C, float* out,
                        crf_stream_t stream);
int crfconv_gather_rows_backward(const float* gout, const int32_t* rev_ptr,
                                 const int32_t* rev_eid, int64_t m_src, int C, float* dx,
                                 crf_stream_t stream);

int crfconv_add_lrelu(const float* a, const float* b, int64_t n, float slope, float* out, crf_stream_t stream);
int crfconv_bn_apply_dropout(const float* x, int64_t M, int C, const float* coef, float slope, float p, uint64_t seed,
                             const int64_t* counter, float* out, int64_t* counter_used, crf_stream_t stream);
int crfconv_dropout_backward(const float* g, int64_t n, float p, uint64_t seed, const int64_t* counter, float* gin,
                             crf_stream_t stream);
int crfconv_linear_forward_dropout(const float* X, const float* W, int64_t M, int Ci, int Co, int transpose_w, float p,
                                   uint64_t seed, const int64_t* counter, float* Y, crf_stream_t stream);
int crfconv_head_supported(int64_t M, int Ci, int Co, int C2);
size_t crfconv_head_mask_words(int64_t M);
size_t crfconv_head_stat_records(int64_t M);
int crfconv_head_stats(const float* X, const float* W1, int64_t M, int Ci, int Co, float* stat_rec, crf_stream_t stream);
size_t crfconv_head_backward_workspace(int64_t M, int Ci, int Co, int C2);
int crfconv_head_forward(const float* X, const float* W1, const float* coef, float slope, float p, uint64_t seed,
                         const int64_t* counter, const float* W2, const float* b2, int64_t M, int Ci, int Co, int C2,
                         float* logits, uint32_t* mask_bits, int64_t* counter_used, crf_stream_t stream);
int crfconv_head_backward(const float* g, const float* X, const float* W1, const float* coef, float slope, float p,
                          const float* W2, const uint32_t* mask_bits, int64_t M, int Ci, int Co, int C2, float* dX, float* dW1,
                          float* dgamma, float* dbeta, float* dW2, float* db2, void* workspace, size_t workspace_bytes,
                          crf_stream_t stream);
int crfconv_bn_apply_add(const float* x, int64_t M, int C, const float* coef, const float* skip, float slope, float* out,
                         crf_stream_t stream);
int crfconv_add_lrelu_backward(const float* gout, const float* out, int64_t n, float slope, float* gin,
                               crf_stream_t stream);
int crfconv_add_mask(const float* a, const float* b, const float* ref, int64_t n, float slope, float* gin, crf_stream_t stream);

size_t crfconv_softmax_ce_workspace(int64_t m);
int crfconv_softmax_ce_forward(const float* logits, const int64_t* target, const float* weight, int64_t m, int C,
                               int64_t ignore_index, int64_t label_shift, float* lse, double* sums, float* loss,
                               void* workspace, size_t workspace_bytes, unsigned* ticket, crf_stream_t stream);
int crfconv_softmax_ce_backward(const float* logits, const int64_t* target, const float* weight, const float* lse,
                                const double* sums, const float* grad_loss, int64_t m, int C, int64_t ignore_index,
                                int64_t label_shift, float* dlogits, crf_stream_t stream);

int crfconv_sgd_step(float* param, const float* grad, float* momentum_buf, int64_t n, float lr, float momentum,
                     float dampening, float weight_decay, int nesterov, int first_step, crf_stream_t stream);
int crfconv_sgd_step_hyper(float* param, const float* grad, float* momentum_buf, int64_t n, const float* hyper,
                           int nesterov, int first_step, crf_stream_t stream);
int crfconv_sgd_step_guarded(float* param, const float* grad, float* momentum_buf, int64_t n, const float* hyper,
                             int nesterov, int first_step, const unsigned* fail_word, crf_stream_t stream);
int crfconv_sgd_step_guarded_all(float* param, const float* grad, float* momentum_buf, int64_t n, const float* hyper,
                                 int nesterov, int first_step, const unsigned* const* fail_words, int n_fail_words,
                                 const float* reduced_flag, crf_stream_t stream);
int crfconv_sgd_guard_publish(const unsigned* const* fail_words, int n_fail_words, float* slot, crf_stream_t stream);

size_t crfconv_adam_workspace(int64_t n);
size_t crfconv_adam_coef_floats(void);
int crfconv_adam_step(float* param, const float* grad, float* exp_avg, float* exp_avg_sq, float* max_exp_avg_sq, int64_t n,
                      const double* hyper, long long* t, float* coef, float* grad_norm, int decoupled, int clip, void* workspace,
                      size_t workspace_bytes, const unsigned* const* fail_words, int n_fail_words, const float* reduced_flag,
                      crf_stream_t stream);

int crfconv_random_subsets(const int* n, const int* s, int64_t* const* out, int32_t* const* rank, int nlevels, uint64_t seed,
                           const int64_t* counter, crf_stream_t stream);
size_t crfconv_upindex_workspace(int64_t B, int64_t N);
int crfconv_upindex_from_table(const float* pos, const float* sub_pos, const int64_t* neighbor_idx, const int32_t* rank, int64_t B, int64_t N,
                               int K, int64_t S, int64_t* up_idx, void* workspace, size_t workspace_bytes, crf_stream_t stream);
int crfconv_gather_rows_batched(const void* const* src, void* const* dst, const int* row_bytes, int njobs, const int64_t* index,
                                int per_cloud, int64_t B, int64_t N, int64_t S, crf_stream_t stream);
size_t crfconv_argsort_codes_workspace(int64_t B, int64_t N);
int crfconv_argsort_codes(const int64_t* code, int64_t B, int64_t N, int64_t* order, void* workspace,
                          size_t workspace_bytes, crf_stream_t stream);

int crfconv_meanfield_step(const float* xin, const float* z, const float* s, const int32_t* idx32, int K, int k0,
                           int64_t m, int H, const float* Q, const float* P, float* xout, crf_stream_t stream);

int crfconv_kernel_weights_forward(const float* fk, const int32_t* idx32, int K, const float* Wg, int G, int H,
                                   int64_t m, float* w, crf_stream_t stream);
size_t crfconv_kernel_weights_partials(int64_t m);
int crfconv_kernel_weights_backward(const float* gw, const float* fk, const int32_t* idx32, const int32_t* rev_ptr,
                                    const int32_t* rev_eid, int K, const float* Wg, int G, int H, int64_t m,
                                    float* dfk_self, float* dfk, double* dW_partial, crf_stream_t stream);

int crfconv_confusion_accumulate(const int64_t* y_true, const int64_t* y_pred, const float* logits, int64_t n_rows,
                                 int n_class, int64_t ignore_index, int64_t label_shift, int64_t* hist,
                                 int32_t* bad_count, crf_stream_t stream);

int crfconv_vote_accumulate(const float* probs, const float* logits, const int64_t* point_idx, int64_t n_rows, int C,
                            double smooth, float* test_probs, int64_t n_cloud, int32_t* bad_count, crf_stream_t stream);
int crfconv_vote_accumulate_counted(const float* probs, const float* logits, const int64_t* point_idx, int64_t n_rows, int C, double smooth,
                                    float* test_probs, int64_t n_cloud, int32_t* bad_count, int32_t* visits, crf_stream_t stream);
int crfconv_vote_fold(float* acc, int32_t* acc_visits, const float* later, const int32_t* later_visits, int64_t n, int C, double smooth,
                      crf_stream_t stream);

int crfconv_vote_project(const float* test_probs, const int64_t* proj_idx, int64_t n_proj, int C, int64_t n_cloud,
                         int label_offset, uint8_t* preds, int32_t* bad_count, crf_stream_t stream);

size_t crfconv_argmin_workspace(void);
int crfconv_argmin_f64(const double* values, int64_t n, double* out_value, int64_t* out_index, void* workspace,
                       size_t workspace_bytes, crf_stream_t stream);

size_t crfconv_possibility_crop_workspace(int64_t n, int64_t k);
int crfconv_possibility_crop(const float* points, int64_t n, int64_t k, const int64_t* pick_index, const double* noise,
                             const int64_t* perm, const double* point_weight, double* possibility, int64_t* out_idx,
                             float* out_xyz, double* out_center, void* workspace, size_t workspace_bytes,
                             crf_stream_t stream);

typedef struct crf_augment_spec {
    int32_t rotate_axis;
    float deg_lo, deg_hi;
    int32_t scale;
    float scale_lo, scale_span;
    int32_t flip_axes;
    int32_t noise;
    float sigma, clip;
    int32_t drop;
    float drop_p;
} crf_augment_spec;
size_t crfconv_augment_workspace(int64_t B, int64_t N);
// ... 50 lines not shown
```

Baseline: 45.66 M points/s.

## Fold deferred join BN-apply into next block's linear forward prologue

```diff
diff --git a/crfconv_amd/_lib.py b/crfconv_amd/_lib.py
--- a/crfconv_amd/_lib.py
+++ b/crfconv_amd/_lib.py
@@ -93,6 +93,8 @@
     'crfconv_linear_forward_cat': (_i, [_vp, _vp, _i, _vp, _vp, _i64, _i, _i, _vp, _vp, _vp]),
     'crfconv_linear_forward_uv_supported': (_i, [_i, _i]),
     'crfconv_linear_forward_uv': (_i, [_vp, _vp, _i64, _i, _i, _vp, _vp, _vp]),
+    'crfconv_linear_forward_apply_supported': (_i, [_i, _i]),
+    'crfconv_linear_forward_apply': (_i, [_vp, _vp, _i64, _i, _i, _vp, _vp, _vp]),
     'crfconv_mlp_small_forward_uv_supported': (_i, [_i]),
     'crfconv_mlp_small_forward_join_uv': (_i, [_vp, _vp, _i64, _i, _i, _vp, _vp, _vp, _vp, _f, _f, _f, _vp, _f, _vp, _vp, _vp, _vp, _sz, _vp, _sz, _vp]),
     'crfconv_gemm_stats_uv_supported': (_i, [_i64, _i, _i]),
diff --git a/crfconv_amd/csrc/apply_fold.hpp b/crfconv_amd/csrc/apply_fold.hpp
--- /dev/null
+++ b/crfconv_amd/csrc/apply_fold.hpp
@@ -0,0 +1,22 @@
+#pragma once
+
+#include "common.hpp"
+
+namespace crf {
+
+__device__ __forceinline__ float4 apply_affine4(const float4 a, const float4 b, const float4 y) {
+    return make_float4(fmaf(a.x, y.x, b.x), fmaf(a.y, y.y, b.y), fmaf(a.z, y.z, b.z), fmaf(a.w, y.w, b.w));
+}
+__device__ __forceinline__ float4 apply_skip4(float4 o, const float4 k) {
+    o.x = add_rn(o.x, k.x); o.y = add_rn(o.y, k.y); o.z = add_rn(o.z, k.z); o.w = add_rn(o.w, k.w);
+    return o;
+}
+__device__ __forceinline__ float4 apply_lrelu4(float4 o, const float slope) {
+    o.x = o.x > 0.f ? o.x : slope * o.x;
+    o.y = o.y > 0.f ? o.y : slope * o.y;
+    o.z = o.z > 0.f ? o.z : slope * o.z;
+    o.w = o.w > 0.f ? o.w : slope * o.w;
+    return o;
+}
+
+}
diff --git a/crfconv_amd/csrc/linear.hip b/crfconv_amd/csrc/linear.hip
--- a/crfconv_amd/csrc/linear.hip
+++ b/crfconv_amd/csrc/linear.hip
@@ -4,6 +4,7 @@
 #include "crf_matrices_body.hpp"
 #include "reduce64_body.hpp"
 #include "uv_fold.hpp"
+#include "apply_fold.hpp"
 
 #include <cstdlib>
 
@@ -775,7 +776,7 @@
 #endif
 constexpr int LF_BLOCK = LF_BLOCK_, LF_WAVES = LF_BLOCK / WAVE;
 
-constexpr int EPI_NONE = 0, EPI_ADD = 1, EPI_DROPOUT = 2, EPI_ADD_MASK = 3, EPI_UV = 4, EPI_BN_ACT = 5;
+constexpr int EPI_NONE = 0, EPI_ADD = 1, EPI_DROPOUT = 2, EPI_ADD_MASK = 3, EPI_UV = 4, EPI_BN_ACT = 5, EPI_APPLY = 6;
 #ifndef LF_PF_MAX_
 #define LF_PF_MAX_ 4
 #endif
@@ -793,19 +794,27 @@
                                                               unsigned long long drop_seed = 0ull, unsigned drop_threshold = 0u,
                                                               float drop_scale = 1.f,
                                                               const float* __restrict__ mask_ref = nullptr, float mask_slope = 1.f,
-                                                              const UvFold uv = UvFold()) {
+                                                              const UvFold uv = UvFold(),
+                                                              float* __restrict__ apply_out = nullptr) {
     static_assert(EPI != EPI_ADD_MASK || (PRO && VEC4), "the masked epilogue is the aligned dX product's");
     static_assert(EPI != EPI_UV || (!PRO && VEC4 && NCH == 1), "the combine prologue is the narrow aligned forward's");
     static_assert(EPI != EPI_BN_ACT || !PRO, "the BatchNorm epilogue is the forward product's");
-    constexpr bool UV = EPI == EPI_UV, TWO = PRO || UV;
+    static_assert(EPI != EPI_APPLY || (!PRO && VEC4 && NCH > 0), "the apply prologue is the aligned forward's hoisted loop");
+    constexpr bool UV = EPI == EPI_UV, APL = EPI == EPI_APPLY, TWO = PRO || UV || APL;
     constexpr bool BNA = EPI == EPI_BN_ACT;
     extern __shared__ float sW[];
     const int Cip = ((Ci + 15) / 16) * 16 + 4;
     const int Cik = ((Ci + 15) / 16) * 16;
     float* sPro = sW + 16 * TCO * Cip;
-    [[maybe_unused]] float* sTile = sPro + (PRO ? 5 * Cik : 0);
+    [[maybe_unused]] float* sTile = sPro + (PRO ? 5 * Cik : (APL ? 2 * Cik : 0));
     if constexpr (PRO) {
         for (int t = threadIdx.x; t < 5 * Cik; t += LF_BLOCK) {
+            const int which = t / Cik, k = t - which * Cik;
+            sPro[t] = k < Ci ? pro[which * Ci + k] : 0.f;
+        }
+    }
+    if constexpr (APL) {
+        for (int t = threadIdx.x; t < 2 * Cik; t += LF_BLOCK) {
             const int which = t / Cik, k = t - which * Cik;
             sPro[t] = k < Ci ? pro[which * Ci + k] : 0.f;
         }
@@ -887,6 +896,9 @@
         } else if constexpr (UV) {
             xa = *reinterpret_cast<const float4*>(X + r * Ci + k0);
             xb2 = *reinterpret_cast<const float4*>(uv.V + r * Ci + k0);
+        } else if constexpr (APL) {
+            xa = *reinterpret_cast<const float4*>(X + r * Ci + k0);
+            if (addend != nullptr) xb2 = *reinterpret_cast<const float4*>(addend + r * Ci + k0);
         } else if (Xb != nullptr) {
             if (k0 < xsplit) xa = *reinterpret_cast<const float4*>(X + r * xsplit + k0);
             else xa = *reinterpret_cast<const float4*>(Xb + r * (Ci - xsplit) + (k0 - xsplit));
@@ -942,6 +954,15 @@
         if (blockIdx.y == 0) *reinterpret_cast<float4*>(uv.out + r * Ci + 4 * g) = o;
         return o;
     };
+    [[maybe_unused]] auto apl_operand = [&](int64_t r, bool rv, int c, float4 y, float4 k) -> float4 {
+        const int k0 = 16 * c + 4 * g;
+        if (!rv || k0 >= Ci) return zero4;
+        float4 o = apply_affine4(*reinterpret_cast<const float4*>(sPro + k0), *reinterpret_cast<const float4*>(sPro + Cik + k0), y);
+        if (addend != nullptr) o = apply_skip4(o, k);
+        o = apply_lrelu4(o, slope);
+        if (blockIdx.y == 0) *reinterpret_cast<float4*>(apply_out + r * Ci + k0) = o;
+        return o;
+    };
     constexpr int NCA = NCH > 0 ? NCH : 1;
     constexpr bool PF = NCH > 0 && NCH <= LF_PF_MAX_;
     const int64_t row_stride = (int64_t)gridDim.x * (LF_BLOCK / WAVE) * 16;
@@ -976,6 +997,7 @@
                 const int k0 = 16 * c + 4 * g;
                 float4 xv;
                 if constexpr (UV) xv = uv_operand(r, rv, fa[c], fb[c]);
+                else if constexpr (APL) xv = apl_operand(r, rv, c, fa[c], fb[c]);
                 else xv = operand(rv, c, fa[c], fb[PRO ? c : 0]);
 #pragma unroll
                 for (int t = 0; t < TCO; ++t) {
@@ -1304,14 +1326,9 @@
         for (int u = 0; u < 4; ++u) {
             const int64_t r = rb + (int64_t)u * (FR_BLOCK / 4);
             if (r >= r1) continue;
-            float4 o = make_float4(fmaf(a.x, v[u].x, b.x), fmaf(a.y, v[u].y, b.y), fmaf(a.z, v[u].z, b.z), fmaf(a.w, v[u].w, b.w));
-            if constexpr (ADD) {
-                o.x = add_rn(o.x, k[u].x); o.y = add_rn(o.y, k[u].y); o.z = add_rn(o.z, k[u].z); o.w = add_rn(o.w, k[u].w);
-            }
-            o.x = o.x > 0.f ? o.x : slope * o.x;
-            o.y = o.y > 0.f ? o.y : slope * o.y;
-            o.z = o.z > 0.f ? o.z : slope * o.z;
-            o.w = o.w > 0.f ? o.w : slope * o.w;
+            float4 o = apply_affine4(a, b, v[u]);
+            if constexpr (ADD) o = apply_skip4(o, k[u]);
+            o = apply_lrelu4(o, slope);
             *reinterpret_cast<float4*>(y + r * C + c) = o;
         }
     }
@@ -1362,12 +1379,13 @@
 
 }
 
-static size_t lf_lds_bytes_at(int Ci, int tco, bool pro) {
+static size_t lf_lds_bytes_at(int Ci, int tco, bool pro, bool apply = false) {
     const size_t cip = (size_t)((Ci + 15) / 16) * 16 + 4, cik = cip - 4;
     size_t floats = 16 * (size_t)tco * cip;
     const size_t stats = (size_t)crf::LF_WAVES * 4 * 16 * (size_t)tco;
     if (floats < stats) floats = stats;
     if (pro) floats += 5 * cik;
+    if (apply) floats += 2 * cik;
     if (tco >= 2) floats += (size_t)crf::LF_WAVES * 16 * (16 * (size_t)tco + 4);
     return sizeof(float) * floats;
 }
@@ -1492,6 +1510,42 @@
     if (tco == 2) LFU(2);
     else LFU(4);
 #undef LFU
+    CRF_LAUNCH_CHECK();
+    return CRF_OK;
+}
+
+extern "C" int crfconv_linear_forward_apply_supported(int Ci, int Co) {
+    if (Ci < 4 || Co < 4 || Ci % 4 != 0 || Co % 4 != 0 || Ci > 128) return 0;
+    const int tco = lf_tco(Ci, Co, false);
+    return (tco <= 4 && lf_lds_bytes_at(Ci, tco, false, true) <= 64 * 1024) ? 1 : 0;
+}
+
+extern "C" int crfconv_linear_forward_apply(const crf_bn_apply_job* p, const float* W, int64_t M, int Ci, int Co, float* Y,
+                                            float* stat_rec, crf_stream_t stream) {
+    CRF_REQUIRE(p && W && Y, CRF_ERR_ARG, "null pointer");
+    CRF_REQUIRE(p->stat_rec && p->x && p->gamma && p->beta && p->coef && p->y, CRF_ERR_ARG, "apply record: null pointer");
+    CRF_REQUIRE(M > 0 && p->M == M && p->C == Ci, CRF_ERR_ARG, "apply record: [%lld, %d] is not the operand [%lld, %d]", (long long)p->M,
+                p->C, (long long)M, Ci);
+    CRF_REQUIRE(p->y != p->x && p->y != p->skip, CRF_ERR_ARG, "apply record: the output aliases an input");
+    CRF_REQUIRE(crfconv_linear_forward_apply_supported(Ci, Co), CRF_ERR_UNSUPPORTED, "apply prologue: %d -> %d (multiples of 4, Ci <= 128)", Ci, Co);
+    if (int rc = crfconv_bn_coef_from_nrecords(p->stat_rec, p->nrec, M, Ci, p->gamma, p->beta, p->run_mean, p->run_var, p->momentum, p->eps,
+                                               p->coef, stream)) return rc;
+    const int tiles = (Co + 15) / 16;
+    const int tco = lf_tco(Ci, Co, false);
+    const int gy = (tiles + tco - 1) / tco;
+    const dim3 grid((unsigned)crf::lf_blocks(M), (unsigned)gy), blk(crf::LF_BLOCK);
+    const size_t lds = lf_lds_bytes_at(Ci, tco, false, true);
+    hipStream_t st = crf::as_stream(stream);
+    const int nch = lf_hoist_chunks(Ci, true);
+#define LFA2(T, N) hipLaunchKernelGGL((crf::linear_fwd_kernel<T, false, true, crf::EPI_APPLY, N>), grid, blk, lds, st, p->x, W, (const float*)nullptr, M, Ci, Co, 0, Y, stat_rec, (const float*)nullptr, (const float*)p->coef, p->slope, (const float*)nullptr, 0, (float*)nullptr, 0, p->skip, (const long long*)nullptr, 0ull, 0u, 1.f, (const float*)nullptr, 1.f, crf::UvFold(), p->y)
+#define LFA(T) do { if (nch == 1) LFA2(T, 1); else if (nch == 2) LFA2(T, 2); else if (nch == 4) LFA2(T, 4); else LFA2(T, 8); } while (0)
+    switch (tco) {
+        case 1: LFA(1); break;
+        case 2: LFA(2); break;
+        default: LFA(4); break;
+    }
+#undef LFA
+#undef LFA2
     CRF_LAUNCH_CHECK();
     return CRF_OK;
 }
diff --git a/crfconv_amd/models/common.py b/crfconv_amd/models/common.py
--- a/crfconv_amd/models/common.py
+++ b/crfconv_amd/models/common.py
@@ -53,14 +53,16 @@
         return x
 
 
-def mlp_fork(mlp, x, input_mask=None):
+def mlp_fork(mlp, x, input_mask=None, input_apply=None):
     if (mlp.training and mlp.bn is not None and x.dtype == torch.float32 and mlp.bn.batch_norm.affine and x.requires_grad
             and mlp.lin.out_features % 4 == 0 and mlp.lin.out_features <= 1024
             and (mlp.activation is None or isinstance(mlp.activation, nn.LeakyReLU))
             and ops.mlp_block_ok(x, mlp.lin.weight, mlp.lin.bias, mlp.bn.batch_norm, True)):
         require_gpu(x)
         slope = 1.0 if mlp.activation is None else mlp.activation.negative_slope
-        return ops.mlp_block(x, mlp.lin.weight, mlp.bn.batch_norm, slope, fork=True, input_mask=input_mask)
+        return ops.mlp_block(x, mlp.lin.weight, mlp.bn.batch_norm, slope, fork=True, input_mask=input_mask, input_apply=input_apply)
+    if input_apply is not None:
+        input_apply.flush()
     return mlp(x), x
 
 
@@ -71,7 +73,7 @@
     return mlp.lin.weight, mlp.bn.batch_norm, (1.0 if mlp.activation is None else mlp.activation.negative_slope)
 
 
-def mlp_group(pairs, shared=False, input_mask=None):
+def mlp_group(pairs, shared=False, input_mask=None, input_apply=None):
     blocks = []
     for mlp, x, fork in pairs:
         spec = _group_spec(mlp, x)
@@ -79,13 +81,13 @@
             return None
         require_gpu(x)
         blocks.append((x, spec[0], spec[1], spec[2], fork))
-    return ops.mlp_group(blocks, shared=shared, input_mask=input_mask)
+    return ops.mlp_group(blocks, shared=shared, input_mask=input_mask, input_apply=input_apply)
 
 
-def mlp_join(mlp, x, skip, slope=0.01, mask=None, combine=None):
+def mlp_join(mlp, x, skip, slope=0.01, mask=None, combine=None, apply=None):
     if (mlp.training and mlp.bn is not None and mlp.activation is None and mlp.lin.bias is None and x.dtype == torch.float32
             and mlp.bn.batch_norm.affine and mlp.lin.out_features % 4 == 0):
-        out = ops.mlp_block_join(x, mlp.lin.weight, mlp.bn.batch_norm, skip, slope, mask=mask, combine=combine)
+        out = ops.mlp_block_join(x, mlp.lin.weight, mlp.bn.batch_norm, skip, slope, mask=mask, combine=combine, apply=apply)
         if out is not None:
             return out
     if combine is not None:
diff --git a/crfconv_amd/models/point_conv_big.py b/crfconv_amd/models/point_conv_big.py
--- a/crfconv_amd/models/point_conv_big.py
+++ b/crfconv_amd/models/point_conv_big.py
@@ -74,21 +74,22 @@
         pooled = ops.neighbor_maxpool(_flat(x), table_of(idx, x.shape[1]))
         return pooled.reshape(x.shape[0], -1, x.shape[-1])
 
-    def forward(self, x, pos, neighbor_idx, return_input_alias=False, prefold=None, join_mask=None, input_mask=None):
+    def forward(self, x, pos, neighbor_idx, return_input_alias=False, prefold=None, join_mask=None, input_mask=None, join_apply=None,
+                input_apply=None):
         strided = not torch.is_tensor(pos)
         skip = None
         sc = self.shortcut
         grouped = None
         if isinstance(sc, MLP):
-            grouped = mlp_group([(self.lin_in, x, True), (sc, x, False)], shared=True, input_mask=input_mask)
+            grouped = mlp_group([(self.lin_in, x, True), (sc, x, False)], shared=True, input_mask=input_mask, input_apply=input_apply)
         if grouped is not None:
             (h_in, x), skip = grouped
             if strided:
                 skip = self.max_pooling(skip, neighbor_idx)
             y, comb = self.point_conv(h_in, pos, neighbor_idx, prefold=prefold, defer_combine=True)
-            out = mlp_join(self.lin_out, y, skip, 0.01, mask=join_mask, combine=comb)
+            out = mlp_join(self.lin_out, y, skip, 0.01, mask=join_mask, combine=comb, apply=join_apply)
             return (out, x) if return_input_alias else out
-        h_in, x = mlp_fork(self.lin_in, x, input_mask)
+        h_in, x = mlp_fork(self.lin_in, x, input_mask, input_apply)
         if (strided and self.training and isinstance(sc, MLP) and sc.bn is not None and sc.activation is None
                 and sc.lin.bias is None and x.dtype == torch.float32 and sc.bn.batch_norm.affine):
             pooled = ops.mlp_block_pool(_flat(x), sc.lin.weight, sc.bn.batch_norm, table_of(neighbor_idx, x.shape[1]),
@@ -106,7 +107,7 @@
             if strided:
                 skip = self.max_pooling(skip, neighbor_idx)
         y, comb = self.point_conv(h_in, pos, neighbor_idx, prefold=prefold, defer_combine=True)
-        out = mlp_join(self.lin_out, y, skip, 0.01, mask=join_mask, combine=comb)
+        out = mlp_join(self.lin_out, y, skip, 0.01, mask=join_mask, combine=comb, apply=join_apply)
         return (out, x) if return_input_alias else out
 
 
@@ -171,16 +172,19 @@
         if self.training and data.x.is_cuda and not ops.state.no_prefold:
             pre = ops.point_conv_prefold([blk.point_conv.prefold_entry(p, i) for blk, p, i in plan], True)
         masks = [ops.JoinMask() for _ in plan]
-        h = plan[0][0](data.x, plan[0][1], plan[0][2], prefold=pre[0], join_mask=masks[0])
-        h = plan[1][0](h, plan[1][1], plan[1][2], prefold=pre[1], join_mask=masks[1], input_mask=masks[0])
+        applies = [ops.ApplyHandle() for _ in plan]
+        h = plan[0][0](data.x, plan[0][1], plan[0][2], prefold=pre[0], join_mask=masks[0], join_apply=applies[0])
+        h = plan[1][0](h, plan[1][1], plan[1][2], prefold=pre[1], join_mask=masks[1], input_mask=masks[0], join_apply=applies[1],
+                       input_apply=applies[0])
         skips = [h]
         for lvl in range(1, len(WIDTHS)):
             if lvl == 2 and self.phase_hook is not None:
                 self.phase_hook('coarse')
             (b1, p1, i1), (b2, p2, i2) = plan[2 * lvl], plan[2 * lvl + 1]
-            h, skips[-1] = b1(h, p1, i1, return_input_alias=True, prefold=pre[2 * lvl], join_mask=masks[2 * lvl], input_mask=masks[2 * lvl - 1])
+            h, skips[-1] = b1(h, p1, i1, return_input_alias=True, prefold=pre[2 * lvl], join_mask=masks[2 * lvl], input_mask=masks[2 * lvl - 1],
+                              join_apply=applies[2 * lvl], input_apply=applies[2 * lvl - 1])
             h = b2(h, p2, i2, prefold=pre[2 * lvl + 1], join_mask=masks[2 * lvl + 1] if lvl + 1 < len(WIDTHS) else None,
-                   input_mask=masks[2 * lvl])
+                   input_mask=masks[2 * lvl], join_apply=applies[2 * lvl + 1] if lvl + 1 < len(WIDTHS) else None, input_apply=applies[2 * lvl])
             skips.append(h)
         ops.flush_riders()
         for d, mat, lvl in zip(decoders, mats, range(len(WIDTHS) - 2, -1, -1)):
diff --git a/crfconv_amd/ops/_base.py b/crfconv_amd/ops/_base.py
--- a/crfconv_amd/ops/_base.py
+++ b/crfconv_amd/ops/_base.py
@@ -140,6 +140,8 @@
     no_prefold = False
     no_mask_fold = __import__('os').environ.get('CRFCONV_NO_MASK_FOLD') is not None
     no_combine_fold = _env_families('CRFCONV_NO_COMBINE_FOLD')
+    no_apply_fold = _env_families('CRFCONV_NO_APPLY_FOLD')
+    apply_fold_min_elems = 4 << 20
     small_mlp_disabled = __import__('os').environ.get('CRFCONV_NO_ONE_LAUNCH_MLP') is not None
     small_bwd_one_launch = __import__('os').environ.get('CRFCONV_SMALL_BWD_TWO_LAUNCHES') is None
     dw_hosts_mats = __import__('os').environ.get('CRFCONV_NO_TAIL_RIDERS') is None
diff --git a/crfconv_amd/ops/mlp.py b/crfconv_amd/ops/mlp.py
--- a/crfconv_amd/ops/mlp.py
+++ b/crfconv_amd/ops/mlp.py
@@ -23,6 +23,48 @@
     return float(mask.slope)
 
 
+class ApplyHandle:
+    __slots__ = ('args', 'out')
+
+    def __init__(self):
+        self.args = self.out = None
+
+    def arm(self, rec, y, g, b, run_mean, run_var, momentum, eps, skip, slope, coef, out):
+        self.args = (rec, y, g, b, run_mean, run_var, float(momentum), float(eps), skip, float(slope), coef, out)
+        self.out = out
+
+    @property
+    def pending(self):
+        return self.args is not None
+
+    @staticmethod
+    def fold_off(family):
+        off = state.no_apply_fold
+        return off is True or (bool(off) and family in off)
+
+    def feeds(self, x):
+        return self.pending and x.data_ptr() == self.out.data_ptr() and tuple(x.shape) == tuple(self.out.shape) and x.is_contiguous()
+
+    def _job(self):
+        adr = lambda t: None if t is None else t.data_ptr()
+        rec, y, g, b, rm, rv, mom, eps, skip, slope, coef, out = self.args
+        return _lib.BnApplyJob(adr(rec), rec.shape[0], adr(y), y.shape[0], y.shape[1], adr(g), adr(b), adr(rm), adr(rv), mom, eps,
+                               adr(skip), slope, adr(coef), adr(out))
+
+    def take(self):
+        job, keep = self._job(), self.args
+        self.args = self.out = None
+        return job, keep
+
+    def flush(self):
+        if self.args is None:
+            return
+        rec, y, g, b, rm, rv, mom, eps, skip, slope, coef, out = self.args
+        _lib.call('crfconv_bn_apply_from_records', ptr(rec), rec.shape[0], ptr(y), y.shape[0], y.shape[1], ptr(g), ptr(b), ptr(rm), ptr(rv),
+                  mom, eps, ptr(skip), slope, ptr(coef), ptr(out), stream_ptr())
+        self.args = self.out = None
+
+
 def _bn_args(bn):
     return bn.weight, bn.bias, bn.running_mean, bn.running_var, 0.1 if bn.momentum is None else bn.momentum, bn.eps
 
@@ -31,9 +73,16 @@
     return bool(fork and x.requires_grad and torch.is_grad_enabled() and not state.no_fork)
 
 
-def _stream_fwd(x, Wc, gamma, beta, run_mean, run_var, momentum, eps, slope=None, skip=None, fold=None):
+def _stream_fwd(x, Wc, gamma, beta, run_mean, run_var, momentum, eps, slope=None, skip=None, fold=None, apply=None, defer=None):
     st = stream_ptr()
-    if fold is not None:
+    if apply is not None:
+        m, ci = x.shape
+        co = Wc.shape[0]
+        y = torch.empty((m, co), dtype=torch.float32, device=x.device)
+        nrec = _lib.load().crfconv_linear_forward_stat_records(m)
+        rec = torch.empty((nrec, 4, co), dtype=torch.float32, device=x.device)
+        _lib.call('crfconv_linear_forward_apply', ctypes.byref(apply[0]), ptr(Wc), m, ci, co, ptr(y), ptr(rec), st)
+    elif fold is not None:
         m, ci = x.shape
         co = Wc.shape[0]
         y = torch.empty((m, co), dtype=torch.float32, device=x.device)
@@ -58,6 +107,9 @@
                   float(eps), ptr(coef), st)
         return y, coef, None
     out = torch.empty_like(y)
+    if defer is not None:
+        defer.arm(rec, y, g, b, run_mean, run_var, momentum, eps, skip, slope, coef, out)
+        return y, coef, out
     _lib.call('crfconv_bn_apply_from_records', ptr(rec), rec.shape[0], ptr(y), m, co, ptr(g), ptr(b), ptr(run_mean), ptr(run_var),
               float(momentum), float(eps), ptr(skip), float(slope), ptr(coef), ptr(out), st)
     return y, coef, out
@@ -114,12 +166,12 @@
 class _MLPBlock(torch.autograd.Function):
 
     @staticmethod
-    def forward(ctx, x_in, W, gamma, beta, run_mean, run_var, momentum, eps, slope, fork=False, mask=None):
+    def forward(ctx, x_in, W, gamma, beta, run_mean, run_var, momentum, eps, slope, fork=False, mask=None, apply=None):
         x = x_in.contiguous()
         Wc = W.contiguous()
         ci, co = x.shape[1], Wc.shape[0]
         ctx.mask_slope = _take_mask(mask, fork and ci % 4 == 0 and co % 4 == 0)
-        y, coef, out = _stream_fwd(x, Wc, gamma, beta, run_mean, run_var, momentum, eps, slope)
+        y, coef, out = _stream_fwd(x, Wc, gamma, beta, run_mean, run_var, momentum, eps, slope, apply=apply)
         ctx.prm = (W, gamma, beta)
         ctx.save_for_backward(x, Wc, y, coef)
         ctx.slope = float(slope)
@@ -133,16 +185,16 @@
         x, W, y, coef = ctx.saved_tensors
         gA = torch.zeros_like(y) if gA is None else gA.contiguous()
         return (*_stream_bwd(ctx.prm, x, W, y, coef, gA, ctx.slope, ctx.needs_input_grad[0], True, g_alias, ctx.mask_slope),
-                None, None, None, None, None, None, None)
+                None, None, None, None, None, None, None, None)
 
 
 class _MLPBlockJoin(torch.autograd.Function):
 
     @staticmethod
-    def forward(ctx, x, W, gamma, beta, run_mean, run_var, momentum, eps, skip, slope, mask=None, fold=None):
+    def forward(ctx, x, W, gamma, beta, run_mean, run_var, momentum, eps, skip, slope, mask=None, fold=None, defer=None):
         x, Wc, skip = x.contiguous(), W.contiguous(), skip.contiguous()
         ctx.mask = mask
-        y, coef, out = _stream_fwd(x, Wc, gamma, beta, run_mean, run_var, momentum, eps, slope, skip, fold)
+        y, coef, out = _stream_fwd(x, Wc, gamma, beta, run_mean, run_var, momentum, eps, slope, skip, fold, defer=defer)
         ctx.prm = (W, gamma, beta)
         ctx.save_for_backward(x, Wc, y, coef, out)
         ctx.slope = float(slope)
@@ -153,7 +205,7 @@
         x, W, y, coef, out = ctx.saved_tensors
         g1 = _join_g1(ctx, g.contiguous(), out)
         gskip = g1 if ctx.needs_input_grad[8] else None
-        return (*_stream_bwd(ctx.prm, x, W, y, coef, g1, 1.0, ctx.needs_input_grad[0]), None, None, None, None, gskip, None, None, None)
+        return (*_stream_bwd(ctx.prm, x, W, y, coef, g1, 1.0, ctx.needs_input_grad[0]), None, None, None, None, gskip, None, None, None, None)
 
 
 class _MLPBlockDropout(torch.autograd.Function):
@@ -475,7 +527,7 @@
     return 'tiled' if lib.crfconv_gemm_stats_uv_supported(m, co, ci) == 1 else None
 
 
-def mlp_block_join(x, W, bn, skip, slope, mask=None, combine=None):
+def mlp_block_join(x, W, bn, skip, slope, mask=None, combine=None, apply=None):
     if state.no_join or skip.shape[:-1] != x.shape[:-1] or skip.shape[-1] != W.shape[0] or skip.dtype != torch.float32:
         return None
     m = x.numel() // x.shape[-1]
@@ -497,7 +549,11 @@
         mask.slope = float(slope)
     else:
         mask = None
-    out = fn.apply(x.reshape(-1, ci), W, *_bn_args(bn), skip.reshape(-1, co), slope, mask, fold)
+    if (not small and apply is not None and not apply.pending and not apply.fold_off('join') and torch.is_grad_enabled()
+            and m * co >= state.apply_fold_min_elems):
+        out = fn.apply(x.reshape(-1, ci), W, *_bn_args(bn), skip.reshape(-1, co), slope, mask, fold, apply)
+    else:
+        out = fn.apply(x.reshape(-1, ci), W, *_bn_args(bn), skip.reshape(-1, co), slope, mask, fold)
     return out.reshape(x.shape[:-1] + (co,))
 
 
@@ -628,7 +684,7 @@
         return tuple(rets)
 
 
-def mlp_group(blocks, shared=False, input_mask=None):
+def mlp_group(blocks, shared=False, input_mask=None, input_apply=None):
     if not (2 <= len(blocks) <= 4):
         return None
     lib = _lib.load()
@@ -649,6 +705,8 @@
         args += [xa, W, *_bn_args(bn), float(slope), use_fork]
         shapes.append((x.shape, W.shape[0], fork, use_fork))
     fold = input_mask if (shared and len(blocks) == 2 and args[9]) else None
+    if input_apply is not None:
+        input_apply.flush()
     res = list(_MLPSmallGroup.apply(bool(shared), fold, *args))
     out = []
     for (xs, co, fork, use_fork), (x, _, _, _, _) in zip(shapes, blocks):
@@ -740,16 +798,23 @@
             and _lib.load().crfconv_mlp_backward_supported(m, ci, co) == 1)
 
 
-def mlp_block(x, W, bn, slope=1.0, fork=False, input_mask=None):
+def mlp_block(x, W, bn, slope=1.0, fork=False, input_mask=None, input_apply=None):
     require_gpu(x, W)
     shape = x.shape
     tick(bn)
     x2 = x.reshape(-1, shape[-1])
     fn = _MLPSmall if _mlp_small_ok(x2.shape[0], shape[-1], W.shape[0]) else _MLPBlock
+    apply = None
+    if input_apply is not None and input_apply.pending:
+        if (fn is _MLPBlock and input_apply.feeds(x2) and not input_apply.fold_off('join')
+                and _lib.load().crfconv_linear_forward_apply_supported(shape[-1], W.shape[0]) == 1):
+            apply = input_apply.take()
+        else:
+            input_apply.flush()
     if _use_fork(fork, x2):
-        out, alias = fn.apply(x2, W, *_bn_args(bn), slope, True, input_mask)
+        out, alias = fn.apply(x2, W, *_bn_args(bn), slope, True, input_mask, *(() if apply is None else (apply,)))
         return out.reshape(shape[:-1] + (W.shape[0],)), alias.reshape(shape)
-    out = fn.apply(x2, W, *_bn_args(bn), slope, False, None)
+    out = fn.apply(x2, W, *_bn_args(bn), slope, False, None, *(() if apply is None else (apply,)))
     out = out.reshape(shape[:-1] + (W.shape[0],))
     return (out, x) if fork else out
 
diff --git a/include/crfconv_amd.h b/include/crfconv_amd.h
--- a/include/crfconv_amd.h
+++ b/include/crfconv_amd.h
@@ -350,6 +350,9 @@
                  float* run_mean; float* run_var; float momentum; float eps; const float* skip; float slope; float* coef; float* y;
 } crf_bn_apply_job;
 int crfconv_bn_apply_from_records_jobs(const crf_bn_apply_job* jobs, int njobs, crf_stream_t stream);
+int crfconv_linear_forward_apply_supported(int Ci, int Co);
+int crfconv_linear_forward_apply(const crf_bn_apply_job* p, const float* W, int64_t M, int Ci, int Co, float* Y, float* stat_rec,
+                                 crf_stream_t stream);
 typedef struct { const float* gA; const float* Y; const float* coef; const float* W; const float* addend; int64_t M; int Ci; int Co;
                  int training; float slope; float* gY; float* dX; float* dgamma; float* dbeta; void* workspace; size_t workspace_bytes;
                  const float* mask_ref; float mask_slope;
```

Result: no change. 45.62 M points/s (-0.1%).
